# Hansard-T/FHE-Linformer

Hardware: AMD Instinct MI355X
Metric: encrypted Linformer-d128 forward ms/sample (lower is better)
Workload: dtype u64

## Files before the change

fhe-linformer_amd/capi.py:

```python
import ctypes as C
import os

import numpy as np

_HERE = os.path.dirname(os.path.abspath(__file__))
_LIB = None


class FhelinError(RuntimeError):
    def __init__(self, code, msg):
        super().__init__(f"fhelin error {code}: {msg}")
        self.code = code


class Params(C.Structure):
    _fields_ = [
        ("log_n", C.c_int32), ("n_q", C.c_int32), ("first_bits", C.c_int32), ("scale_bits", C.c_int32),
        ("n_p", C.c_int32), ("special_bits", C.c_int32), ("dnum", C.c_int32), ("log_slots", C.c_int32),
        ("hamming", C.c_int32), ("device", C.c_int32), ("seed", C.c_uint64),
    ]


PRESETS = {
    "bench": dict(log_n=16, n_q=24, first_bits=55, scale_bits=52, n_p=6, special_bits=60, dnum=4, log_slots=14, hamming=192),
# ... 127 lines not shown
        "fhelin_fc_rotsum": (i32, [vp, vp, i32, i32, C.POINTER(vp)]),
        "fhelin_fc_repeat": (i32, [vp, vp, i32, i32, C.POINTER(vp)]),
        "fhelin_fc_add_many": (i32, [vp, C.POINTER(vp), i32, C.POINTER(vp)]),
        "fhelin_fc_matmul_pt": (i32, [vp, C.POINTER(vp), i32, vp, vp, i32, i32, C.POINTER(vp)]),
        "fhelin_fc_matmul_ct": (i32, [vp, C.POINTER(vp), i32, vp, i32, i32, C.POINTER(vp)]),
        "fhelin_fc_matmulRElarge": (i32, [vp, C.POINTER(vp), i32, C.POINTER(vp), i32, vp, C.c_double, C.POINTER(vp)]),
        "fhelin_fc_matmulCRlarge": (i32, [vp, C.POINTER(vp), i32, C.POINTER(vp), vp, C.POINTER(vp)]),
        "fhelin_fc_matmulScores": (i32, [vp, C.POINTER(vp), i32, vp, C.POINTER(vp)]),
        "fhelin_fc_wrapUpRepeated": (i32, [vp, C.POINTER(vp), i32, C.POINTER(vp)]),
        "fhelin_fc_wrapUpExpanded": (i32, [vp, C.POINTER(vp), i32, C.POINTER(vp)]),
        "fhelin_fc_unwrapExpanded": (i32, [vp, vp, i32, C.POINTER(vp)]),
        "fhelin_fc_unwrapScoresExpanded": (i32, [vp, vp, i32, C.POINTER(vp)]),
        "fhelin_fc_unwrap_512_in_4_128": (i32, [vp, vp, i32, C.POINTER(vp)]),
        "fhelin_fc_unwrapRepeatedLarge": (i32, [vp, C.POINTER(vp), i32, i32, C.POINTER(vp)]),
        "fhelin_fc_generate_containers": (i32, [vp, C.POINTER(vp), i32, vp, C.POINTER(vp), C.POINTER(i32)]),
        "fhelin_fc_wrap_containers": (i32, [vp, C.POINTER(vp), i32, i32, C.POINTER(vp)]),
        "fhelin_mult_real": (i32, [vp, vp, C.c_double, C.POINTER(vp)]),
        "fhelin_add_real": (i32, [vp, vp, C.c_double, C.POINTER(vp)]),
        "fhelin_mult_many": (i32, [vp, C.POINTER(vp), i32, C.POINTER(vp)]),
        "fhelin_lincomb": (i32, [vp, C.POINTER(vp), C.POINTER(C.c_double), i32, C.c_double, C.POINTER(vp)]),
        "fhelin_eval_poly": (i32, [vp, vp, C.POINTER(C.c_double), i32, C.POINTER(vp)]),
        "fhelin_eval_chebyshev": (i32, [vp, vp, C.POINTER(C.c_double), i32, C.c_double, C.c_double, C.POINTER(vp)]),
        "fhelin_eval_chebyshev_batch": (i32, [vp, C.POINTER(vp), i32, C.POINTER(C.c_double), i32, C.c_double, C.c_double, C.POINTER(vp)]),
        "fhelin_bootstrap_setup": (i32, [vp, i32, i32, i32]),
        "fhelin_bootstrap": (i32, [vp, vp, C.POINTER(vp)]),
        "fhelin_bootstrap_config": (i32, [vp, i32, i32, i32, i32]),
        "fhelin_bootstrap_partial": (i32, [vp, vp, i32, C.POINTER(vp)]),
        "fhelin_bootstrap_drop": (i32, [vp, vp, i32, C.POINTER(vp)]),
        "fhelin_bootstrap_batch": (i32, [vp, C.POINTER(vp), i32, C.POINTER(vp)]),
        "fhelin_bootstrap_iter": (i32, [vp, vp, i32, C.POINTER(vp)]),
        "fhelin_bootstrap_iter_batch": (i32, [vp, C.POINTER(vp), i32, i32, C.POINTER(vp)]),
        "fhelin_bootstrap_iter_drop": (i32, [vp, vp, i32, i32, C.POINTER(vp)]),
        "fhelin_bootstrap_describe": (i32, [vp, C.POINTER(i32), i32, C.POINTER(i32)]),
        "fhelin_bootstrap_diag": (i32, [vp, i32, i32, i32, C.POINTER(vp)]),
        "fhelin_bootstrap_cheb": (i32, [vp, C.POINTER(C.c_double), i32, C.POINTER(i32)]),
        "fhelin_fcb_matmulScores": (i32, [vp, C.POINTER(vp), i32, C.POINTER(vp), i32, C.POINTER(vp)]),
        "fhelin_fcb_matmul_ct": (i32, [vp, C.POINTER(vp), C.POINTER(vp), i32, i32, i32, C.POINTER(vp)]),
        "fhelin_fcb_wrapUpRepeated": (i32, [vp, C.POINTER(vp), i32, i32, C.POINTER(vp)]),
        "fhelin_fcb_wrapUpExpanded": (i32, [vp, C.POINTER(vp), i32, i32, C.POINTER(vp)]),
        "fhelin_fcb_unwrapExpanded": (i32, [vp, C.POINTER(vp), i32, i32, C.POINTER(vp)]),
        "fhelin_fcb_unwrapRepeatedLarge": (i32, [vp, C.POINTER(vp), i32, i32, i32, C.POINTER(vp)]),
        "fhelin_fcb_generate_containers": (i32, [vp, C.POINTER(vp), i32, i32, vp, C.POINTER(vp), C.POINTER(i32)]),
        "fhelin_fc_rotsum_batch": (i32, [vp, C.POINTER(vp), i32, i32, i32, i32, C.POINTER(vp)]),
        "fhelin_add_plain_batch": (i32, [vp, C.POINTER(vp), i32, vp, C.POINTER(vp)]),
        "fhelin_eval_poly_batch": (i32, [vp, C.POINTER(vp), i32, C.POINTER(C.c_double), i32, C.POINTER(vp)]),
        "fhelin_mult_many_batch": (i32, [vp, C.POINTER(vp), i32, i32, C.POINTER(vp)]),
        "fhelin_evalkeys_save": (i32, [vp, C.c_char_p]),
        "fhelin_evalkeys_params": (i32, [C.c_char_p, C.POINTER(Params)]),
        "fhelin_evalkeys_info": (i32, [C.c_char_p, C.POINTER(i32), C.POINTER(i32)]),
        "fhelin_evalkeys_load": (i32, [vp, C.c_char_p]),
        "fhelin_evalkeys_save_compact": (i32, [vp, C.c_char_p]),
        "fhelin_ctx_set_seeded_keys": (i32, [vp, i32]),
        "fhelin_ctx_key_set_seed": (i32, [vp, vp]),
        "fhelin_debug_key_digest": (i32, [vp, vp, i32, i32, C.POINTER(C.c_uint64), C.POINTER(i32)]),
        "fhelin_ctx_set_seeded_encryption": (i32, [vp, i32]),
        "fhelin_ct_compact_bytes": (i32, [vp, C.POINTER(C.c_size_t)]),
        "fhelin_ct_export_compact": (i32, [vp, vp, vp, C.c_size_t]),
        "fhelin_compact_info": (i32, [vp, C.c_size_t, C.POINTER(i32), C.POINTER(i32), C.POINTER(i32), C.POINTER(i32)]),
        "fhelin_ct_import_compact": (i32, [vp, C.POINTER(vp), C.POINTER(C.c_size_t), i32, C.POINTER(vp)]),
        "fhelin_debug_seeded_expand": (i32, [vp, vp, C.c_uint64, i32, i32, i32, vp, f32p]),
        "fhelin_client_ingest_wrapped": (i32, [vp, vp, vp, vp, i32, i32, vp, vp, vp, vp, vp, vp, i32, i32, vp, C.POINTER(vp),
                                               C.POINTER(i32), vp]),
        "fhelin_client_ingest_wrapped_interleaved": (i32, [vp, i32, C.POINTER(vp), C.POINTER(vp), vp, i32, i32, vp, vp, vp, vp, vp, vp, i32,
                                                           i32, vp, C.POINTER(vp), C.POINTER(i32), C.POINTER(vp)]),
        "fhelin_wrapped_info": (i32, [vp, C.POINTER(i32), C.POINTER(i32), C.POINTER(i32), vp, i32]),
        "fhelin_unwrap_inputs": (i32, [vp, C.POINTER(vp), i32, C.POINTER(vp)]),
        "fhelin_sanitize": (i32, [vp, C.POINTER(vp), i32, vp, i32, i32, C.POINTER(vp)]),
        "fhelin_debug_flood": (i32, [vp, vp, C.c_uint64, i32, i32, vp, C.c_size_t]),
        "fhelin_decrypt_flooded": (i32, [vp, vp, i32, C.POINTER(C.c_double), i32]),
        "fhelin_debug_sampler_peek": (i32, [vp, i32, vp, u64p]),
        "fhelin_debug_pt_from_residues": (i32, [vp, vp, i32, C.POINTER(vp)]),
        "fhelin_debug_pt_from_residues_full": (i32, [vp, vp, C.c_double, C.c_double, C.POINTER(vp)]),
        "fhelin_lt_create": (i32, [vp, C.POINTER(C.c_double), C.POINTER(i32), i32, i32, i32, C.POINTER(vp)]),
        "fhelin_lt_create_pts": (i32, [vp, C.POINTER(vp), C.POINTER(i32), C.POINTER(i32), i32, i32, C.POINTER(vp)]),
        "fhelin_lt_info": (i32, [vp, C.POINTER(i32), C.POINTER(i32), C.POINTER(i32), C.POINTER(i32)]),
        "fhelin_lt_rotations": (i32, [vp, C.POINTER(i32), i32, C.POINTER(i32)]),
        "fhelin_lt_apply": (i32, [vp, vp, C.POINTER(vp), i32, i32, C.POINTER(vp)]),
        "fhelin_lt_free": (None, [vp]),
        "fhelin_debug_dot_plain": (i32, [vp, C.POINTER(vp), C.POINTER(vp), i32, C.POINTER(vp)]),
        "fhelin_debug_dot_groups": (i32, [vp, C.POINTER(vp), i32, i32, C.POINTER(vp), i32, C.POINTER(vp)]),
        "fhelin_debug_dot_cyclic": (i32, [vp, C.POINTER(vp), i32, C.POINTER(vp), C.POINTER(vp)]),
        "fhelin_debug_dot_window": (i32, [vp, C.POINTER(vp), C.POINTER(vp), C.POINTER(vp), C.POINTER(vp), i32]),
        "fhelin_debug_rotate_many_batch": (i32, [vp, C.POINTER(vp), i32, C.POINTER(i32), i32, C.POINTER(vp)]),
        "fhelin_ctx_set_interleave": (i32, [vp, i32]),
        "fhelin_ctx_interleave": (i32, [vp, C.POINTER(i32)]),
        "fhelin_evalkeys_interleave": (i32, [C.c_char_p, C.POINTER(i32)]),
        "fhelin_encrypt_interleaved_batch": (i32, [vp, C.POINTER(C.c_double), i32, i32, i32, i32, C.POINTER(vp)]),
        "fhelin_decrypt_interleaved": (i32, [vp, vp, i32, C.POINTER(C.c_double), i32]),
        "fhelin_decrypt_batch": (i32, [vp, C.POINTER(vp), i32, i32, i32, C.POINTER(i32), i32, C.POINTER(C.c_double), i32]),
        "fhelin_ctx_set_device_decode": (i32, [vp, i32]),
        "fhelin_client_ingest_interleaved": (i32, [vp, i32, C.POINTER(vp), C.POINTER(vp), vp, i32, i32, vp, vp, vp, vp, vp, vp, i32, i32,
                                                   C.POINTER(vp), C.POINTER(vp)]),
    }
    for name, (res, args) in sigs.items():
        fn = getattr(lib, name)
        fn.restype = res
        fn.argtypes = args
    _LIB = lib
    return lib


def compact_info(blob):
    lib = load_library()
    b = bytes(blob)
    v = [C.c_int32() for _ in range(4)]
    rc = lib.fhelin_compact_info(C.c_char_p(b), len(b), *[C.byref(x) for x in v])
    if rc != 0:
        raise FhelinError(rc, lib.fhelin_last_error().decode())
    return dict(zip(("log_n", "ell", "deg", "slots"), (x.value for x in v)))


def interleave(vectors):
    v = np.asarray(vectors)
    assert v.ndim == 2
    return np.ascontiguousarray(v.T).reshape(-1)


def deinterleave(physical, stride):
    w = np.asarray(physical)
    assert w.ndim == 1 and w.size % stride == 0
    return np.ascontiguousarray(w.reshape(-1, stride).T)


def _np_u64(a):
    a = np.ascontiguousarray(a, dtype=np.uint64)
    return a, a.ctypes.data_as(C.c_void_p)


class DevBuf:

    def __init__(self, eng, nbytes):
        self.eng, self.nbytes = eng, int(nbytes)
        p = C.c_void_p()
        eng._ck(eng.lib.fhelin_dev_alloc(eng.h, self.nbytes, C.byref(p)))
        self.ptr = p

    def upload(self, arr):
        arr = np.ascontiguousarray(arr)
        assert arr.nbytes <= self.nbytes
        self.eng._ck(self.eng.lib.fhelin_dev_upload(self.eng.h, self.ptr, arr.ctypes.data_as(C.c_void_p), arr.nbytes))
        return self

    def download(self, shape, dtype=np.uint64):
        out = np.empty(shape, dtype=dtype)
        assert out.nbytes <= self.nbytes
        self.eng._ck(self.eng.lib.fhelin_dev_download(self.eng.h, out.ctypes.data_as(C.c_void_p), self.ptr, out.nbytes))
        return out

    def free(self):
        if self.ptr:
            self.eng._ck(self.eng.lib.fhelin_dev_free(self.eng.h, self.ptr))
            self.ptr = None


class Engine:

    def __init__(self, preset="bench", device=0, seed=0, seed_bytes=None, interleave=1, **overrides):
        self.lib = load_library()
        cfg = dict(PRESETS[preset]) if isinstance(preset, str) else dict(preset)
        cfg.update(overrides)
        self.params = Params(device=device, seed=seed, **cfg)
        h = C.c_void_p()
        if seed_bytes is not None:
            assert len(seed_bytes) == 32
            sb = (C.c_uint8 * 32)(*bytes(seed_bytes))
            rc = self.lib.fhelin_ctx_create_seeded(C.byref(self.params), sb, C.byref(h))
# ... 632 lines not shown

    def raw_mult_relin(self, a, b):
        return self._un(self.lib.fhelin_raw_mult_relin, a, b.h)

    @staticmethod
    def _harr_opt(objs):
        return (C.c_void_p * len(objs))(*[(o.h if o is not None else None) for o in objs])

    def debug_pt_from_residues(self, residues):
        r = np.ascontiguousarray(residues, dtype=np.uint64)
        ell, n = r.shape
        assert n == self.N
        h = C.c_void_p()
        self._ck(self.lib.fhelin_debug_pt_from_residues(self.h, r.ctypes.data_as(C.c_void_p), ell, C.byref(h)))
        return Pt(self, h)

    def debug_pt_from_residues_full(self, residues, scale):
        r = np.ascontiguousarray(residues, dtype=np.uint64)
        assert r.shape == (self.n_q + self.n_p, self.N)
        hi = float(scale)
        lo = float(np.longdouble(scale) - np.longdouble(hi))
        h = C.c_void_p()
        self._ck(self.lib.fhelin_debug_pt_from_residues_full(self.h, r.ctypes.data_as(C.c_void_p), hi, lo, C.byref(h)))
        return Pt(self, h)

    def lt_create(self, diags, indices, n1=0, slots=None):
        slots = (1 << self.params.log_slots) if slots is None else int(slots)
        n = len(indices)
        d = np.ascontiguousarray(diags, dtype=np.float64).reshape(n, -1) if n else np.zeros((0, slots))
        assert n == 0 or d.shape[1] == slots
        idx = (C.c_int32 * max(n, 1))(*[int(i) for i in indices])
        h = C.c_void_p()
        self._ck(self.lib.fhelin_lt_create(self.h, d.ctypes.data_as(C.POINTER(C.c_double)), idx, n, slots, int(n1), C.byref(h)))
        return LinearTransform(self, h)

    def lt_create_pts(self, pts, baby, giant):
        n2, n1 = len(giant), len(baby)
        assert len(pts) == n2 and all(len(r) == n1 for r in pts)
        b = (C.c_int32 * n1)(*[int(i) for i in baby])
        g = (C.c_int32 * n2)(*[int(i) for i in giant])
        h = C.c_void_p()
        self._ck(self.lib.fhelin_lt_create_pts(self.h, self._harr_opt([p for r in pts for p in r]), b, g, n1, n2, C.byref(h)))
        return LinearTransform(self, h)

    def lt_apply(self, lt, v, rescale=False):
        outs = self._outs(max(len(v), 1))
        self._ck(self.lib.fhelin_lt_apply(self.h, lt.h, self._harr(v), len(v), int(bool(rescale)), outs))
        return self._cts(outs, len(v))

    def debug_dot_plain(self, cts, pts):
        assert len(cts) == len(pts)
        h = C.c_void_p()
        self._ck(self.lib.fhelin_debug_dot_plain(self.h, self._harr(cts), self._harr(pts), len(cts), C.byref(h)))
        return Ct(self, h)

    def debug_dot_groups(self, cts, pts):
        nb, na, ng = len(cts), len(cts[0]), len(pts)
        assert all(len(r) == na for r in cts) and all(len(r) == na for r in pts)
        outs = self._outs(nb * ng)
        self._ck(self.lib.fhelin_debug_dot_groups(self.h, self._harr([c for r in cts for c in r]), nb, na,
                                                  self._harr_opt([p for r in pts for p in r]), ng, outs))
        flat = self._cts(outs, nb * ng)
        return [flat[x * ng:(x + 1) * ng] for x in range(nb)]

    def debug_dot_cyclic(self, cts, pts):
        assert len(pts) == 32
        outs = self._outs(32)
        self._ck(self.lib.fhelin_debug_dot_cyclic(self.h, self._harr(cts), len(cts), self._harr(pts), outs))
        return self._cts(outs, 32)

    def debug_dot_window(self, cur, prev, pts, dest, accumulate=False):
        assert len(cur) == len(prev) == len(pts) == len(dest) == 32
        self._ck(self.lib.fhelin_debug_dot_window(self.h, self._harr_opt(cur), self._harr_opt(prev), self._harr(pts), self._harr(dest),
                                                  int(bool(accumulate))))

    def debug_rotate_many_batch(self, cts, indices):
        n = len(indices)
        idx = (C.c_int32 * n)(*indices)
        outs = self._outs(len(cts) * n)
        self._ck(self.lib.fhelin_debug_rotate_many_batch(self.h, self._harr(cts), len(cts), idx, n, outs))
        flat = self._cts(outs, len(cts) * n)
        return [flat[i * n:(i + 1) * n] for i in range(len(cts))]

    @staticmethod
    def _harr(objs):
        return (C.c_void_p * len(objs))(*[o.h for o in objs])

    def _outs(self, n):
        return (C.c_void_p * n)()

    def _cts(self, arr, n):
        return [Ct(self, C.c_void_p(arr[i])) for i in range(n)]

    def mult_real(self, a, k):
        return self._un(self.lib.fhelin_mult_real, a, float(k))

    def add_real(self, a, k):
        return self._un(self.lib.fhelin_add_real, a, float(k))

    def mult_many(self, v):
        h = C.c_void_p()
        self._ck(self.lib.fhelin_mult_many(self.h, self._harr(v), len(v), C.byref(h)))
        return Ct(self, h)

    def lincomb(self, v, coeffs, c0=0.0):
        cf = np.ascontiguousarray(coeffs, dtype=np.float64)
        h = C.c_void_p()
        self._ck(self.lib.fhelin_lincomb(self.h, self._harr(v), cf.ctypes.data_as(C.POINTER(C.c_double)), len(v), float(c0), C.byref(h)))
        return Ct(self, h)

    def eval_poly(self, x, coeffs):
        cf = np.ascontiguousarray(coeffs, dtype=np.float64)
        return self._un(self.lib.fhelin_eval_poly, x, cf.ctypes.data_as(C.POINTER(C.c_double)), cf.size)

    def eval_chebyshev(self, x, coeffs, a=-1.0, b=1.0):
        cf = np.ascontiguousarray(coeffs, dtype=np.float64)
        return self._un(self.lib.fhelin_eval_chebyshev, x, cf.ctypes.data_as(C.POINTER(C.c_double)), cf.size, float(a), float(b))

    def eval_chebyshev_batch(self, xs, coeffs, a=-1.0, b=1.0):
        cf = np.ascontiguousarray(coeffs, dtype=np.float64)
        outs = self._outs(len(xs))
        self._ck(self.lib.fhelin_eval_chebyshev_batch(self.h, self._harr(xs), len(xs), cf.ctypes.data_as(C.POINTER(C.c_double)), cf.size,
                                                      float(a), float(b), outs))
        return self._cts(outs, len(xs))

    def bootstrap(self, a):
        return self._un(self.lib.fhelin_bootstrap, a)

    def bootstrap_setup(self, budget_enc=3, budget_dec=3, slots=0):
        self._ck(self.lib.fhelin_bootstrap_setup(self.h, budget_enc, budget_dec, slots))

    def bootstrap_config(self, K=28, R=3, cheb_degree=47, correction=10):
        self._ck(self.lib.fhelin_bootstrap_config(self.h, K, R, cheb_degree, correction))

    def bootstrap_batch(self, v):
        outs = self._outs(len(v))
        self._ck(self.lib.fhelin_bootstrap_batch(self.h, self._harr(v), len(v), outs))
        return self._cts(outs, len(v))

    def bootstrap_drop(self, a, drop):
        return self._un(self.lib.fhelin_bootstrap_drop, a, int(drop))

    def bootstrap_iter(self, a, precision):
        return self._un(self.lib.fhelin_bootstrap_iter, a, int(precision))

    def bootstrap_iter_batch(self, v, precision):
        outs = self._outs(len(v))
        self._ck(self.lib.fhelin_bootstrap_iter_batch(self.h, self._harr(v), len(v), int(precision), outs))
        return self._cts(outs, len(v))

    def bootstrap_iter_drop(self, a, precision, drop):
        return self._un(self.lib.fhelin_bootstrap_iter_drop, a, int(precision), int(drop))

    def bootstrap_describe(self):
        n = C.c_int32()
        self._ck(self.lib.fhelin_bootstrap_describe(self.h, None, 0, C.byref(n)))
        d = (C.c_int32 * n.value)()
        self._ck(self.lib.fhelin_bootstrap_describe(self.h, d, n.value, C.byref(n)))
        d = list(d)
        out = dict(zip(("packed", "slots", "K", "R", "cheb_degree", "correction", "depth"), d[:7]))
        out["packed"] = bool(out["packed"])
        n_c2s, n_s2c = d[7], d[8]
        pos, stages = 9, []
        for k in range(n_c2s + n_s2c):
            which, idx = (0, k) if k < n_c2s else (1, k - n_c2s)
            st_slots, nt = d[pos], d[pos + 1]
# ... 306 lines not shown
```

fhe-linformer_amd/csrc/capi_debug.cpp:

```cpp
#include "../../include/fhelin.h"
#include <hip/hip_runtime.h>
#include <algorithm>
#include <vector>
#include "capi_internal.h"

using namespace fhelin;

#define NEED(x) if (!(x)) return capi_fail(FHELIN_ERR_ARG, "null argument")

namespace {
std::vector<CtPtr> cts_in(fhelin_ctx* c, const fhelin_ct* const* v, int n, bool nullable = false) {
    std::vector<CtPtr> in(n);
    for (int i = 0; i < n; ++i) {
        if (!v[i]) {
            if (!nullable) throw Error(FHELIN_ERR_ARG, "null ciphertext in array");
            continue;
        }
        const CtPtr& p = ct_in(c, v[i]);
        if (p->npoly != 2 || p->deg != 1) throw Error(FHELIN_ERR_ARG, "debug_dot: operands are degree-1 ciphertexts of two components");
        in[i] = p;
    }
    return in;
}
std::vector<PtPtr> pts_in(const fhelin_pt* const* v, int n, bool nullable = false) {
// ... 58 lines not shown

int fhelin_debug_dot_plain(fhelin_ctx* c, const fhelin_ct* const* cts, const fhelin_pt* const* pts, int32_t n, fhelin_ct** out) {
    NEED(c && cts && pts && out);
    FHELIN_TRY
    if (n < 1) throw Error(FHELIN_ERR_ARG, "debug_dot_plain: at least one term");
    *out = wrap(c, c->ev.dot_plain(cts_in(c, cts, n), pts_in(pts, n)));
    FHELIN_CATCH
}

int fhelin_debug_dot_groups(fhelin_ctx* c, const fhelin_ct* const* cts, int32_t nb, int32_t na, const fhelin_pt* const* pts, int32_t ng,
                            fhelin_ct** outs) {
    NEED(c && cts && pts && outs);
    FHELIN_TRY
    if (nb < 1 || na < 1 || na > EwDotGroups::MAX_A || ng < 1 || ng > EwDotGroups::MAX_G)
        throw Error(FHELIN_ERR_ARG, "debug_dot_groups: 1 <= na <= 16, 1 <= ng <= 8, nb >= 1");
    std::vector<CtPtr> flat = cts_in(c, cts, nb * na);
    std::vector<std::vector<PtPtr>> p(ng);
    for (int g = 0; g < ng; ++g) p[g] = pts_in(pts + (size_t)g * na, na, true);
    const CtPtr& f = flat[0];
    for (const CtPtr& x : flat)
        if (x->ell != f->ell) throw Error(FHELIN_ERR_ARG, "debug_dot_groups: operands of one limb count");
    std::vector<CtPtr> dest = c->ev.new_ct_batch(nb * ng, 2, f->ell, f->deg + 1, f->scale, f->slots);
    bool ok;
    if (nb == 1) {
        ok = c->ev.dot_plain_groups(flat, p, 0, dest);
    } else {
        flat = c->ev.make_contiguous(flat);
        std::vector<std::vector<CtPtr>> in(nb), o(nb);
        for (int x = 0; x < nb; ++x) {
            in[x].assign(flat.begin() + (size_t)x * na, flat.begin() + (size_t)(x + 1) * na);
            o[x].assign(dest.begin() + (size_t)x * ng, dest.begin() + (size_t)(x + 1) * ng);
        }
        ok = c->ev.dot_plain_groups_batch(in, p, 0, o);
    }
    if (!ok) throw Error(FHELIN_ERR_STATE, "debug_dot_groups: the evaluator refused the operands (no fall-back here)");
    for (int i = 0; i < nb * ng; ++i) outs[i] = wrap(c, dest[i]);
    FHELIN_CATCH
}

int fhelin_debug_dot_cyclic(fhelin_ctx* c, const fhelin_ct* const* cts, int32_t n, const fhelin_pt* const* pts, fhelin_ct** outs) {
    NEED(c && cts && pts && outs);
    FHELIN_TRY
    constexpr int P = EwCyclic::PERIOD;
    if (n < 1 || n > P) throw Error(FHELIN_ERR_ARG, "debug_dot_cyclic: 1 <= n <= 32");
    std::vector<CtPtr> in = cts_in(c, cts, n);
    std::vector<CtPtr> dest = c->ev.new_ct_batch(P, 2, in[0]->ell, in[0]->deg + 1, in[0]->scale, in[0]->slots);
    if (!c->ev.dot_plain_cyclic(in, pts_in(pts, P), dest))
        throw Error(FHELIN_ERR_STATE, "debug_dot_cyclic: the evaluator refused the operands (no fall-back here)");
    for (int k = 0; k < P; ++k) outs[k] = wrap(c, dest[k]);
    FHELIN_CATCH
}

int fhelin_debug_dot_window(fhelin_ctx* c, const fhelin_ct* const* cur, const fhelin_ct* const* prev, const fhelin_pt* const* pts,
                            fhelin_ct* const* dest, int32_t accumulate) {
    NEED(c && cur && prev && pts && dest);
    FHELIN_TRY
    constexpr int W = EwWindow::W;
    std::vector<CtPtr> d(W);
    for (int t = 0; t < W; ++t) {
        if (!dest[t]) throw Error(FHELIN_ERR_ARG, "null ciphertext in array");
        d[t] = ct_in(c, dest[t]);
    }
    if (!c->ev.dot_plain_window(cts_in(c, cur, W, true), cts_in(c, prev, W, true), pts_in(pts, W), d, accumulate != 0))
        throw Error(FHELIN_ERR_STATE, "debug_dot_window: the evaluator refused the operands (no fall-back here)");
    FHELIN_CATCH
}

int fhelin_debug_rotate_many_batch(fhelin_ctx* c, const fhelin_ct* const* cts, int32_t n_ct, const int32_t* indices, int32_t n,
                                   fhelin_ct** outs) {
    NEED(c && cts && indices && outs);
    FHELIN_TRY
    if (n_ct < 1 || n < 1) throw Error(FHELIN_ERR_ARG, "debug_rotate_many_batch: at least one ciphertext and one index");
    std::vector<CtPtr> in(n_ct);
    for (int i = 0; i < n_ct; ++i) {
        if (!cts[i]) throw Error(FHELIN_ERR_ARG, "null ciphertext in array");
        in[i] = ct_in(c, cts[i]);
    }
    const std::vector<std::vector<CtPtr>> o = c->ev.rotate_many_batch(in, std::vector<int>(indices, indices + n));
    for (int i = 0; i < n_ct; ++i)
        for (int k = 0; k < n; ++k) outs[(size_t)i * n + k] = wrap(c, o[i][k]);
    FHELIN_CATCH
}

}
```

fhe-linformer_amd/csrc/context.cpp:

```cpp
#include "context.h"
#include <hip/hip_runtime.h>
#include <algorithm>
#include <cstdio>
#include <cstdlib>
#include <cstring>
#include <sys/random.h>
#include <time.h>
#include <cxxabi.h>
#include <dlfcn.h>
#include <execinfo.h>

namespace fhelin {

template <class T>
const T* Context::upload_table(const std::vector<T>& v) {
    void* p = nullptr;
    size_t bytes = std::max<size_t>(v.size() * sizeof(T), 16);
    hip_check(hipMalloc(&p, bytes), "hipMalloc(table)");
    if (!v.empty()) hip_check(hipMemcpy(p, v.data(), v.size() * sizeof(T), hipMemcpyHostToDevice), "hipMemcpy(table)");
    table_allocs.push_back(p);
    return static_cast<const T*>(p);
}
template const u64* Context::upload_table<u64>(const std::vector<u64>&);
template const int* Context::upload_table<int>(const std::vector<int>&);
// ... 19 lines not shown
        while (got < sizeof p.seed_bytes) {
            const ssize_t n = getrandom(p.seed_bytes + got, sizeof p.seed_bytes - got, 0);
            if (n <= 0) throw Error(FHELIN_ERR_INTERNAL, "getrandom failed: no entropy for key generation");
            got += (size_t)n;
        }
    }
    p.have_seed_bytes = true;
}

static Params resolve_params(Params p) {
    resolve_seed(p);
    if (p.n_p < 0 && p.n_q >= 1 && p.dnum >= 1 && p.special_bits >= 1) {
        const int a = (p.n_q + p.dnum - 1) / p.dnum;
        const int first = p.first_bits + (std::min(a, p.n_q) - 1) * p.scale_bits;
        const int other = p.n_q > a ? std::min(a, p.n_q - a) * p.scale_bits : 0;
        p.n_p = (std::max(first, other) + p.special_bits - 1) / p.special_bits;
    }
    return p;
}

Context::Context(const Params& p_in) : prm(resolve_params(p_in)) {
    const Params& p = prm;
    if (p.log_n < 12 || p.log_n > 17) throw Error(FHELIN_ERR_ARG, "log_n must be in [12,17]");
    if (p.n_q < 1 || p.n_q > 64 || p.n_p < 0 || p.n_p > 16) throw Error(FHELIN_ERR_ARG, "bad limb counts");
    if (p.dnum < 1) throw Error(FHELIN_ERR_ARG, "dnum must be >= 1");
    if (p.first_bits > 60 || p.scale_bits > 60 || p.special_bits > 60) throw Error(FHELIN_ERR_ARG, "primes must be <= 60 bits");
    if (p.first_bits < 20 || p.scale_bits < 20 || (p.n_p > 0 && p.special_bits < 20)) throw Error(FHELIN_ERR_ARG, "primes must be >= 20 bits");
    if (p.log_slots < 1 || p.log_slots > p.log_n - 1) throw Error(FHELIN_ERR_ARG, "log_slots out of range");
    N = 1 << p.log_n;
    L = p.n_q - 1;
    K = p.n_p;
    alpha = (p.n_q + p.dnum - 1) / p.dnum;
    if (alpha > 16) throw Error(FHELIN_ERR_ARG, "digit size > 16 limbs not supported");
    if ((p.n_q + alpha - 1) / alpha > 16) throw Error(FHELIN_ERR_ARG, "more than 16 key-switching digits not supported");
    try {
        chain = make_prime_chain(p.log_n, p.n_q, p.first_bits, p.scale_bits, p.n_p, p.special_bits);
    } catch (const std::exception& e) {
        throw Error(FHELIN_ERR_ARG, std::string("prime chain: ") + e.what());
    }
    moduli = chain.q;
    moduli.insert(moduli.end(), chain.p.begin(), chain.p.end());
    for (u64 q : moduli)
        if (q >> 60) throw Error(FHELIN_ERR_ARG, "prime chain: a modulus is >= 2^60 (lower scale_bits or first_bits)");
    for (u64 q : moduli) {
        barrett.push_back(h_barrett(q));
        tw.push_back(make_twiddles(q, p.log_n));
    }
    sf_real.assign(p.n_q + 1, 0.0L);
    sf_real[0] = (long double)chain.q[L];
    for (int k = 0; k < L; ++k) sf_real[k + 1] = sf_real[k] * sf_real[k] / (long double)chain.q[L - k];

    pool.fill_word = DevicePool::parse_fill(std::getenv("FHELIN_POOL_FILL"));

    if (p.device < 0) return;

    int ndev = 0;
    if (hipGetDeviceCount(&ndev) != hipSuccess || ndev <= 0)
        throw Error(FHELIN_ERR_NO_DEVICE, "no HIP device visible: the fhe-linformer_amd engine has no CPU fallback");
    if (p.device >= ndev) throw Error(FHELIN_ERR_ARG, "device index out of range");
    hip_check(hipSetDevice(p.device), "hipSetDevice");
    hip_check(hipStreamCreateWithFlags(&stream, hipStreamNonBlocking), "hipStreamCreate");
    main_stream = stream;
    own_stream = true;
    {
        int want = 2;
        if (const char* e = std::getenv("FHELIN_LANES")) want = std::atoi(e);
        n_lanes = std::max(0, std::min(want, DevicePool::MAX_LANES - 1));
        for (int k = 1; k <= n_lanes; ++k) {
            hip_check(hipStreamCreateWithFlags(&lane_stream[k], hipStreamNonBlocking), "hipStreamCreate(lane)");
            hip_check(hipEventCreateWithFlags(&lane_event[k], hipEventDisableTiming), "hipEventCreate(lane)");
        }
        hip_check(hipEventCreateWithFlags(&fork_event, hipEventDisableTiming), "hipEventCreate(fork)");
        pool.lane_stream[0] = main_stream;
        for (int k = 1; k <= n_lanes; ++k) pool.lane_stream[k] = lane_stream[k];
        pool.have_streams = true;
        if (const char* e = std::getenv("FHELIN_ASYNC")) async_lanes = std::atoi(e) != 0;
        if (const char* e = std::getenv("FHELIN_FUSE_MODDOWN")) fuse_moddown = std::atoi(e) != 0;
        if (const char* e = std::getenv("FHELIN_FUSE_FINISH")) fuse_finish = std::atoi(e) != 0;
        if (const char* e = std::getenv("FHELIN_HOST_ENCODE")) host_encode = std::atoi(e) != 0;
        if (const char* e = std::getenv("FHELIN_DEVICE_DECODE")) device_decode = std::atoi(e) != 0;
        if (const char* e = std::getenv("FHELIN_ROT_GATHER")) rot_gather = std::atoi(e) != 0;
        if (const char* e = std::getenv("FHELIN_FUSE_LIFT")) fuse_lift = std::atoi(e) != 0;
        if (const char* e = std::getenv("FHELIN_LDS_DIGITS")) lds_digits = std::atoi(e) != 0;
        if (const char* e = std::getenv("FHELIN_NTT_TRACE")) trace_small_ntt = std::atoi(e);
        if (const char* e = std::getenv("FHELIN_SCALAR_TRACE")) trace_scalar = std::atoi(e);
        if (const char* e = std::getenv("FHELIN_HOST_WAITS")) trace_waits = std::atoi(e) != 0;
    }
    hip_check(hipEventCreate(&ev_start), "hipEventCreate");
    stage_words = (size_t)2 << p.log_n;
    for (int i = 0; i < STAGE_SLOTS; ++i) {
        hip_check(hipHostMalloc(reinterpret_cast<void**>(&stage_buf[i]), stage_words * sizeof(u64), hipHostMallocDefault), "hipHostMalloc(stage)");
        hip_check(hipEventCreateWithFlags(&stage_ev[i], hipEventDisableTiming), "hipEventCreate(stage)");
    }
    hip_check(hipHostMalloc(reinterpret_cast<void**>(&small_buf), (size_t)SMALL_SLOTS * SMALL_WORDS * sizeof(u64), hipHostMallocDefault), "hipHostMalloc(stage, small)");
    for (int i = 0; i < SMALL_SLOTS; ++i) hip_check(hipEventCreateWithFlags(&small_ev[i], hipEventDisableTiming), "hipEventCreate(stage, small)");
    hip_check(hipEventCreate(&ev_stop), "hipEventCreate");
    has_device = true;

    const int nl = (int)moduli.size();
    {
        std::vector<u64> bar(2 * nl), ninv(8 * nl, 0);
        for (int i = 0; i < nl; ++i) {
            bar[2 * i] = barrett[i].r0;
            bar[2 * i + 1] = barrett[i].r1;
            ninv[8 * i] = tw[i].n_inv;
            ninv[8 * i + 1] = tw[i].n_inv_s;
            ninv[8 * i + 2] = tw[i].w1_n_inv;
            ninv[8 * i + 3] = tw[i].w1_n_inv_s;
            int bits = 0;
            while (bits < 64 && (moduli[i] >> bits)) ++bits;
            if (bits >= 12 && bits <= 60) {
                ninv[8 * i + 4] = (u64)(bits - 10);
                ninv[8 * i + 5] = (u64)((((u128)1) << (bits + 22)) / moduli[i]);
            }
        }
        dt.log_n = p.log_n;
        dt.n_limbs = nl;
        dt.moduli = upload_table(moduli);
        dt.barrett = upload_table(bar);
        {
            std::vector<u64> qi(nl);
            for (int i = 0; i < nl; ++i) {
                u64 x = moduli[i];
                for (int it = 0; it < 6; ++it) x *= 2 - moduli[i] * x;
                qi[i] = x;
            }
            dt.qinv = upload_table(qi);
            std::vector<u64> mr(2 * (size_t)nl);
            for (int i = 0; i < nl; ++i) {
                mr[2 * i] = mont_r(moduli[i]);
                mr[2 * i + 1] = h_shoup(mr[2 * i], moduli[i]);
            }
            dt.mont = upload_table(mr);
        }
        dt.ninv = upload_table(ninv);
        std::vector<u64> f((size_t)nl * 2 * N), g((size_t)nl * 2 * N);
        for (int i = 0; i < nl; ++i) {
            std::memcpy(&f[(size_t)i * 2 * N], tw[i].fwd.data(), sizeof(u64) * 2 * N);
            std::memcpy(&g[(size_t)i * 2 * N], tw[i].inv.data(), sizeof(u64) * 2 * N);
        }
        dt.tw_fwd = upload_table(f);
        dt.tw_inv = upload_table(g);
        const size_t tiles = N >> 12;
        const size_t per_limb = tiles * 15 * 256 * 2;
        for (int dir = 0; dir < 2; ++dir) {
            const std::vector<u64>& src = dir ? g : f;
            std::vector<u64> r((size_t)nl * per_limb);
            for (int i = 0; i < nl; ++i)
                for (size_t T = 0; T < tiles; ++T)
                    for (int kb = 0; kb < 4; ++kb)
                        for (int j = 0; j < (8 >> kb); ++j)
                            for (size_t tau = 0; tau < 256; ++tau) {
                                const size_t idx = (N >> (kb + 1)) + ((((T << 8) | tau)) << (3 - kb)) + j;
                                const size_t s_ = (size_t)(8 >> kb) - 1 + j;
                                const size_t o = (size_t)i * per_limb + ((T * 15 + s_) * 256 + tau) * 2;
                                r[o] = src[(size_t)i * 2 * N + 2 * idx];
                                r[o + 1] = src[(size_t)i * 2 * N + 2 * idx + 1];
                            }
            (dir ? dt.tw_rows_inv : dt.tw_rows_fwd) = upload_table(r);
        }
    }
    {
        std::vector<u64> phatinv(2 * std::max(K, 1)), phatmod((size_t)std::max(K, 1) * (L + 1)), pinv(2 * (L + 1));
        for (int j = 0; j < K; ++j) {
            u64 pj = chain.p[j];
            u64 hat = prod_mod(chain.p, j, pj);
// ... 307 lines not shown
```

fhe-linformer_amd/csrc/context.h:

```cpp
#pragma once
#include <cstdint>
#include <map>
#include <memory>
#include <stdexcept>
#include <string>
#include <unordered_map>
#include <vector>
#include <hip/hip_runtime_api.h>
#include "../../include/fhelin.h"
#include "hostmath.h"
#include "pool.h"
#include "kernels.h"

namespace fhelin {

struct Params {
    int log_n = 16;
    int n_q = 24;
    int first_bits = 55;
    int scale_bits = 52;
    int n_p = 6;
    int special_bits = 60;
    int dnum = 4;
    int log_slots = 14;
// ... 51 lines not shown
    hipStream_t lane_stream[DevicePool::MAX_LANES] = {};
    hipEvent_t lane_event[DevicePool::MAX_LANES] = {};
    hipEvent_t fork_event = nullptr;
    bool async_lanes = true;
    int async_rr = 0;
    u64 lane_seq[DevicePool::MAX_LANES] = {};
    std::vector<std::pair<u64, std::shared_ptr<void>>> lane_hold[DevicePool::MAX_LANES];
    void release_holds(int lane, u64 up_to_seq);
    void fork_lanes();
    void join_lanes();
    struct LaneScope {
        Context& c;
        LaneScope(Context& ctx, int k) : c(ctx) {
            c.stream = c.lane_stream[k];
            c.pool.cur_lane = k;
        }
        ~LaneScope() {
            c.stream = c.main_stream;
            c.pool.cur_lane = 0;
        }
    };
    DevicePool pool;
    DeviceTables dt{};
    std::vector<void*> table_allocs;
    hipEvent_t ev_start = nullptr, ev_stop = nullptr;

    static constexpr int STAGE_SLOTS = 64;
    u64* stage_buf[STAGE_SLOTS] = {};
    hipEvent_t stage_ev[STAGE_SLOTS] = {};
    bool stage_used[STAGE_SLOTS] = {};
    int stage_next = 0;
    size_t stage_words = 0;
    static constexpr int SMALL_SLOTS = 256;
    static constexpr size_t SMALL_WORDS = 8192;
    u64* small_buf = nullptr;
    hipEvent_t small_ev[SMALL_SLOTS] = {};
    bool small_used[SMALL_SLOTS] = {};
    int small_next = 0;
    void upload_async(u64* dst, const u64* src, size_t words);

    const u64* d_phatinv = nullptr;
    const u64* d_phatmod = nullptr;
    const u64* d_pinv = nullptr;
    const u64* d_pmod = nullptr;
    const u64* d_qlinv = nullptr;
    const u64* d_qlmod = nullptr;
    std::vector<LevelTables> lvl;
    std::map<u64, const u32*> automorph_maps;

    explicit Context(const Params& p);
    ~Context();
    Context(const Context&) = delete;
    Context& operator=(const Context&) = delete;

    void require_device() const;
    template <class T> T* dalloc(size_t count) { return static_cast<T*>(pool.alloc(count * sizeof(T))); }
    template <class T> Scratch<T> scratch(size_t count) { return Scratch<T>(pool, count); }
    template <class T> const T* upload_table(const std::vector<T>& v);
    int limb_id_q(int i) const { return i; }
    int limb_id_p(int j) const { return L + 1 + j; }
    int digits_at(int ell) const { return (ell + alpha - 1) / alpha; }
    u64 galois_element(long rot_index) const;
    int stride = 1;
    bool stride_explicit = false;
    bool stride_locked = false;
    u64 rot_element(int rot_index) const { return stride == 1 ? galois_element(rot_index) : galois_element((long)stride * rot_index); }
    struct PhysicalScope {
        Context& c;
        int was;
        explicit PhysicalScope(Context& ctx) : c(ctx), was(ctx.stride) { c.stride = 1; }
        ~PhysicalScope() { c.stride = was; }
    };
    const u32* automorph_map(u64 galois);
    const u32* automorph_inverse_of(const u32* map);
    std::map<const u32*, const u32*> automorph_inverse;
    u32 automorph_ginv_of(const u32* map) const;
    std::map<const u32*, u32> automorph_ginv;
    bool fuse_finish = true;
    bool fuse_moddown = false;
    bool host_encode = false;
    bool device_decode = false;
    bool rot_gather = true;
    bool fuse_lift = true;
    bool lds_digits = true;
    struct FftDev {
        const u32* rot = nullptr;
        const double* ksi = nullptr;
    };
    std::map<int, FftDev> fft_dev;
    void sync();
    void ntt(const LimbBatch& b, bool inverse, int active = -1) {
        stats.limb_ntt += (u64)(active >= 0 ? active : b.nvec);
        if (trace_small_ntt && b.nvec <= trace_small_ntt) note_small_ntt(b.nvec);
        launch_ntt(dt, b, inverse, stream);
    }
    bool trace_waits = false;
    std::map<std::string, std::pair<u64, u64>> wait_sites;
    void note_wait(const char* site, u64 ns) {
        auto& e = wait_sites[site];
        e.first += 1;
        e.second += ns;
    }
    int trace_small_ntt = 0;
    std::map<std::string, std::pair<u64, u64>> small_ntt_sites;
    void note_small_ntt(int nvec);
    int trace_scalar = 0;
    std::map<std::string, std::pair<u64, u64>> scalar_sites;
    void note_scalar(int nvec);
    void ntt_epilogue(const LimbBatch& b, const NttEpilogue& ep) {
        stats.limb_ntt += (u64)b.nvec;
        if (trace_small_ntt && b.nvec <= trace_small_ntt) note_small_ntt(b.nvec);
        launch_ntt_epilogue(dt, b, ep, stream);
    }
};

}
```

fhe-linformer_amd/csrc/evaluator.cpp:

```cpp
#include "evaluator.h"
#include <map>
#include <hip/hip_runtime.h>
#include <cmath>
#include <cstring>

namespace fhelin {

DevBlock::~DevBlock() {
    if (d && ctx) {
        try { ctx->pool.free(d); } catch (...) {}
    }
}
Ciphertext::~Ciphertext() {
    if (async_ev) (void)hipEventDestroy(async_ev);
    if (d && ctx && !block) {
        try { ctx->pool.free(d); } catch (...) {}
    }
}
Encoding::~Encoding() {
    if (ready) (void)hipEventDestroy(ready);
    if (d && ctx) {
        try { ctx->pool.free(d, lanes_ordered); } catch (...) {}
    }
}
// ... 115 lines not shown
            it.b[i] = nullptr;
        }
        launch_ew_items(c_.dt, it, 4, v[0]->ell, c_.stream);
    }
    hip_check(hipGetLastError(), "batch gather");
    return o;
}

KeyPtr Evaluator::new_key() {
    c_.require_device();
    auto k = std::make_shared<EvalKey>();
    k->ctx = &c_;
    k->digits = c_.digits_at(c_.L + 1);
    k->d = c_.dalloc<u64>(k->words());
    c_.stride_locked = true;
    return k;
}

void Evaluator::keyswitch(const u64* c_ntt, int ell, const EvalKey& key, u64* out, const u64* add0, const u64* add1,
                          const u32* map, const u64* post) {
    keyswitch_batch(1, c_ntt, 0, ell, key, out, 0, add0, add1, 0, map, post, 0);
}

void Evaluator::keyswitch_batch(int B, const u64* c_ntt, size_t c_stride, int ell, const EvalKey& key, u64* out, size_t out_stride,
                                const u64* add0, const u64* add1, size_t add_stride, const u32* map, const u64* post,
                                size_t post_stride) {
    keyswitch_impl(B, nullptr, c_ntt, c_stride, ell, &key, out, out_stride, add0, add1, add_stride, map, post, post_stride);
}

void Evaluator::keyswitch_rows(const KsRows& rows, const u64* c_ntt, size_t c_stride, int ell, u64* out, size_t out_stride,
                               const u64* add0, size_t add_stride) {
    const int B = (int)rows.keys.size();
    if (B < 1) return;
    if (B > KsShape::MAX_ROWS || rows.maps.size() != rows.keys.size()) throw Error(FHELIN_ERR_ARG, "keyswitch_rows: bad row count");
    keyswitch_impl(B, &rows, c_ntt, c_stride, ell, nullptr, out, out_stride, add0, nullptr, add_stride, nullptr, nullptr, 0);
}

void Evaluator::keyswitch_impl(int B, const KsRows* rows, const u64* c_ntt, size_t c_stride, int ell, const EvalKey* key, u64* out,
                               size_t out_stride, const u64* add0, const u64* add1, size_t add_stride, const u32* map, const u64* post,
                               size_t post_stride) {
    c_.require_device();
    if (c_.K < 1) throw Error(FHELIN_ERR_STATE, "hybrid key switching needs at least one special prime");
    if (B < 1) return;
    const size_t N = c_.N;
    const int K = c_.K;
    KsShape sh{ell, K, c_.alpha, c_.lvl[ell].beta, c_.L + 1, B, c_stride, out_stride, add_stride, post_stride};
    const bool shared = rows && rows->shared_input;
    if (rows) {
        sh.per_row = 1;
        sh.shared_input = shared ? 1 : 0;
        for (int b = 0; b < B; ++b) {
            sh.evk_row[b] = rows->keys[b]->d;
            sh.map_row[b] = rows->maps[b];
        }
    }
    KsShape shu = sh;
    shu.batch = shared ? 1 : B;
    c_.stats.keyswitch += (u64)B;
    c_.stats.keyswitch_limbs += (u64)B * ell;
    const bool identity = !map && !rows;
    const bool gather = !identity && !add1 && rot_in_gather();
    const u64* evk = key ? key->d : nullptr;
    if (gather) {
        sh.gather = 1;
        if (rows) {
            for (int b = 0; b < B; ++b) {
                sh.evk_row[b] = permuted(*rows->keys[b], rows->maps[b]);
                sh.ginv_row[b] = c_.automorph_ginv_of(rows->maps[b]);
            }
        } else {
            evk = permuted(*key, map);
            sh.map_row[0] = map;
            sh.ginv = c_.automorph_ginv_of(map);
        }
        if (add0) {
            sh.gsrc = add0;
            sh.gsrc_stride = add_stride;
            sh.gsrc_pmod = c_.d_pmod;
        }
    }
    Scratch<u64> ext = modup(shu, c_ntt, !gather);
    Scratch<u64> accQ = c_.scratch<u64>((size_t)B * 2 * ell * N);
    Scratch<u64> accP = c_.scratch<u64>((size_t)B * 2 * K * N);
    launch_ks_inner(c_.dt, sh, accQ, accP, ext, evk, c_ntt, c_.stream);
    if (gather) moddown(sh, accQ, accP, out, nullptr, nullptr, nullptr, post, true);
    else moddown(sh, accQ, accP, out, add0, add1, map, post, c_.fuse_moddown || (c_.fuse_finish && identity));
    launch_ok("keyswitch");
}


Scratch<u64> Evaluator::modup(const KsShape& up, const u64* src, bool times_r2, int group2, size_t group2_stride) {
    const size_t N = c_.N;
    const int n = up.batch, ell = up.ell, nt = ell + c_.K;
    const LevelTables& lt = c_.lvl[ell];
    Scratch<u64> cc = c_.scratch<u64>((size_t)n * ell * N);
    {
        LimbBatch ib{cc, n * ell, nullptr, 0, ell, src};
        if (n > 1 && up.c_stride != (size_t)ell * N) {
            ib.src_group = ell;
            ib.src_group_stride = up.c_stride;
        }
        if (group2 > 0) {
            ib.src_group2 = group2;
            ib.src_group2_stride = group2_stride;
        }
        c_.ntt(ib, true);
    }
    Scratch<u64> ext = c_.scratch<u64>((size_t)n * lt.beta * nt * N);
    launch_modup_conv(c_.dt, up, ext, cc, src, lt.up_hatinv, times_r2 ? lt.up_hatmod_r2 : lt.up_hatmod, c_.stream);
    LimbBatch eb{ext, n * lt.beta * nt, lt.ext_limb_tab, 0, 1};
    eb.tab_len = lt.beta * nt;
    eb.lazy_out = true;
    c_.ntt(eb, false, n * (lt.beta * nt - ell));
    return ext;
}

void Evaluator::moddown(const KsShape& sh, const u64* accQ, u64* accP, u64* out, const u64* add0, const u64* add1, const u32* map,
                        const u64* post, bool row_pass, const std::function<void(const u64* conv)>& finish) {
    const size_t N = c_.N;
    const int B = sh.batch, ell = sh.ell, K = c_.K;
    if (row_pass && sh.gsrc && !sh.gsrc_pmod) throw Error(FHELIN_ERR_INTERNAL, "moddown: the row pass cannot gather");
    c_.ntt(LimbBatch{accP, B * 2 * K, nullptr, c_.L + 1, K}, true);
    Scratch<u64> conv = c_.scratch<u64>((size_t)B * 2 * ell * N);
    launch_moddown_conv(c_.dt, sh, conv, accP, c_.d_phatinv, c_.d_phatmod, c_.stream);
    const LimbBatch cb{conv, B * 2 * ell, nullptr, 0, ell};
    if (row_pass) {
        NttEpilogue ep;
        ep.acc = accQ;
        ep.acc_poly_stride = (size_t)ell * N;
        ep.out = out;
        ep.out_stride = sh.out_stride;
        ep.w = c_.d_pinv;
        ep.ell = ell;
        ep.add0 = add0;
        ep.add1 = add1;
        ep.add_stride = sh.add_stride;
        ep.post = post;
        ep.post_stride = sh.post_stride;
        if (sh.gather) {
        } else if (sh.per_row) {
            ep.per_row = 1;
            for (int b = 0; b < B; ++b) ep.invmap_row[b] = c_.automorph_inverse_of(sh.map_row[b]);
        } else if (map) {
            ep.invmap = c_.automorph_inverse_of(map);
        }
        c_.ntt_epilogue(cb, ep);
        return;
    }
    c_.ntt(cb, false);
    if (finish) finish(conv);
    else launch_moddown_finish(c_.dt, sh, out, accQ, conv, c_.d_pinv, add0, add1, map, post, c_.stream);
}

void Evaluator::moddown_rescale(const KsShape& sh, const u64* accQ, u64* accP, u64* out) {
    const size_t N = c_.N;
    const int B = sh.batch, ell = sh.ell, K = c_.K;
    const LevelTables& lt = c_.lvl[ell];
    c_.ntt(LimbBatch{accP, B * 2 * K, nullptr, c_.L + 1, K}, true);
    Scratch<u64> top = c_.scratch<u64>((size_t)B * 2 * N);
    {
        LimbBatch tb{top, B * 2, nullptr, ell - 1, 1, accQ + (size_t)(ell - 1) * N};
        tb.src_group = 1;
        tb.src_group_stride = (size_t)ell * N;
        c_.ntt(tb, true);
    }
    Scratch<u64> conv = c_.scratch<u64>((size_t)B * 2 * (ell - 1) * N);
    launch_moddown_rescale_conv(c_.dt, sh, conv, accP, top, lt.md_hatinv, lt.md_hatmod, lt.md_mmod, c_.stream);
    moddown_rescale_finish(sh, out, accQ, conv, lt.md_minv);
}

void Evaluator::moddown_rescale_exact(const KsShape& sh, const u64* accQ, u64* accP, u64* out, u32 f2) {
    const size_t N = c_.N;
    const int B = sh.batch, ell = sh.ell, K = c_.K;
    const LevelTables& lt = c_.lvl[ell];
    {
        LimbBatch ib{accP, B * 2 * (K + 1), lt.mdx_limb_tab, 0, 1};
        ib.tab_len = K + 1;
        c_.ntt(ib, true);
    }
    Scratch<u64> conv = c_.scratch<u64>((size_t)B * 2 * (ell - 1) * N);
    launch_moddown_rescale_exact_conv(c_.dt, sh, f2, conv, accP, c_.d_phatinv, c_.d_phatmod, c_.d_pinv, c_.d_pmod,
                                      c_.d_qlmod + (size_t)(ell - 1) * (c_.L + 1), c_.stream);
    moddown_rescale_finish(sh, out, accQ, conv, lt.md_minv);
}

void Evaluator::moddown_rescale_finish(const KsShape& sh, u64* out, const u64* accQ, u64* conv, const u64* minv) {
    const int e1 = sh.ell - 1;
    const LimbBatch cb{conv, sh.batch * 2 * e1, nullptr, 0, e1};
    if (c_.fuse_finish) {
        NttEpilogue ep;
        ep.acc = accQ;
        ep.acc_poly_stride = (size_t)sh.ell * c_.N;
        ep.out = out;
        ep.out_stride = sh.out_stride;
        ep.w = minv;
        ep.ell = e1;
        c_.ntt_epilogue(cb, ep);
        return;
    }
    c_.ntt(cb, false);
    launch_moddown_rescale_finish(c_.dt, sh, out, accQ, conv, minv, c_.stream);
}

Evaluator::Rotations Evaluator::rotations(const int* indices, int n) {
    Rotations rot;
    rot.n = n;
    for (int r = 0; r < n; ++r) {
        const RotKey k = rotation_key(indices[r]);
        rot.key[r] = k.key.get();
        rot.map[r] = k.map;
        if (k.g % (u64)(c_.N / 256) != 1) rot.tiles_in_place = false;
    }
    return rot;
}

void Evaluator::set_rotations(KsShape& sh, const Rotations& rot, bool shared_digits, const u64* const* keys) {
    sh.n_rot = rot.n;
    for (int r = 0; r < rot.n; ++r) {
        sh.map_rot[r] = rot.map[r];
        sh.evk_rot[r] = keys ? keys[r] : permuted(*rot.key[r], rot.map[r]);
    }
    if (shared_digits) sh.lds_digits = c_.lds_digits && rot.tiles_in_place ? 1 : 0;
}

void Evaluator::rotation_sum(KsShape& sh, const u64* ext, const u64* c1, const u64* c0, size_t c0_stride, u64* out, const u64* post) {
    const size_t N = c_.N;
    const bool rp = sum_in_row_pass();
    sh.gsrc = c0;
    sh.gsrc_stride = c0_stride;
    if (rp) sh.gsrc_pmod = c_.d_pmod;
    Scratch<u64> accQ = c_.scratch<u64>((size_t)sh.batch * 2 * sh.ell * N);
    Scratch<u64> accP = c_.scratch<u64>((size_t)sh.batch * 2 * sh.k * N);
    launch_ks_inner_multi(c_.dt, sh, accQ, accP, ext, c1, c_.stream);
    moddown(sh, accQ, accP, out, nullptr, nullptr, nullptr, post, rp);
}

int Evaluator::slot_count(int slots) const { return slots > 0 ? slots : (1 << c_.prm.log_slots); }

Evaluator::RotKey Evaluator::rotation_key(int index) {
    const u64 g = c_.rot_element(index);
    auto it = rot_keys.find(g);
    if (it == rot_keys.end()) throw Error(FHELIN_ERR_KEY, "no rotation key for index " + std::to_string(index) + " (EvalRotateKeyGen list)");
    return RotKey{it->second, c_.automorph_map(g), g};
}

bool Evaluator::have_rotation_keys(const std::vector<int>& indices, int slots) const {
    const int ns = slot_count(slots);
    for (int r : indices) {
        if (r % ns == 0) return false;
        if (!rot_keys.count(c_.rot_element(r))) return false;
    }
    return !indices.empty();
}

const u64* Evaluator::permuted(const EvalKey& key, const u32* map) {
    if (key.d_perm) return key.d_perm;
    const int nvec = key.digits * 2 * (c_.L + 1 + c_.K);
    key.d_perm = c_.dalloc<u64>(key.words());
    launch_automorph_pack30(c_.dt, key.d_perm, key.d, map, nvec, c_.stream);
    launch_ok("key permutation");
    hip_check(hipStreamSynchronize(c_.stream), "key permutation sync");
    return key.d_perm;
}

std::vector<CtPtr> Evaluator::rotate_sum_batch(const std::vector<CtPtr>& vin, const std::vector<int>& indices) {
    if (vin.empty()) return {};
    const int R = (int)indices.size();
    if (R < 1 || R > KsShape::MAX_ROT) throw Error(FHELIN_ERR_ARG, "rotate_sum_batch: 1..7 rotations");
    if (!have_rotation_keys(indices, vin[0]->slots)) throw Error(FHELIN_ERR_KEY, "rotate_sum_batch: missing rotation key");
    if (c_.K < 1) throw Error(FHELIN_ERR_STATE, "hybrid key switching needs at least one special prime");
    const Rotations rot = rotations(indices.data(), R);
    const size_t N = c_.N;
    return for_groups(vin.size(), batch_limit, [&](size_t f, size_t i) { return same_shape(*vin[f], *vin[i]); },
                      [&](const std::vector<size_t>& idx) {
        if (vin[idx[0]]->npoly != 2) throw Error(FHELIN_ERR_STATE, "rotate: ciphertext must have 2 components");
        const std::vector<CtPtr> chunk = make_contiguous(pick(vin, idx), 0);
        const int B = (int)chunk.size(), ell = chunk[0]->ell;
        const size_t pn = (size_t)ell * N, ctw = 2 * pn;
        std::vector<CtPtr> o = new_ct_batch(B, 2, ell, chunk[0]->deg, chunk[0]->scale, chunk[0]->slots);
        const u64* base = chunk[0]->d;
        KsShape sh{ell, c_.K, c_.alpha, c_.lvl[ell].beta, c_.L + 1, B, ctw, ctw, pn, ctw};
        set_rotations(sh, rot, true);
        int steps = 0;
        while ((1 << steps) < R + 1) ++steps;
        c_.stats.keyswitch += (u64)B * steps;
        c_.stats.keyswitch_limbs += (u64)B * steps * ell;
        {
            Scratch<u64> ext = modup(sh, base + pn, false);
            rotation_sum(sh, ext, base + pn, base, ctw, o[0]->d, base);
            launch_ok("rotate_sum_batch");
        }
        for (int b = 0; b < B; ++b) o[b]->scale = vin[idx[b]]->scale;
        return o;
    });
}

Evaluator::FoldedKey Evaluator::folded_key(const PtPtr& p, int index, long double scale) {
    const RotKey rk = rotation_key(index);
    for (size_t i = 0; i < folded_keys.size(); ++i) {
        const FoldedKey& f = folded_keys[i];
        if (f.pt.get() == p.get() && f.key.get() == rk.key.get() && f.index == index && f.scale == scale) {
            FoldedKey hit = f;
            if (i + 1 != folded_keys.size()) {
                folded_keys.erase(folded_keys.begin() + i);
                folded_keys.push_back(hit);
            }
            return hit;
        }
    }
    FoldedKey f;
    f.pt = p;
    f.key = rk.key;
    f.index = index;
    f.scale = scale;
    const int nl = c_.L + 1 + c_.K;
    f.enc = p->at(nl, scale);
    f.d = std::make_shared<DevBlock>();
    f.d->ctx = &c_;
    f.d->d = c_.dalloc<u64>(f.key->words());
    launch_fold_key(c_.dt, f.d->d, f.key->d, rk.map, f.enc->d, f.key->digits * 2 * nl, c_.stream);
    launch_ok("fold_key");
    hip_check(hipStreamSynchronize(c_.stream), "fold_key sync");
    if (folded_keys.size() >= MAX_FOLDED) {
        hip_check(hipStreamSynchronize(c_.main_stream), "folded key eviction sync");
        for (int k = 1; k <= c_.n_lanes; ++k) hip_check(hipStreamSynchronize(c_.lane_stream[k]), "folded key eviction sync (lane)");
        folded_keys.erase(folded_keys.begin());
    }
    folded_keys.push_back(f);
    return f;
}

std::vector<CtPtr> Evaluator::hoisted_dot_rows(const std::vector<CtPtr>& xin, const std::vector<PtPtr>& pts, const std::vector<int>& indices,
                                              bool rescale_out) {
    if (xin.empty()) return {};
    const int R = (int)indices.size();
    if (R < 1 || R > KsShape::MAX_ROT || (int)pts.size() != R + 1)
        throw Error(FHELIN_ERR_ARG, "hoisted_dot_rows: 1..7 rotations, one plaintext per rotation + the unrotated term's");
    if (!have_rotation_keys(indices, xin[0]->slots)) throw Error(FHELIN_ERR_KEY, "hoisted_dot_rows: missing rotation key");
    if (c_.K < 1) throw Error(FHELIN_ERR_STATE, "hybrid key switching needs at least one special prime");
    const int ns = slot_count(xin[0]);
    for (int r : indices)
        if (r % ns == 0) throw Error(FHELIN_ERR_ARG, "hoisted_dot_rows: a rotation by 0 is the unrotated term (pts[0])");
    if (rescale_out && c_.K + 1 > 16)
        return rescale_batch(hoisted_dot_rows(xin, pts, indices, false));
    std::vector<CtPtr> x = xin;
    {
        std::vector<CtPtr> need;
        std::vector<size_t> pos;
        for (size_t i = 0; i < x.size(); ++i)
            if (x[i]->deg >= 2) {
                need.push_back(x[i]);
                pos.push_back(i);
            }
        if (!need.empty()) {
            std::vector<CtPtr> r = rescale_batch(need);
            for (size_t k = 0; k < pos.size(); ++k) x[pos[k]] = r[k];
        }
    }
    const Rotations rot = rotations(indices.data(), R);
    const size_t N = c_.N;
    const int K = c_.K;
    hipStream_t s = c_.stream;
    return for_groups(x.size(), batch_limit, [&](size_t f, size_t i) { return same_shape(*x[f], *x[i]); },
                      [&](const std::vector<size_t>& idx) {
        if (x[idx[0]]->npoly != 2) throw Error(FHELIN_ERR_STATE, "hoisted_dot_rows: ciphertext must have 2 components");
        const std::vector<CtPtr> chunk = make_contiguous(pick(x, idx), 0);
        const int B = (int)chunk.size(), ell = chunk[0]->ell;
        const size_t pn = (size_t)ell * N, ctw = 2 * pn;
        const long double sf = c_.sf_real[chunk[0]->level()];
        const bool merged = rescale_out && ell >= 2 && K + 1 <= 16;
        if (rescale_out && !merged) throw Error(FHELIN_ERR_STATE, "hoisted_dot_rows: no limb left to drop");
        const int oell = merged ? ell - 1 : ell;
        std::vector<CtPtr> o = new_ct_batch(B, 2, oell, merged ? chunk[0]->deg : chunk[0]->deg + 1, chunk[0]->scale * sf, chunk[0]->slots);
        const u64* base = chunk[0]->d;
        KsShape sh{ell, K, c_.alpha, c_.lvl[ell].beta, c_.L + 1, B, ctw, (size_t)2 * oell * N, pn, ctw};
        HoistAdd h;
        h.n_rot = R;
        std::vector<FoldedKey> hold;
        const std::shared_ptr<Encoding> e0 = pts[0]->at(ell, sf);
        h.v[0] = e0->d;
        const u64* folded[KsShape::MAX_ROT];
        for (int r = 0; r < R; ++r) {
            hold.push_back(folded_key(pts[r + 1], indices[r], sf));
            folded[r] = hold.back().d->d;
            h.v[r + 1] = hold.back().enc->d;
        }
        set_rotations(sh, rot, true, folded);
        for (int r = 0; r < R; ++r) h.map[r] = sh.map_rot[r];
        c_.stats.keyswitch += (u64)B * R;
        c_.stats.keyswitch_limbs += (u64)B * R * ell;
        c_.stats.ct_pt_mult += (u64)B * (R + 1);
        c_.stats.ct_pt_limbs += (u64)B * (R + 1) * ell;
        if (merged) {
            c_.stats.rescale += (u64)B;
            c_.stats.rescale_limbs += (u64)B * ell;
        }
        {
            Scratch<u64> ext = modup(sh, base + pn, false);
            Scratch<u64> accQ = c_.scratch<u64>((size_t)B * 2 * ell * N);
            Scratch<u64> accP = c_.scratch<u64>((size_t)B * 2 * K * N);
            launch_ks_inner_multi(c_.dt, sh, accQ, accP, ext, base + pn, s);
            if (!merged) {
                Scratch<u64> pre = c_.scratch<u64>((size_t)B * ctw);
                launch_hoist_addends(c_.dt, sh, h, pre, base, s);
                moddown(sh, accQ, accP, o[0]->d, nullptr, nullptr, nullptr, pre, sum_in_row_pass());
            } else {
                h.acc = accQ;
                h.pmod = c_.d_pmod;
                launch_hoist_addends(c_.dt, sh, h, nullptr, base, s);
                moddown_rescale(sh, accQ, accP, o[0]->d);
            }
            launch_ok("hoisted_dot_rows");
        }
        for (int b = 0; b < B; ++b) {
            o[b]->scale = x[idx[b]]->scale * sf;
            if (merged) o[b]->scale = o[b]->scale / (long double)c_.chain.q[ell - 1];
        }
        return o;
    });
}

std::vector<CtPtr> Evaluator::linear_transform_rows(const std::vector<CtPtr>& xin, const std::vector<std::vector<PtPtr>>& pts,
                                                    const std::vector<int>& baby, const std::vector<int>& giant, bool rescale_out) {
    const int n1 = (int)baby.size(), n2 = (int)giant.size();
    if (n1 < 1 || n1 > LtDot::MAX_STEPS || n2 < 1 || (int)pts.size() != n2 || baby[0] != 0)
        throw Error(FHELIN_ERR_ARG, "linear_transform_rows: 1..32 baby steps (the first unrotated), >= 1 giant steps, pts [n2][n1]");
    for (const auto& row : pts)
        if ((int)row.size() != n1) throw Error(FHELIN_ERR_ARG, "linear_transform_rows: pts [n2][n1]");
    c_.require_device();
    if (c_.stride != 1) throw Error(FHELIN_ERR_STATE, "linear_transform_rows: interleaved samples (slot stride != 1) are not supported");
    if (c_.K < 1) throw Error(FHELIN_ERR_STATE, "hybrid key switching needs at least one special prime");
    if (xin.empty()) return {};
    const int ns = slot_count(xin[0]);
    struct Step {
        int b;
        const EvalKey* key;
        const u32* map;
    };
    std::vector<Step> steps;
    for (int b = 0; b < n1; ++b) {
        bool any = false;
        for (int g = 0; g < n2; ++g) any = any || pts[g][b];
        if (!any) continue;
        if (b > 0 && baby[b] % ns == 0) throw Error(FHELIN_ERR_ARG, "linear_transform_rows: a baby step by 0 is the unrotated term (baby[0])");
        if (b == 0) {
            steps.push_back(Step{0, nullptr, nullptr});
        } else {
            const RotKey rk = rotation_key(baby[b]);
            steps.push_back(Step{b, rk.key.get(), rk.map});
        }
    }
    if (steps.empty()) throw Error(FHELIN_ERR_ARG, "linear_transform_rows: no term");
    for (int g : giant)
        if (g % ns != 0) (void)rotation_key(g);
    std::vector<CtPtr> x = xin;
    rescale_degree2(x, nullptr, "linear_transform_rows: ciphertext must have 2 components");
    const size_t N = c_.N;
    const int K = c_.K, nl = c_.L + 1 + K;
    std::vector<CtPtr> out = for_groups(x.size(), std::max(1, batch_limit / n2), [&](size_t f, size_t i) { return same_shape(*x[f], *x[i]); },
                                        [&](const std::vector<size_t>& idx) {
        const std::vector<CtPtr> chunk = make_contiguous(pick(x, idx), 0);
        const int B = (int)chunk.size(), ell = chunk[0]->ell;
        const size_t pn = (size_t)ell * N, ctw = 2 * pn;
        const long double sf = c_.sf_real[chunk[0]->level()];
        std::vector<std::shared_ptr<Encoding>> enc((size_t)n2 * n1);
        size_t terms = 0;
        for (int g = 0; g < n2; ++g)
            for (int b = 0; b < n1; ++b)
                if (pts[g][b]) {
                    enc[(size_t)g * n1 + b] = pts[g][b]->at(nl, sf);
                    ++terms;
                }
        std::vector<CtPtr> o = new_ct_batch(B * n2, 2, ell, chunk[0]->deg + 1, chunk[0]->scale * sf, chunk[0]->slots);
        const u64* base = chunk[0]->d;
        KsShape sh{ell, K, c_.alpha, c_.lvl[ell].beta, c_.L + 1, B, ctw, ctw, pn, ctw};
        c_.stats.ct_pt_mult += (u64)B * terms;
        c_.stats.ct_pt_limbs += (u64)B * terms * ell;
        {
            Scratch<u64> ext = modup(sh, base + pn, false);
            Scratch<u64> accQ = c_.scratch<u64>((size_t)B * n2 * 2 * ell * N);
            Scratch<u64> accP = c_.scratch<u64>((size_t)B * n2 * 2 * K * N);
            std::vector<Scratch<u64>> tabs;
            for (int g0 = 0; g0 < n2; g0 += LtStep::MAX_G) {
                LtDot ld;
// ... 360 lines not shown
    bool uniform = xs.size() >= 2 && !c_.fuse_moddown && c_.K >= 1;
    for (const CtPtr& x : xs)
        uniform = uniform && x->npoly == 2 && x->ell == xs[0]->ell && x->deg == xs[0]->deg && x->slots == xs[0]->slots;
    if (!uniform) {
        for (size_t i = 0; i < xs.size(); ++i) out[i] = rotate_many(xs[i], indices);
        return out;
    }
    const int ns = slot_count(xs[0]);
    std::vector<size_t> todo;
    for (size_t i = 0; i < xs.size(); ++i) out[i].resize(indices.size());
    for (size_t k = 0; k < indices.size(); ++k) {
        if (indices[k] % ns == 0)
            for (size_t i = 0; i < xs.size(); ++i) out[i][k] = xs[i];
        else
            todo.push_back(k);
    }
    const int R = (int)todo.size();
    if (R == 0) return out;
    const bool gather = rot_in_gather() && R <= (int)KsShape::MAX_ROWS;
    std::vector<const EvalKey*> keys;
    std::vector<const u32*> maps;
    for (size_t k : todo) {
        const RotKey rk = rotation_key(indices[k]);
        keys.push_back(rk.key.get());
        maps.push_back(rk.map);
    }
    const size_t N = c_.N;
    const int K = c_.K, L1 = c_.L + 1, ell = xs[0]->ell;
    const size_t pn = (size_t)ell * N, ctw = 2 * pn;
    const LevelTables& lt = c_.lvl[ell];
    const int nt = ell + K;
    hipStream_t s = c_.stream;
    const size_t per_pass = (size_t)std::max(1, 160 / R);
    for (size_t lo = 0; lo < xs.size(); lo += per_pass) {
        const size_t hi = std::min(xs.size(), lo + per_pass);
        const int B = (int)(hi - lo);
        std::vector<CtPtr> in = make_contiguous(std::vector<CtPtr>(xs.begin() + lo, xs.begin() + hi), 6);
        const u64* base = in[0]->d;
        const int rows = B * R;
        c_.stats.keyswitch += (u64)rows;
        c_.stats.keyswitch_limbs += (u64)rows * ell;
        std::vector<CtPtr> o = new_ct_batch(rows, 2, ell, xs[lo]->deg, xs[lo]->scale, xs[lo]->slots);
        {
            Scratch<u64> ext = modup(KsShape{ell, K, c_.alpha, lt.beta, L1, B, ctw, 0, 0, 0}, base + pn, !gather);
            Scratch<u64> accQ = c_.scratch<u64>((size_t)rows * 2 * ell * N);
            Scratch<u64> accP = c_.scratch<u64>((size_t)rows * 2 * K * N);
            auto row_shape = [&](int first, int cnt) {
                KsShape sh{ell, K, c_.alpha, lt.beta, L1, B * cnt, ctw, ctw, ctw, 0};
                sh.per_row = 1;
                sh.shared_input = 1;
                sh.row_mod = cnt;
                sh.ext_batch_stride = (size_t)lt.beta * nt * N;
                for (int b = 0; b < cnt; ++b) {
                    sh.evk_row[b] = keys[first + b]->d;
                    sh.map_row[b] = maps[first + b];
                }
                return sh;
            };
            auto for_row_chunks = [&](auto&& launch) {
                for (int i = 0; i < B; ++i)
                    for (int first = 0; first < R; first += KsShape::MAX_ROWS) {
                        const int cnt = std::min(R - first, (int)KsShape::MAX_ROWS);
                        KsShape sh1{ell, K, c_.alpha, lt.beta, L1, cnt, 0, ctw, 0, 0};
                        sh1.per_row = 1;
                        sh1.shared_input = 1;
                        for (int b = 0; b < cnt; ++b) {
                            sh1.evk_row[b] = keys[first + b]->d;
                            sh1.map_row[b] = maps[first + b];
                        }
                        launch(sh1, (size_t)i * R + first, i);
                    }
            };
            const bool one_chunk = R <= (int)KsShape::MAX_ROWS;
            if (gather) {
                KsShape sh = row_shape(0, R);
                sh.gather = 1;
                for (int b = 0; b < R; ++b) {
                    sh.evk_row[b] = permuted(*keys[b], maps[b]);
                    sh.ginv_row[b] = c_.automorph_ginv_of(maps[b]);
                }
                sh.gsrc = base;
                sh.gsrc_stride = ctw;
                sh.gsrc_pmod = c_.d_pmod;
                launch_ks_inner(c_.dt, sh, accQ, accP, ext, nullptr, base + pn, s);
                moddown(sh, accQ, accP, o[0]->d, nullptr, nullptr, nullptr, nullptr, true);
            } else {
                if (one_chunk) launch_ks_inner(c_.dt, row_shape(0, R), accQ, accP, ext, nullptr, base + pn, s);
                else
                    for_row_chunks([&](const KsShape& sh1, size_t row0, int i) {
                        launch_ks_inner(c_.dt, sh1, accQ + row0 * 2 * ell * N, accP + row0 * 2 * K * N, ext + (size_t)i * lt.beta * nt * N, nullptr,
                                        base + pn + (size_t)i * ctw, s);
                    });
                moddown(KsShape{ell, K, c_.alpha, lt.beta, L1, rows, 0, ctw, 0, 0}, accQ, accP, nullptr, nullptr, nullptr, nullptr, nullptr, false,
                        [&](const u64* conv) {
                            if (one_chunk)
                                launch_moddown_finish(c_.dt, row_shape(0, R), o[0]->d, accQ, conv, c_.d_pinv, base, nullptr, nullptr, nullptr, s);
                            else
                                for_row_chunks([&](const KsShape& sh1, size_t row0, int i) {
                                    launch_moddown_finish(c_.dt, sh1, o[row0]->d, accQ + row0 * 2 * ell * N, conv + row0 * 2 * ell * N,
                                                          c_.d_pinv, base + (size_t)i * ctw, nullptr, nullptr, nullptr, s);
                                });
                        });
            }
            launch_ok("rotate_many_batch");
        }
        for (int i = 0; i < B; ++i)
            for (int r = 0; r < R; ++r) {
                o[(size_t)i * R + r]->scale = xs[lo + i]->scale;
                out[lo + i][todo[r]] = o[(size_t)i * R + r];
            }
    }
    return out;
}

std::vector<CtPtr> Evaluator::rescale_batch(const std::vector<CtPtr>& vin) {
    return for_groups(vin.size(), batch_limit,
                      [&](size_t f, size_t i) { return vin[i]->npoly == 2 && vin[f]->npoly == 2 && vin[i]->ell == vin[f]->ell; },
                      [&](const std::vector<size_t>& idx) {
        if (idx.size() < 2) return std::vector<CtPtr>{rescale(vin[idx[0]])};
        const std::vector<CtPtr> chunk = make_contiguous(pick(vin, idx), 5);
        const int B = (int)chunk.size(), ell = chunk[0]->ell, P = 2 * B;
        if (ell < 2) throw Error(FHELIN_ERR_STATE, "rescale: no limb left to drop");
        const size_t N = c_.N;
        const u64* base = chunk[0]->d;
        Scratch<u64> last = c_.scratch<u64>((size_t)P * N);
        c_.stats.rescale += (u64)B;
        c_.stats.rescale_limbs += (u64)B * ell;
        LimbBatch lb{last, P, nullptr, ell - 1, 1, base + (size_t)(ell - 1) * N};
        lb.src_group = 1;
        lb.src_group_stride = (size_t)ell * N;
        c_.ntt(lb, true);
        std::vector<CtPtr> o = new_ct_batch(B, 2, ell - 1, 1, 0, chunk[0]->slots);
        rescale_finish(o[0]->d, base, last, P, ell);
        launch_ok("rescale_batch");
        last.reset();
        for (int b = 0; b < B; ++b) {
            const CtPtr& a = vin[idx[b]];
            o[b]->scale = a->scale / (long double)c_.chain.q[ell - 1];
            o[b]->deg = a->deg > 1 ? a->deg - 1 : 1;
        }
        return o;
    });
}

std::vector<CtPtr> Evaluator::mult_plain_batch(const std::vector<CtPtr>& vin, const PtPtr& p) {
    return mult_plain_each(vin, std::vector<PtPtr>(vin.size(), p));
}

std::vector<CtPtr> Evaluator::mult_plain_each(const std::vector<CtPtr>& vin, const std::vector<PtPtr>& p) {
    if (vin.size() != p.size()) throw Error(FHELIN_ERR_ARG, "mult_plain_each: one plaintext per ciphertext");
    if (vin.empty()) return {};
    std::vector<CtPtr> x = vin;
    rescale_degree2(x);
    std::vector<CtPtr> out(x.size());
    bool one_shape = x.size() > 1;
    for (const CtPtr& c : x) one_shape = one_shape && c->npoly == x[0]->npoly && c->ell == x[0]->ell && c->deg == x[0]->deg;
    std::vector<CtPtr> all;
    if (one_shape) all = new_ct_batch((int)x.size(), x[0]->npoly, x[0]->ell, x[0]->deg + 1, x[0]->scale, x[0]->slots);
    for_runs(x.size(), [&](size_t a, size_t b) { return x[a]->npoly == x[b]->npoly && x[a]->ell == x[b]->ell && x[a]->deg == x[b]->deg; },
             [&](size_t lo, size_t hi) {
                 const CtPtr& f = x[lo];
                 std::vector<CtPtr> o = one_shape ? std::vector<CtPtr>(all.begin() + lo, all.begin() + hi)
                                                  : new_ct_batch((int)(hi - lo), f->npoly, f->ell, f->deg + 1, f->scale, f->slots);
                 EwItems it;
                 it.n = (int)(hi - lo);
                 it.vecs = f->npoly * f->ell;
                 it.b_vecs = f->ell;
// ... 331 lines not shown
    for (int k0 = 0; k0 < B; k0 += EwItems::MAX_ITEMS) {
        EwItems it;
        it.n = std::min(B - k0, (int)EwItems::MAX_ITEMS);
        for (int k = 0; k < it.n; ++k) {
            it.out[k] = d[k0 + k]->d;
            it.a[k] = x[idx[k0 + k]]->d;
            it.b[k] = y[idx[k0 + k]]->d;
        }
        launch_tensor_items(c_.dt, it, ell, c_.stream);
    }
    return d;
}

void Evaluator::product_operands(const std::vector<CtPtr>& a, const std::vector<CtPtr>& b, std::vector<CtPtr>& x, std::vector<CtPtr>& y) {
    std::vector<CtPtr> ra = a, rb = b;
    rescale_degree2(ra, &rb, "mult: operands must have 2 components");
    match_batch(ra, rb, x, y);
}

std::vector<CtPtr> Evaluator::mult_batch(const std::vector<CtPtr>& a, const std::vector<CtPtr>& b) {
    if (a.size() != b.size()) throw Error(FHELIN_ERR_ARG, "mult_batch: operand count mismatch");
    if (!relin_key) throw Error(FHELIN_ERR_KEY, "no relinearisation key (EvalMultKeyGen not called)");
    std::vector<CtPtr> x, y;
    product_operands(a, b, x, y);
    std::vector<CtPtr> out = for_groups(a.size(), batch_limit, [&](size_t f, size_t i) { return x[i]->ell == x[f]->ell; },
                                        [&](const std::vector<size_t>& idx) {
        const int B = (int)idx.size(), ell = x[idx[0]]->ell;
        const size_t pn = (size_t)ell * c_.N;
        const std::vector<CtPtr> d = tensor_products(x, y, idx);
        std::vector<CtPtr> o = new_ct_batch(B, 2, ell, 2, 0, x[idx[0]]->slots);
        keyswitch_batch(B, d[0]->d + 2 * pn, 3 * pn, ell, *relin_key, o[0]->d, 2 * pn, d[0]->d, d[0]->d + pn, 3 * pn, nullptr, nullptr, 0);
        for (int k = 0; k < B; ++k) {
            const size_t i = idx[k];
            o[k]->deg = x[i]->deg + y[i]->deg;
            o[k]->scale = x[i]->scale * y[i]->scale;
        }
        return o;
    });
    launch_ok("mult_batch");
    return out;
}

std::vector<CtPtr> Evaluator::mult_affine_rescale_batch(const std::vector<CtPtr>& a, const std::vector<CtPtr>& b, int f, double cadd,
                                                        const std::vector<CtPtr>& sub) {
    if (a.size() != b.size() || (!sub.empty() && sub.size() != a.size())) throw Error(FHELIN_ERR_ARG, "mult_affine_rescale_batch: operand count mismatch");
    if (f != 1 && f != 2) throw Error(FHELIN_ERR_ARG, "mult_affine_rescale_batch: factor 1 or 2");
    if (!relin_key) throw Error(FHELIN_ERR_KEY, "no relinearisation key (EvalMultKeyGen not called)");
    if (c_.K < 1 || c_.K + 1 > 16) throw Error(FHELIN_ERR_STATE, "mult_affine_rescale_batch: 1..15 special primes");
    std::vector<CtPtr> ra = a, rb = b, x(a.size()), y(a.size());
    rescale_degree2(ra, &rb, "mult: operands must have 2 components");
    for (size_t i = 0; i < a.size(); ++i) match(ra[i], rb[i], x[i], y[i]);
    const size_t N = c_.N;
    const int K = c_.K, L1 = c_.L + 1;
    hipStream_t s = c_.stream;
    auto product_scale = [&](size_t i) { return x[i]->scale * y[i]->scale; };
    return for_groups(a.size(), batch_limit,
                      [&](size_t f0, size_t i) { return x[i]->ell == x[f0]->ell && fabsl(product_scale(i) / product_scale(f0) - 1.0L) < 1e-12L; },
                      [&](const std::vector<size_t>& idx) {
        const size_t first = idx[0];
        const int B = (int)idx.size(), ell = x[first]->ell;
        if (ell < 2) throw Error(FHELIN_ERR_STATE, "mult_affine_rescale_batch: no limb left to drop");
        const size_t pn = (size_t)ell * N;
        const long double sc = product_scale(first);
        const LevelTables& lt = c_.lvl[ell];
        const std::vector<CtPtr> d = tensor_products(x, y, idx);
        std::vector<CtPtr> sadj;
        if (!sub.empty()) {
            for (int k = 0; k < B; ++k) sadj.push_back(adjust(sub[idx[k]], ell, 2, sc));
            sadj = make_contiguous(sadj, 7);
        }
        ScalarSet cst;
        if (cadd != 0.0) real_to_scalars(c_, (long double)cadd * sc, ell, cst);
        KsShape sh{ell, K, c_.alpha, lt.beta, L1, B, 3 * pn, (size_t)2 * (ell - 1) * N, pn, 0};
        c_.stats.keyswitch += (u64)B;
        c_.stats.keyswitch_limbs += (u64)B * ell;
        c_.stats.rescale += (u64)B;
        c_.stats.rescale_limbs += (u64)B * ell;
        const u64* c_ntt = d[0]->d + 2 * pn;
        std::vector<CtPtr> o = new_ct_batch(B, 2, ell - 1, 1, 0, x[first]->slots);
        {
            Scratch<u64> ext = modup(sh, c_ntt, true);
            Scratch<u64> accQ = c_.scratch<u64>((size_t)B * 2 * ell * N);
            Scratch<u64> accP = c_.scratch<u64>((size_t)B * 2 * K * N);
            launch_ks_inner(c_.dt, sh, accQ, accP, ext, relin_key->d, c_ntt, s);
            launch_affine_acc(c_.dt, sh, accQ, d[0]->d, sadj.empty() ? nullptr : sadj[0]->d, cst, cadd != 0.0 ? 1 : 0, f, c_.d_pmod, s);
            if (f == 2) launch_ew_add(c_.dt, accP, accP, accP, B * 2 * K, B * 2 * K, L1, K, s);
            moddown_rescale(sh, accQ, accP, o[0]->d);
            launch_ok("mult_affine_rescale_batch");
        }
        for (int k = 0; k < B; ++k) o[k]->scale = product_scale(idx[k]) / (long double)c_.chain.q[ell - 1];
        return o;
    });
}

std::vector<CtPtr> Evaluator::mult_affine_unmerged(const std::vector<CtPtr>& a, const std::vector<CtPtr>& b, const std::vector<AffineSpec>& spec) {
    std::vector<CtPtr> t = mult_batch(a, b);
    const size_t n = t.size();
    {
        std::vector<size_t> pos;
        std::vector<CtPtr> sel;
        for (size_t i = 0; i < n; ++i)
            if (spec[i].f == 2) {
                pos.push_back(i);
                sel.push_back(t[i]);
            }
        if (!sel.empty()) {
            const std::vector<CtPtr> r = add_batch(sel, sel);
            for (size_t j = 0; j < pos.size(); ++j) t[pos[j]] = r[j];
        }
    }
    for (size_t i = 0; i < n; ++i)
        if (spec[i].cadd != 0.0) t[i] = add_real(t[i], spec[i].cadd);
    for (const bool neg : {true, false}) {
        std::vector<size_t> pos;
        std::vector<CtPtr> sel, ad;
        for (size_t i = 0; i < n; ++i)
            if (spec[i].addend && spec[i].negate == neg) {
                pos.push_back(i);
                sel.push_back(t[i]);
                ad.push_back(spec[i].addend);
            }
        if (sel.empty()) continue;
        const std::vector<CtPtr> r = neg ? sub_batch(sel, ad) : add_batch(sel, ad);
        for (size_t j = 0; j < pos.size(); ++j) t[pos[j]] = r[j];
    }
    return rescale_batch(t);
}

std::vector<CtPtr> Evaluator::mult_affine_batch(const std::vector<CtPtr>& a, const std::vector<CtPtr>& b, const std::vector<AffineSpec>& spec) {
    if (a.size() != b.size() || spec.size() != a.size()) throw Error(FHELIN_ERR_ARG, "mult_affine_batch: operand count mismatch");
    if (!relin_key) throw Error(FHELIN_ERR_KEY, "no relinearisation key (EvalMultKeyGen not called)");
    for (const AffineSpec& sp : spec) {
        if (sp.f != 1 && sp.f != 2) throw Error(FHELIN_ERR_ARG, "mult_affine_batch: factor 1 or 2");
        if (sp.addend && sp.addend->npoly != 2) throw Error(FHELIN_ERR_STATE, "add: component count mismatch");
    }
    if (!exact_products_on()) return mult_affine_unmerged(a, b, spec);
    const size_t n = a.size();
    std::vector<CtPtr> x, y;
    product_operands(a, b, x, y);
    for (size_t i = 0; i < n; ++i)
        if (x[i]->ell < 2 || (spec[i].addend && spec[i].addend->ell < x[i]->ell)) return mult_affine_unmerged(x, y, spec);
    const size_t N = c_.N;
    const int K = c_.K, L1 = c_.L + 1;
    hipStream_t s = c_.stream;
    static_assert(AffineItems::MAX_ITEMS <= EwItems::MAX_ITEMS, "the tensor products of a group are one launch");
    return for_groups(n, std::min(batch_limit, (int)AffineItems::MAX_ITEMS), [&](size_t f, size_t i) { return x[i]->ell == x[f]->ell; },
                      [&](const std::vector<size_t>& idx) {
        const size_t first = idx[0];
        const int B = (int)idx.size(), ell = x[first]->ell;
        const size_t pn = (size_t)ell * N;
        const std::vector<CtPtr> d = tensor_products(x, y, idx);
        AffineItems items;
        std::vector<CtPtr> adj(B);
        std::map<std::pair<const Ciphertext*, long double>, CtPtr> adjusted;
        std::vector<u64> cst((size_t)B * ell, 0);
        for (int k = 0; k < B; ++k) {
            const size_t i = idx[k];
            const AffineSpec& sp = spec[i];
            const long double sc = x[i]->scale * y[i]->scale;
            if (sp.f == 2) items.f2 |= 1u << k;
            if (sp.addend) {
                const CtPtr& ad = sp.addend;
                const std::pair<const Ciphertext*, long double> key{ad.get(), sc};
                auto hit = ad->deg == 1 ? adjusted.find(key) : adjusted.end();
                if (hit != adjusted.end()) {
                    adj[k] = hit->second;
                } else {
// ... 421 lines not shown
```

fhe-linformer_amd/csrc/evaluator.h:

```cpp
#pragma once
#include <cmath>
#include <functional>
#include <map>
#include <memory>
#include <vector>
#include "context.h"
#include "kernels_elem.h"

namespace fhelin {

struct DevBlock {
    Context* ctx = nullptr;
    u64* d = nullptr;
    ~DevBlock();
};

struct Ciphertext {
    Context* ctx = nullptr;
    u64* d = nullptr;
    std::shared_ptr<DevBlock> block;
    int npoly = 2;
    int ell = 0;
    int deg = 1;
    long double scale = 0;
// ... 39 lines not shown
    std::shared_ptr<Plaintext> shared;
    static constexpr size_t MAX_SHARED_ENCODINGS = 64;
    bool fixed = false;
};
typedef std::shared_ptr<Plaintext> PtPtr;

struct EvalKey {
    Context* ctx = nullptr;
    u64* d = nullptr;
    mutable u64* d_perm = nullptr;
    int digits = 0;
    bool seeded = false;
    ~EvalKey();
    size_t words() const { return (size_t)digits * 2 * (ctx->L + 1 + ctx->K) * ctx->N; }
};
typedef std::shared_ptr<EvalKey> KeyPtr;

inline bool same_scale(const Ciphertext& a, const Ciphertext& b) { return fabsl(b.scale / a.scale - 1.0L) < 1e-9L; }
inline bool same_shape(const Ciphertext& a, const Ciphertext& b) {
    return a.npoly == 2 && b.npoly == 2 && a.ell == b.ell && a.deg == b.deg && same_scale(a, b);
}

void real_to_scalars(const Context& c, long double v, int ell, ScalarSet& sc);

class Evaluator {
public:
    explicit Evaluator(Context& c) : c_(c) {}
    Context& ctx() { return c_; }

    CtPtr new_ct(int npoly, int ell, int deg, long double scale, int slots);
    std::vector<CtPtr> new_ct_batch(int count, int npoly, int ell, int deg, long double scale, int slots);
    static u64* contiguous_base(const std::vector<CtPtr>& v);
    std::vector<CtPtr> make_contiguous(const std::vector<CtPtr>& v, int site = -1);
    u64 gather_copies[8] = {};
    bool dot_groups = true;
    bool cheb_leaf_at_product = true;
    bool cheb_leaf_classes = true;
    bool cheb_rounds = true;
    bool adjust_items = true;
    int batch_limit = 32;
    CtPtr clone(const CtPtr& a);
    KeyPtr new_key();

    std::map<u64, KeyPtr> rot_keys;
    KeyPtr relin_key;
    KeyPtr conj_key;

    void keyswitch(const u64* c_ntt, int ell, const EvalKey& key, u64* out, const u64* add0, const u64* add1, const u32* map,
                   const u64* post = nullptr);
    void keyswitch_batch(int batch, const u64* c_ntt, size_t c_stride, int ell, const EvalKey& key, u64* out, size_t out_stride,
                         const u64* add0, const u64* add1, size_t add_stride, const u32* map, const u64* post, size_t post_stride);
    struct KsRows {
        std::vector<const EvalKey*> keys;
        std::vector<const u32*> maps;
        bool shared_input = false;
    };
    void keyswitch_rows(const KsRows& rows, const u64* c_ntt, size_t c_stride, int ell, u64* out, size_t out_stride, const u64* add0,
                        size_t add_stride);
    std::vector<CtPtr> rotate_sum_batch(const std::vector<CtPtr>& v, const std::vector<int>& indices);
    bool have_rotation_keys(const std::vector<int>& indices, int slots) const;
    const u64* permuted(const EvalKey& key, const u32* map);
    CtPtr rotate_each_sum(const std::vector<CtPtr>& v, const std::vector<int>& indices);
    std::vector<CtPtr> rotate_each_sum_rows(const std::vector<std::vector<CtPtr>>& rows, const std::vector<int>& indices);
    std::vector<CtPtr> hoisted_dot_rows(const std::vector<CtPtr>& xs, const std::vector<PtPtr>& pts, const std::vector<int>& indices,
                                        bool rescale_out = false);
    std::vector<CtPtr> linear_transform_rows(const std::vector<CtPtr>& xs, const std::vector<std::vector<PtPtr>>& pts,
                                             const std::vector<int>& baby, const std::vector<int>& giant, bool rescale_out = false);
    bool merged_products = false;
    bool merged_rescale = true;
    bool double_hoist = true;
    struct FoldedKey {
        PtPtr pt;
        KeyPtr key;
        int index = 0;
        long double scale = 0;
        std::shared_ptr<Encoding> enc;
        std::shared_ptr<DevBlock> d;
    };
    std::vector<FoldedKey> folded_keys;
    static constexpr size_t MAX_FOLDED = 12;
    FoldedKey folded_key(const PtPtr& p, int index, long double scale);
    std::vector<CtPtr> rotate_many(const CtPtr& a, const std::vector<int>& indices);
    std::vector<std::vector<CtPtr>> rotate_many_batch(const std::vector<CtPtr>& xs, const std::vector<int>& indices);
    std::vector<CtPtr> rotate_galois_batch(const std::vector<CtPtr>& v, u64 galois, const EvalKey& key, bool accumulate);
    std::vector<CtPtr> conjugate_batch(const std::vector<CtPtr>& v);
    std::vector<CtPtr> raw_modraise_batch(const std::vector<CtPtr>& v, int new_ell);
    std::vector<CtPtr> rotate_each(const std::vector<CtPtr>& v, const std::vector<int>& indices);
    std::vector<CtPtr> rotate_add_batch(const std::vector<CtPtr>& v, int index);
    std::vector<CtPtr> rotate_batch(const std::vector<CtPtr>& v, int index);
    std::vector<CtPtr> rotate_batch_impl(const std::vector<CtPtr>& v, int index, bool accumulate);
    std::vector<CtPtr> mult_plain_batch(const std::vector<CtPtr>& v, const PtPtr& p);
    std::vector<CtPtr> mult_plain_each(const std::vector<CtPtr>& v, const std::vector<PtPtr>& p);
    bool dot_plain_groups(const std::vector<CtPtr>& cts, const std::vector<std::vector<PtPtr>>& pts, long double pt_scale,
                          const std::vector<CtPtr>& dest);
    bool dot_plain_cyclic(const std::vector<CtPtr>& cts, const std::vector<PtPtr>& pts, const std::vector<CtPtr>& dest);
    bool dot_plain_window(const std::vector<CtPtr>& cur, const std::vector<CtPtr>& prev, const std::vector<PtPtr>& pts,
                          const std::vector<CtPtr>& dest, bool accumulate);
    bool dot_plain_groups_batch(const std::vector<std::vector<CtPtr>>& cts, const std::vector<std::vector<PtPtr>>& pts, long double pt_scale,
                                const std::vector<std::vector<CtPtr>>& dest);
    CtPtr dot_plain(const std::vector<CtPtr>& v, const std::vector<PtPtr>& p, long double pt_scale = 0,
                    const CtPtr& dest = CtPtr());
    std::vector<CtPtr> add_batch(const std::vector<CtPtr>& a, const std::vector<CtPtr>& b);
    std::vector<CtPtr> add_plain_batch(const std::vector<CtPtr>& v, const PtPtr& p);
    std::vector<CtPtr> sub_batch(const std::vector<CtPtr>& a, const std::vector<CtPtr>& b);
    std::vector<CtPtr> mult_batch(const std::vector<CtPtr>& a, const std::vector<CtPtr>& b);
    std::vector<CtPtr> mult_affine_rescale_batch(const std::vector<CtPtr>& a, const std::vector<CtPtr>& b, int f, double cadd,
                                                 const std::vector<CtPtr>& sub);
    struct AffineSpec {
        int f = 1;
        double cadd = 0;
        CtPtr addend;
        bool negate = false;
    };
    bool exact_products = true;
    bool exact_products_on() const { return exact_products && c_.K >= 1 && c_.K + 1 <= 16; }
    std::vector<CtPtr> mult_affine_batch(const std::vector<CtPtr>& a, const std::vector<CtPtr>& b, const std::vector<AffineSpec>& spec);
    std::vector<CtPtr> eval_chebyshev_many(const std::vector<CtPtr>& xs, const std::vector<double>& coeffs, double a, double b);
    std::vector<CtPtr> rescale_batch(const std::vector<CtPtr>& v);

    CtPtr add(const CtPtr& a, const CtPtr& b);
    CtPtr sub(const CtPtr& a, const CtPtr& b);
    CtPtr negate(const CtPtr& a);
    CtPtr add_plain(const CtPtr& a, const PtPtr& p);
    CtPtr mult_plain(const CtPtr& a, const PtPtr& p);
    CtPtr mult(const CtPtr& a, const CtPtr& b);
    CtPtr mult_no_relin(const CtPtr& a, const CtPtr& b);
    CtPtr relinearize(const CtPtr& a);
    CtPtr mult_int(const CtPtr& a, u64 k, bool raise_deg, long double new_scale, int keep_ell = 0);
    std::vector<CtPtr> adjust_deg1_batch(const std::vector<CtPtr>& v, int ell, long double scale);
    std::vector<CtPtr> adjust_deg1_batch(const std::vector<CtPtr>& v, int ell, const std::vector<long double>& scales);
    std::vector<CtPtr> scaled_diff_batch(const std::vector<CtPtr>& u, const std::vector<CtPtr>& w, const std::vector<u128>& a,
                                         const std::vector<u128>& c, bool raise_deg, const std::vector<long double>& scales);
    CtPtr mult_real(const CtPtr& a, double c);
    CtPtr add_real(const CtPtr& a, double c);
    CtPtr lincomb(const std::vector<CtPtr>& terms, const std::vector<double>& coef, double c0);
    CtPtr lincomb_at(const std::vector<CtPtr>& terms, const std::vector<double>& coef, double c0, long double want_scale, int keep_ell);
    CtPtr rotate(const CtPtr& a, int index);
    CtPtr conjugate(const CtPtr& a);
    CtPtr eval_poly(const CtPtr& x, const std::vector<double>& coeffs);
    CtPtr eval_chebyshev(const CtPtr& x, const std::vector<double>& coeffs, double a, double b);
    CtPtr mult_many(const std::vector<CtPtr>& v);
    std::vector<CtPtr> eval_poly_many(const std::vector<CtPtr>& xs, const std::vector<double>& coeffs);
    std::vector<CtPtr> mult_many_rows(const std::vector<std::vector<CtPtr>>& vs);
    CtPtr rescale(const CtPtr& a);
    CtPtr level_reduce(const CtPtr& a, int new_ell);
    CtPtr adjust(const CtPtr& a, int ell, int deg, long double scale);

    CtPtr raw_rescale(const CtPtr& a);
    void lift_and_ntt(u64* lifted, const u64* last, int P, int ell, const NttEpilogue* ep = nullptr, const u64* qlm_row = nullptr);
    void rescale_finish(u64* out, const u64* c, const u64* last, int P, int ell, const u64* qlinv_row = nullptr, const u64* qlm_row = nullptr);
    CtPtr raw_rotate(const CtPtr& a, u64 galois, const EvalKey& key, bool accumulate = false, const u32* map = nullptr);
    CtPtr rotate_add(const CtPtr& a, int index);
    CtPtr raw_mult_relin(const CtPtr& a, const CtPtr& b, const EvalKey& key);
    CtPtr raw_modraise(const CtPtr& a, int new_ell);

private:
    Context& c_;
    void keyswitch_impl(int batch, const KsRows* rows, const u64* c_ntt, size_t c_stride, int ell, const EvalKey* key, u64* out,
                        size_t out_stride, const u64* add0, const u64* add1, size_t add_stride, const u32* map, const u64* post,
                        size_t post_stride);
    Scratch<u64> modup(const KsShape& up, const u64* src, bool times_r2, int group2 = 0, size_t group2_stride = 0);
    void moddown(const KsShape& sh, const u64* accQ, u64* accP, u64* out, const u64* add0, const u64* add1, const u32* map, const u64* post,
                 bool row_pass = false, const std::function<void(const u64* conv)>& finish = nullptr);
    void moddown_rescale(const KsShape& sh, const u64* accQ, u64* accP, u64* out);
    void moddown_rescale_exact(const KsShape& sh, const u64* accQ, u64* accP, u64* out, u32 f2);
    int slot_count(int slots) const;
    int slot_count(const CtPtr& a) const { return slot_count(a->slots); }
    struct RotKey {
        const KeyPtr& key;
        const u32* map;
        u64 g;
    };
    RotKey rotation_key(int index);
    struct Rotations {
        int n = 0;
        const EvalKey* key[KsShape::MAX_ROT] = {};
        const u32* map[KsShape::MAX_ROT] = {};
        bool tiles_in_place = true;
    };
    Rotations rotations(const int* indices, int n);
    void set_rotations(KsShape& sh, const Rotations& rot, bool shared_digits, const u64* const* keys = nullptr);
    void rotation_sum(KsShape& sh, const u64* ext, const u64* c1, const u64* c0, size_t c0_stride, u64* out, const u64* post);
    void rescale_degree2(std::vector<CtPtr>& a, std::vector<CtPtr>* b = nullptr, const char* two_components = nullptr);
    std::vector<CtPtr> tensor_products(const std::vector<CtPtr>& x, const std::vector<CtPtr>& y, const std::vector<size_t>& idx);
    void product_operands(const std::vector<CtPtr>& a, const std::vector<CtPtr>& b, std::vector<CtPtr>& x, std::vector<CtPtr>& y);
    std::vector<CtPtr> mult_affine_unmerged(const std::vector<CtPtr>& a, const std::vector<CtPtr>& b, const std::vector<AffineSpec>& spec);
    bool sum_in_row_pass() const { return c_.fuse_finish && c_.rot_gather; }
    bool rot_in_gather() const { return c_.fuse_finish && c_.rot_gather && !c_.fuse_moddown; }
    void moddown_rescale_finish(const KsShape& sh, u64* out, const u64* accQ, u64* conv, const u64* minv);
    typedef std::vector<CtPtr> CtRow;
    CtRow cheb_recurse(const std::vector<double>& c, const std::vector<CtRow>& T, const std::map<int, CtRow>& G, int baby);
    std::vector<CtPtr> add_sub_batch(const std::vector<CtPtr>& a, const std::vector<CtPtr>& b, int op);
    void match(const CtPtr& a, const CtPtr& b, CtPtr& ao, CtPtr& bo);
    void match_batch(const std::vector<CtPtr>& a, const std::vector<CtPtr>& b, std::vector<CtPtr>& x, std::vector<CtPtr>& y);
};

}
```

fhe-linformer_amd/csrc/kernels_elem.h:

```cpp
#pragma once
#include "kernels.h"

namespace fhelin {

struct ScalarSet {
    u64 v[128];
};

void launch_ew_mul(const DeviceTables& t, u64* out, const u64* a, const u64* b, int nvec, int b_mod, int limb_first, int limb_count, hipStream_t s);
void launch_ew_add(const DeviceTables& t, u64* out, const u64* a, const u64* b, int nvec, int b_mod, int limb_first, int limb_count, hipStream_t s);
void launch_ew_sub(const DeviceTables& t, u64* out, const u64* a, const u64* b, int nvec, int b_mod, int limb_first, int limb_count, hipStream_t s);
void launch_ew_muladd(const DeviceTables& t, u64* out, const u64* acc, const u64* a, const u64* b, int nvec, int b_mod, int limb_first,
                      int limb_count, hipStream_t s);
void launch_ew_neg(const DeviceTables& t, u64* out, const u64* a, int nvec, int limb_first, int limb_count, hipStream_t s);
void launch_ew_scalar(const DeviceTables& t, u64* out, const u64* a, const ScalarSet& sc, int nvec, int limb_first, int limb_count, hipStream_t s,
                      int in_limbs = 0);
void launch_ew_addscalar(const DeviceTables& t, u64* out, const u64* a, const ScalarSet& sc, int nvec, int limb_first, int limb_count, hipStream_t s,
                         int add_vecs = -1);
struct LinComb {
    static constexpr int MAX_TERMS = 32;
    int n = 0;
    int vecs = 0;
    const u64* a[MAX_TERMS];
};
// ... 33 lines not shown
    static constexpr int MAX_ITEMS = 32;
    int n = 0;
    int vecs = 0;
    int ell = 0;
    u64* out[MAX_ITEMS];
    const u64* u[MAX_ITEMS];
    const u64* w[MAX_ITEMS];
};
void launch_ew_scaled_diff(const DeviceTables& t, const EwScaledDiff& d, const u64* consts, hipStream_t s);
struct EwScalarItems {
    static constexpr int MAX_ITEMS = EwItems::MAX_ITEMS;
    int n = 0;
    int npoly = 0;
    int ell = 0;
    int in_limbs[MAX_ITEMS];
    const u64* a[MAX_ITEMS];
};
void launch_ew_scalar_items(const DeviceTables& t, const EwScalarItems& d, u64* out, const u64* consts, hipStream_t s);
void launch_ew_dot(const DeviceTables& t, u64* out, const EwItems& it, int limb_count, hipStream_t s);
struct EwDotGroups {
    static constexpr int MAX_A = 16, MAX_G = 8;
    int na = 0, ng = 0, ell = 0;
    const u64* a[MAX_A];
    const u64* p[MAX_G][MAX_A];
    u64* out[MAX_G];
    int nbatch = 1;
    size_t a_stride[MAX_A] = {};
    size_t out_stride[MAX_G] = {};
    u32 pmask[MAX_G] = {};
};
void launch_ew_dot_groups(const DeviceTables& t, const EwDotGroups& d, hipStream_t s);
struct EwCyclic {
    static constexpr int PERIOD = 32;
    int n = 0, ell = 0;
    const u64* a[PERIOD];
    const u64* m[PERIOD];
    u64* out[PERIOD];
};
void launch_ew_cyclic_dot(const DeviceTables& t, const EwCyclic& d, hipStream_t s);
struct EwWindow {
    static constexpr int W = 32;
    int ell = 0, accumulate = 0;
    u32 cur_mask = 0, prev_mask = 0;
    const u64* cur[W];
    const u64* prev[W];
    const u64* m[W];
    u64* out[W];
};
void launch_ew_window_dot(const DeviceTables& t, const EwWindow& d, hipStream_t s);

struct KsShape {
    int ell;
    int k;
    int alpha;
    int beta;
    int L1;
    int batch = 1;
    size_t c_stride = 0;
    size_t out_stride = 0;
    size_t add_stride = 0;
    size_t post_stride = 0;
    static constexpr int MAX_ROWS = 16;
    int per_row = 0;
    int shared_input = 0;
    int row_mod = 0;
    const u64* evk_row[MAX_ROWS] = {};
    const u32* map_row[MAX_ROWS] = {};
    static constexpr int MAX_ROT = 7;
    int n_rot = 0;
    const u64* evk_rot[MAX_ROT] = {};
    const u32* map_rot[MAX_ROT] = {};
    size_t rot_ext_stride = 0;
    size_t rot_input_stride = 0;
    int lds_digits = 0;
    size_t ext_batch_stride = 0;
    const u64* gsrc = nullptr;
    size_t gsrc_stride = 0;
    const u64* gsrc_pmod = nullptr;
    int gather = 0;
    u32 ginv = 0;
    u32 ginv_row[MAX_ROWS] = {};
    int tch = 16;
    int accp_limbs = 0;
};
void launch_modup_conv(const DeviceTables& t, const KsShape& sh, u64* ext, const u64* cc, const u64* c_ntt, const u64* hatinv,
                       const u64* hatmod, hipStream_t s);
void launch_ks_inner(const DeviceTables& t, const KsShape& sh, u64* accQ, u64* accP, const u64* ext, const u64* evk, const u64* c_ntt,
                     hipStream_t s);
void launch_ks_inner_multi(const DeviceTables& t, const KsShape& sh, u64* accQ, u64* accP, const u64* ext, const u64* c_ntt,
                           hipStream_t s);
void launch_fold_key(const DeviceTables& t, u64* out, const u64* key, const u32* map, const u64* V, int nvec, hipStream_t s);
struct HoistAdd {
    int n_rot = 0;
    const u64* v[KsShape::MAX_ROT + 1] = {};
    const u32* map[KsShape::MAX_ROT] = {};
    u64* acc = nullptr;
    const u64* pmod = nullptr;
};
void launch_hoist_addends(const DeviceTables& t, const KsShape& sh, const HoistAdd& h, u64* pre, const u64* ct, hipStream_t s);
struct LtStep {
    static constexpr int MAX_G = 4;
    const u64* key;
    const u32* map;
    const u64* v[MAX_G];
    u32 mask;
    u32 pad;
};
struct LtDot {
    static constexpr int MAX_STEPS = 32;
    const LtStep* steps = nullptr;
    int n_steps = 0;
    int n_groups = 0;
    int g0 = 0, groups = 0;
    const u64* pmod = nullptr;
};
void launch_ks_inner_dot(const DeviceTables& t, const KsShape& sh, const LtDot& ld, u64* accQ, u64* accP, const u64* ext, const u64* c0,
                         const u64* c1, hipStream_t s);
void launch_moddown_conv(const DeviceTables& t, const KsShape& sh, u64* conv, const u64* accP, const u64* phatinv, const u64* phatmod,
                         hipStream_t s);
void launch_affine_acc(const DeviceTables& t, const KsShape& sh, u64* accQ, const u64* d, const u64* sub, const ScalarSet& cst, int has_cst, int f,
                       const u64* pmod, hipStream_t s);
void launch_moddown_rescale_conv(const DeviceTables& t, const KsShape& sh, u64* conv, const u64* accP, const u64* top, const u64* hatinv,
                                 const u64* hatmod, const u64* mmod, hipStream_t s);
void launch_moddown_rescale_finish(const DeviceTables& t, const KsShape& sh, u64* out, const u64* accQ, const u64* conv, const u64* minv,
                                   hipStream_t s);
struct AffineItems {
    static constexpr int MAX_ITEMS = 32;
    const u64* add[MAX_ITEMS] = {};
    u32 f2 = 0, neg = 0, cst = 0;
};
void launch_affine_acc_items(const DeviceTables& t, const KsShape& sh, const AffineItems& it, u64* accQ, u64* accP, const u64* d,
                             const u64* consts, const u64* pmod, hipStream_t s);
void launch_moddown_rescale_exact_conv(const DeviceTables& t, const KsShape& sh, u32 f2, u64* conv, const u64* accP, const u64* phatinv,
                                       const u64* phatmod, const u64* pinv, const u64* pmod, const u64* qlm, hipStream_t s);
void launch_moddown_finish(const DeviceTables& t, const KsShape& sh, u64* out, const u64* accQ, const u64* conv, const u64* pinv,
                           const u64* add0, const u64* add1, const u32* map, const u64* post, hipStream_t s);

}
```

fhe-linformer_amd/csrc/kernels_ks.hip:

```cpp
#include <hip/hip_runtime.h>
#include <cstdlib>
#include "kernels.h"
#include "kernels_elem.h"

namespace fhelin {
namespace {

typedef u64 u64x2 __attribute__((ext_vector_type(2)));

__device__ __forceinline__ Barrett load_barrett(const DeviceTables& t, int limb) {
    Barrett b;
    b.q = t.moduli[limb];
    b.r0 = t.barrett[2 * limb];
    b.r1 = t.barrett[2 * limb + 1];
    return b;
}

constexpr int TCH = 16;

template <int MAXA, bool FULL>
__device__ __forceinline__ void modup_body(const DeviceTables& t, const KsShape& sh, u64* __restrict__ ext, const u64* __restrict__ cc,
                                           const u64* __restrict__ hatinv, const u64* __restrict__ hatmod, int j, int lo, int cnt, size_t n) {
    const size_t N = (size_t)1 << t.log_n;
    const int nt = sh.ell + sh.k;
// ... 808 lines not shown
    const u64 q = t.moduli[tt];
    const u64 w = minv[2 * tt], ws = minv[2 * tt + 1];
    const size_t row = ((size_t)1 << t.log_n) >> 1;
    const size_t n2 = (size_t)blockIdx.x * 256 + threadIdx.x;
    const u64x2 a = reinterpret_cast<const u64x2*>(accQ)[(((size_t)bi * 2 + c) * sh.ell + tt) * row + n2];
    const u64x2 b = reinterpret_cast<const u64x2*>(conv)[(((size_t)bi * 2 + c) * e1 + tt) * row + n2];
    u64x2 r;
    r.x = mul_shoup(sub_mod(a.x, b.x, q), w, ws, q);
    r.y = mul_shoup(sub_mod(a.y, b.y, q), w, ws, q);
    reinterpret_cast<u64x2*>(out + (size_t)bi * sh.out_stride)[(size_t)v * row + n2] = r;
}

}

void launch_fold_key(const DeviceTables& t, u64* out, const u64* key, const u32* map, const u64* V, int nvec, hipStream_t s) {
    hipLaunchKernelGGL(fold_key_kernel, dim3((1u << t.log_n) / 512, (unsigned)nvec), dim3(256), 0, s, t, out, key, map, V);
}
void launch_hoist_addends(const DeviceTables& t, const KsShape& sh, const HoistAdd& h, u64* pre, const u64* ct, hipStream_t s) {
    hipLaunchKernelGGL(hoist_addends_kernel, dim3((1u << t.log_n) / 512, (unsigned)(sh.batch * 2 * sh.ell)), dim3(256), 0, s, t, sh, h, pre, ct);
}

void launch_affine_acc(const DeviceTables& t, const KsShape& sh, u64* accQ, const u64* d, const u64* sub, const ScalarSet& cst, int has_cst, int f,
                       const u64* pmod, hipStream_t s) {
    hipLaunchKernelGGL(affine_acc_kernel, dim3((1u << t.log_n) / 512, (unsigned)(sh.batch * 2 * sh.ell)), dim3(256), 0, s, t, sh, accQ, d, sub, cst,
                       has_cst, f, pmod);
}
static int conv_tch(unsigned planes, int targets) {
    static const int force = [] {
        const char* e = std::getenv("FHELIN_CONV_CHUNKS");
        return e ? std::atoi(e) : 0;
    }();
    if (force || planes < 2048u) return TCH;
    return targets > TCH ? targets : TCH;
}
void launch_moddown_rescale_conv(const DeviceTables& t, const KsShape& sh_in, u64* conv, const u64* accP, const u64* top, const u64* hatinv,
                                 const u64* hatmod, const u64* mmod, hipStream_t s) {
    KsShape sh = sh_in;
    const unsigned nx = (1u << t.log_n) / 256;
    sh.tch = conv_tch(nx * (unsigned)(sh.batch * 2), sh.ell - 1);
    dim3 g(nx, (unsigned)(sh.batch * 2), (unsigned)((sh.ell - 1 + sh.tch - 1) / sh.tch));
    hipLaunchKernelGGL(moddown_rescale_conv_kernel, g, dim3(256), 0, s, t, sh, conv, accP, top, hatinv, hatmod, mmod);
}
void launch_affine_acc_items(const DeviceTables& t, const KsShape& sh, const AffineItems& it, u64* accQ, u64* accP, const u64* d,
                             const u64* consts, const u64* pmod, hipStream_t s) {
    dim3 g((1u << t.log_n) / 512, (unsigned)(sh.batch * 2 * sh.ell));
    hipLaunchKernelGGL(affine_acc_items_kernel, g, dim3(256), 0, s, t, sh, it, accQ, accP, d, consts, pmod);
}
void launch_moddown_rescale_exact_conv(const DeviceTables& t, const KsShape& sh_in, u32 f2, u64* conv, const u64* accP, const u64* phatinv,
                                       const u64* phatmod, const u64* pinv, const u64* pmod, const u64* qlm, hipStream_t s) {
    KsShape sh = sh_in;
    const unsigned nx = (1u << t.log_n) / 256;
    sh.tch = conv_tch(nx * (unsigned)(sh.batch * 2), sh.ell - 1);
    dim3 g(nx, (unsigned)(sh.batch * 2), (unsigned)((sh.ell - 1 + sh.tch - 1) / sh.tch));
#define FHELIN_MDX_CASE(K) case K: hipLaunchKernelGGL((moddown_rescale_exact_conv_kernel<K>), g, dim3(256), 0, s, t, sh, f2, conv, accP, phatinv, phatmod, pinv, pmod, qlm); break;
    switch (sh.k) {
        FHELIN_MDX_CASE(1) FHELIN_MDX_CASE(2) FHELIN_MDX_CASE(3) FHELIN_MDX_CASE(4)
        FHELIN_MDX_CASE(5) FHELIN_MDX_CASE(6) FHELIN_MDX_CASE(7) FHELIN_MDX_CASE(8)
        default: hipLaunchKernelGGL((moddown_rescale_exact_conv_kernel<16>), g, dim3(256), 0, s, t, sh, f2, conv, accP, phatinv, phatmod, pinv, pmod, qlm); break;
    }
#undef FHELIN_MDX_CASE
}
void launch_moddown_rescale_finish(const DeviceTables& t, const KsShape& sh, u64* out, const u64* accQ, const u64* conv, const u64* minv,
                                   hipStream_t s) {
    dim3 g((1u << t.log_n) / 512, (unsigned)(sh.batch * 2 * (sh.ell - 1)));
    hipLaunchKernelGGL(moddown_rescale_finish_kernel, g, dim3(256), 0, s, t, sh, out, accQ, conv, minv);
}

void launch_modup_conv(const DeviceTables& t, const KsShape& sh_in, u64* ext, const u64* cc, const u64* c_ntt, const u64* hatinv,
                       const u64* hatmod, hipStream_t s) {
    KsShape sh = sh_in;
    const unsigned nx = (1u << t.log_n) / 256;
    sh.tch = conv_tch(nx * (unsigned)(sh.batch * sh.beta), sh.ell + sh.k);
    dim3 g(nx, (unsigned)(sh.batch * sh.beta), (unsigned)((sh.ell + sh.k + sh.tch - 1) / sh.tch));
#define FHELIN_MODUP_CASE(A) case A: hipLaunchKernelGGL((modup_conv_kernel<A>), g, dim3(256), 0, s, t, sh, ext, cc, c_ntt, hatinv, hatmod); break;
    switch (sh.alpha) {
        FHELIN_MODUP_CASE(1) FHELIN_MODUP_CASE(2) FHELIN_MODUP_CASE(3) FHELIN_MODUP_CASE(4)
        FHELIN_MODUP_CASE(5) FHELIN_MODUP_CASE(6) FHELIN_MODUP_CASE(7) FHELIN_MODUP_CASE(8)
        default: hipLaunchKernelGGL((modup_conv_kernel<16>), g, dim3(256), 0, s, t, sh, ext, cc, c_ntt, hatinv, hatmod); break;
    }
#undef FHELIN_MODUP_CASE
}
void launch_ks_inner(const DeviceTables& t, const KsShape& sh, u64* accQ, u64* accP, const u64* ext, const u64* evk, const u64* c_ntt,
                     hipStream_t s) {
    dim3 g((1u << t.log_n) / 512, (unsigned)(sh.batch * (sh.ell + sh.k)));
    if (sh.gather)
        hipLaunchKernelGGL(ks_inner_kernel<true>, g, dim3(256), 0, s, t, sh, accQ, accP, ext, evk, c_ntt);
    else
        hipLaunchKernelGGL(ks_inner_kernel<false>, g, dim3(256), 0, s, t, sh, accQ, accP, ext, evk, c_ntt);
}
void launch_ks_inner_multi(const DeviceTables& t, const KsShape& sh, u64* accQ, u64* accP, const u64* ext, const u64* c_ntt,
                           hipStream_t s) {
    static const int pair_rows = [] { const char* e = std::getenv("FHELIN_KS_ROW_PAIRS"); return e ? std::atoi(e) : 1; }();
    const bool stage = sh.lds_digits && sh.rot_ext_stride == 0 && sh.beta <= 4;
    if (pair_rows && sh.batch >= 2) {
        dim3 g((1u << t.log_n) / 512, (unsigned)(((sh.batch + 1) / 2) * (sh.ell + sh.k)));
        if (stage)
            hipLaunchKernelGGL((ks_inner_multi_kernel<true, 2>), g, dim3(256), 0, s, t, sh, accQ, accP, ext, c_ntt);
        else
            hipLaunchKernelGGL((ks_inner_multi_kernel<false, 2>), g, dim3(256), 0, s, t, sh, accQ, accP, ext, c_ntt);
        return;
    }
    dim3 g((1u << t.log_n) / 512, (unsigned)(sh.batch * (sh.ell + sh.k)));
    if (stage)
        hipLaunchKernelGGL((ks_inner_multi_kernel<true, 1>), g, dim3(256), 0, s, t, sh, accQ, accP, ext, c_ntt);
    else
        hipLaunchKernelGGL((ks_inner_multi_kernel<false, 1>), g, dim3(256), 0, s, t, sh, accQ, accP, ext, c_ntt);
}
void launch_ks_inner_dot(const DeviceTables& t, const KsShape& sh, const LtDot& ld, u64* accQ, u64* accP, const u64* ext, const u64* c0,
                         const u64* c1, hipStream_t s) {
    dim3 g((1u << t.log_n) / 512, (unsigned)(sh.batch * (sh.ell + sh.k)));
    if (ld.n_groups == 1)
        hipLaunchKernelGGL(ks_inner_dot_kernel<1>, g, dim3(256), 0, s, t, sh, ld, accQ, accP, ext, c0, c1);
    else if (ld.n_groups == 2)
        hipLaunchKernelGGL(ks_inner_dot_kernel<2>, g, dim3(256), 0, s, t, sh, ld, accQ, accP, ext, c0, c1);
    else
        hipLaunchKernelGGL((ks_inner_dot_kernel<LtStep::MAX_G>), g, dim3(256), 0, s, t, sh, ld, accQ, accP, ext, c0, c1);
}
void launch_moddown_conv(const DeviceTables& t, const KsShape& sh_in, u64* conv, const u64* accP, const u64* phatinv, const u64* phatmod,
                         hipStream_t s) {
    KsShape sh = sh_in;
    const unsigned nx = (1u << t.log_n) / 256;
    sh.tch = conv_tch(nx * (unsigned)(2 * sh.batch), sh.ell);
    dim3 g(nx, (unsigned)(2 * sh.batch), (unsigned)((sh.ell + sh.tch - 1) / sh.tch));
#define FHELIN_MODDOWN_CASE(K, S) case K: hipLaunchKernelGGL((moddown_conv_kernel<K, S>), g, dim3(256), 0, s, t, sh, conv, accP, phatinv, phatmod); break;
#define FHELIN_MODDOWN_SWITCH(S)                                                                                                                \
    switch (sh.k) {                                                                                                                             \
        FHELIN_MODDOWN_CASE(1, S) FHELIN_MODDOWN_CASE(2, S) FHELIN_MODDOWN_CASE(3, S) FHELIN_MODDOWN_CASE(4, S)                                 \
        FHELIN_MODDOWN_CASE(5, S) FHELIN_MODDOWN_CASE(6, S) FHELIN_MODDOWN_CASE(7, S) FHELIN_MODDOWN_CASE(8, S)                                 \
        default: hipLaunchKernelGGL((moddown_conv_kernel<16, S>), g, dim3(256), 0, s, t, sh, conv, accP, phatinv, phatmod); break;              \
    }
    if (sh.gather) {
        FHELIN_MODDOWN_SWITCH(true)
    } else {
        FHELIN_MODDOWN_SWITCH(false)
    }
#undef FHELIN_MODDOWN_SWITCH
#undef FHELIN_MODDOWN_CASE
}
void launch_moddown_finish(const DeviceTables& t, const KsShape& sh, u64* out, const u64* accQ, const u64* conv, const u64* pinv,
                           const u64* add0, const u64* add1, const u32* map, const u64* post, hipStream_t s) {
    dim3 g((1u << t.log_n) / 512, (unsigned)(sh.batch * 2 * sh.ell));
    hipLaunchKernelGGL(moddown_finish_kernel, g, dim3(256), 0, s, t, sh, out, accQ, conv, pinv, add0, add1, map, post);
}

}
```

fhe-linformer_amd/csrc/kernels_ntt.hip:

```cpp
#include <hip/hip_runtime.h>
#include <algorithm>
#include <cstdlib>
#include "kernels.h"

namespace fhelin {

namespace {

struct NttArgs {
    u64* data;
    const u64* src;
    const u64* tw;
    const u64* tw_rows;
    const u64* moduli;
    const u64* ninv;
    const int* limb_tab;
    int tab_len;
    int limb_first;
    int limb_count;
    int log_n;
    int nvec;
    int period;
    int lazy_out;
    int src_group;
    size_t src_group_stride;
    int src_group2;
    size_t src_group2_stride;
    const u64* lift_qlm;
    int lift_limb;
    int vec0;
};

__device__ __forceinline__ size_t src_offset(const NttArgs& a, int vec, int log_n) {
    if (a.src_group > 0) {
        const int g = vec / a.src_group;
        const size_t in = (size_t)(vec % a.src_group) << log_n;
        if (a.src_group2 > 0) return (size_t)(g / a.src_group2) * a.src_group2_stride + (size_t)(g % a.src_group2) * a.src_group_stride + in;
        return (size_t)g * a.src_group_stride + in;
    }
    return (size_t)vec << log_n;
}

constexpr int TILE = 4096;
constexpr int LDS_WORDS = TILE + TILE / 16;

__device__ __forceinline__ constexpr int tile_index(int tau, int k, int p) {
    return ((tau >> p) << (p + 4)) | (k << p) | (tau & ((1 << p) - 1));
}
__device__ __forceinline__ constexpr int lds_slot(int e) { return e + (e >> 4); }

__device__ __forceinline__ int limb_of(const NttArgs& a, int vec) {
    return a.limb_tab ? a.limb_tab[a.tab_len ? vec % a.tab_len : vec] : a.limb_first + (vec % a.limb_count);
}

typedef u64 u64x2 __attribute__((ext_vector_type(2)));

__device__ __forceinline__ int uniform(int v) { return __builtin_amdgcn_readfirstlane(v); }
typedef u32 u32x2 __attribute__((ext_vector_type(2)));
typedef u32 u32x4 __attribute__((ext_vector_type(4)));
struct Stream {
    __amdgpu_buffer_rsrc_t r;
};
__device__ __forceinline__ Stream stream(const void* ubase) {
    const u64 v = reinterpret_cast<u64>(ubase);
    const u32 lo = __builtin_amdgcn_readfirstlane((u32)v), hi = __builtin_amdgcn_readfirstlane((u32)(v >> 32));
    Stream s;
    s.r = __builtin_amdgcn_make_buffer_rsrc(reinterpret_cast<void*>(((u64)hi << 32) | lo), 0, 0xffffffff, 0x00020000);
    return s;
}
__device__ __forceinline__ u32 ld32(const Stream& s, u32 lane, int K, int soff = 0) {
    return __builtin_amdgcn_raw_buffer_load_b32(s.r, lane + (K & 4095), soff + (K & ~4095), 0);
}
__device__ __forceinline__ u64 ld64(const Stream& s, u32 lane, int K, int soff = 0) {
    const u32x2 v = __builtin_amdgcn_raw_buffer_load_b64(s.r, lane + (K & 4095), soff + (K & ~4095), 0);
    return ((u64)v.y << 32) | v.x;
}
__device__ __forceinline__ u64x2 ld128(const Stream& s, u32 lane, int K, int soff = 0) {
    const u32x4 v = __builtin_amdgcn_raw_buffer_load_b128(s.r, lane + (K & 4095), soff + (K & ~4095), 0);
    u64x2 r;
    r.x = ((u64)v.y << 32) | v.x;
    r.y = ((u64)v.w << 32) | v.z;
    return r;
}
__device__ __forceinline__ void st64(const Stream& s, u32 lane, int K, u64 x, int soff = 0) {
    u32x2 v;
    v.x = (u32)x;
// ... 146 lines not shown
    if (!INVERSE) {
        constexpr int P0 = LOGCW + A - 4;
        const u32 lane_in = goff(tile_index(tau, 0, P0));
#pragma unroll
        for (int k = 0; k < 16; ++k) x[k] = ld64(sbase, lane_in, goff(tile_index(0, k, P0)));
        if constexpr (LIFT) {
            const u64 half = a.moduli[a.lift_limb] >> 1, qlm = a.lift_qlm[limb];
#pragma unroll
            for (int k = 0; k < 16; ++k) {
                const u64 r = csub_mask(x[k], c.q);
                x[k] = x[k] > half ? sub_mod(r, qlm, c.q) : r;
            }
        }
        RoundTw rt, rn;
        load_round_tw<0, 4>(rt, tw, LOGN, 8 + P0 - LOGCW, 0, tau >> P0);
        fwd_round<0, 4, LAZY>(x, rt, c);
        int p_prev = P0;
        if constexpr (NFULL >= 2) {
            constexpr int P1 = LOGCW + A - 8;
            load_round_tw<0, 4>(rn, tw, LOGN, 8 + P1 - LOGCW, 0, tau >> P1);
            exchange(x, lds, tau, p_prev, P1, false);
            fwd_round<0, 4, LAZY>(x, rn, c);
            p_prev = P1;
        }
        if constexpr (REM > 0) {
            constexpr int PR = LOGCW;
            load_round_tw<0, REM>(rt, tw, LOGN, 8, 0, tau >> PR);
            exchange(x, lds, tau, p_prev, PR, NFULL >= 2);
            fwd_round<0, REM, LAZY>(x, rt, c);
            p_prev = PR;
        }
        constexpr int PL = REM > 0 ? LOGCW : (NFULL >= 2 ? LOGCW + A - 8 : P0);
        (void)p_prev;
        const u32 lane_out = goff(tile_index(tau, 0, PL));
#pragma unroll
        for (int k = 0; k < 16; ++k) st64(base, lane_out, goff(tile_index(0, k, PL)), x[k]);
    } else {
        const u64* ninv = a.ninv + 8 * limb;
        constexpr int P0 = LOGCW;
        const u32 lane_in = goff(tile_index(tau, 0, P0));
#pragma unroll
        for (int k = 0; k < 16; ++k) x[k] = ld64(sbase, lane_in, goff(tile_index(0, k, P0)));
        RoundTw rt, rn;
        load_round_tw<0, 4>(rt, tw, LOGN, 8, 0, tau >> P0);
        inv_round<0, 4, (NFULL == 1 && REM == 0), LAZY, 0, 2>(x, rt, c, ninv);
        int p_prev = P0;
        if constexpr (NFULL >= 2) {
            constexpr int P1 = LOGCW + 4;
            load_round_tw<0, 4>(rn, tw, LOGN, 8 + 4, 0, tau >> P1);
            exchange(x, lds, tau, p_prev, P1, false);
            inv_round<0, 4, (REM == 0), LAZY, 4, 2>(x, rn, c, ninv);
            p_prev = P1;
        }
        if constexpr (REM > 0) {
            constexpr int PR = 8;
            load_round_tw<4 - REM, 4>(rt, tw, LOGN, 8 + PR - LOGCW, 0, tau >> PR);
            exchange(x, lds, tau, p_prev, PR, NFULL >= 2);
            inv_round<4 - REM, 4, true, LAZY, 4 * NFULL, 2>(x, rt, c, ninv);
            p_prev = PR;
        }
        constexpr int PL = REM > 0 ? 8 : (NFULL >= 2 ? LOGCW + 4 : P0);
        (void)p_prev;
        const u32 lane_out = goff(tile_index(tau, 0, PL));
#pragma unroll
        for (int k = 0; k < 16; ++k) st64(base, lane_out, goff(tile_index(0, k, PL)), x[k]);
    }
}

template <int A, bool INVERSE, bool LIFT = false>
__global__ __launch_bounds__(256) __attribute__((amdgpu_waves_per_eu(LIFT ? 3 : 4))) void ntt_cols_kernel(NttArgs a) {
    constexpr int LOGTILES = A - 4;
    __shared__ u64 lds[LDS_WORDS];
    const int vec = a.vec0 + (blockIdx.x >> LOGTILES);
    const int tile = blockIdx.x & ((1 << LOGTILES) - 1);
    const int limb = uniform(limb_of(a, vec));
    if (limb < 0) return;
    const LimbConst c = limb_const(a, limb);
    if (lazy_prime<INVERSE>(c.q))
        cols_body<A, INVERSE, true, LIFT>(a, lds, vec, tile, limb, c);
    else
        cols_body<A, INVERSE, false, LIFT>(a, lds, vec, tile, limb, c);
}

template <bool INVERSE, bool LAZY, bool EPI>
__device__ __forceinline__ void rows_body(const NttArgs& a, u64* lds, int vec, int tile, int limb, const LimbConst& c,
                                          const NttEpilogue* ep) {
    const int log_n = a.log_n;
    const Stream tw = stream(reinterpret_cast<const u64x2*>(a.tw) + ((size_t)limb << log_n));
    const Stream trows = stream(reinterpret_cast<const u64x2*>(a.tw_rows) + (((size_t)limb << (log_n - 12)) + tile) * (15 * 256));
    [[maybe_unused]] u64* const vbase = a.data + ((size_t)vec << log_n) + ((size_t)tile << 12);
    const Stream base = stream(vbase);
    const Stream sbase = stream(a.src + src_offset(a, vec, log_n) + ((size_t)tile << 12));
    const int tau = threadIdx.x;
    const u32 lane4 = 8u * (u32)tile_index(tau, 0, 4), lane8 = 8u * (u32)tile_index(tau, 0, 8);
    auto koff = [](int k, int p) constexpr { return 8 * tile_index(0, k, p); };
    u64 x[16];

    if (!INVERSE) {
#pragma unroll
        for (int k = 0; k < 16; ++k) x[k] = ld64(sbase, lane4, koff(k, 4));
        RoundTw rt, rn;
        load_round_tw<0, 4>(rt, tw, log_n, 4, tile << 4, tau >> 4);
        fwd_round<0, 4, LAZY>(x, rt, c);
        load_round_tw_rows(rn, trows, tau);
        exchange(x, lds, tau, 4, 0, false);
        fwd_round<0, 4, LAZY>(x, rn, c);
        [[maybe_unused]] u64 av[16];
        [[maybe_unused]] int ell = 0, t = 0, poly = 0;
        if constexpr (EPI) {
            ell = ep->ell;
            poly = uniform(vec / ell);
            t = vec - poly * ell;
            const Stream acc = stream(ep->acc + (size_t)poly * ep->acc_poly_stride + ((size_t)t << log_n) + ((size_t)tile << 12));
#pragma unroll
            for (int k = 0; k < 16; ++k) av[k] = ld64(acc, lane8, koff(k, 8));
        }
        [[maybe_unused]] u64 epi_b = 0;
        if constexpr (EPI) {
            if (LAZY) {
                epi_b = 86 * c.q;
            } else if (c.q < (1ull << 60)) {
                epi_b = 10 * c.q;
            } else {
                epi_b = 2 * c.q;
#pragma unroll
                for (int k = 0; k < 16; ++k) x[k] = reduce_lazy_2q(x[k], c.q, c.sh, c.rr);
            }
        } else if (!(LAZY && a.lazy_out && c.q < (1ull << 53))) {
#pragma unroll
            for (int k = 0; k < 16; ++k)
                x[k] = csub_mask(reduce_lazy_2q(x[k], c.q, c.sh, c.rr), c.q);
        }
#if defined(FHELIN_ROWS_DIRECT_STORE)
        if constexpr (!EPI) {
#pragma unroll
            for (int k = 0; k < 16; k += 2) {
                u64x2 v;
                v.x = x[k];
                v.y = x[k + 1];
                reinterpret_cast<u64x2*>(vbase + 16 * tau)[k >> 1] = v;
            }
            return;
        }
#endif
        exchange(x, lds, tau, 0, 8, true);
        if constexpr (EPI) {
            const int bi = poly >> 1, comp = poly & 1;
            const size_t n = (size_t)1 << log_n;
            const u64 w = ep->w[2 * t], ws = ep->w[2 * t + 1];
#pragma unroll
            for (int k = 0; k < 16; ++k) x[k] = mul_shoup(av[k] + epi_b - x[k], w, ws, c.q);
            const u64* add = comp == 0 ? ep->add0 : ep->add1;
            if (add) {
                const Stream adds = stream(add + (size_t)bi * ep->add_stride + (size_t)t * n + ((size_t)tile << 12));
#pragma unroll
                for (int k = 0; k < 16; ++k) x[k] = add_mod(x[k], ld64(adds, lane8, koff(k, 8)), c.q);
            }
            const size_t row_off = (size_t)(comp * ell + t) * n;
            const bool has_post = ep->post != nullptr;
            const Stream post = stream(ep->post + (has_post ? (size_t)bi * ep->post_stride + row_off : 0));
            const Stream out = stream(ep->out + (size_t)bi * ep->out_stride + row_off);
            const int toff = tile << 15;
            const u32* im = ep->per_row ? ep->invmap_row[bi] : ep->invmap;
            if (im) {
                const Stream ims = stream(im + ((size_t)tile << 12));
#pragma unroll
                for (int k = 0; k < 16; ++k) {
                    const u32 j8 = 8u * ld32(ims, 4u * (u32)tau, 4 * tile_index(0, k, 8));
                    u64 r = x[k];
                    if (has_post) r = add_mod(r, ld64(post, j8, 0), c.q);
                    st64(out, j8, 0, r);
                }
            } else {
                if (has_post) {
#pragma unroll
                    for (int k = 0; k < 16; ++k) x[k] = add_mod(x[k], ld64(post, lane8, koff(k, 8), toff), c.q);
                }
#pragma unroll
                for (int k = 0; k < 16; ++k) st64(out, lane8, koff(k, 8), x[k], toff);
            }
        } else {
#pragma unroll
            for (int k = 0; k < 16; ++k) st64(base, lane8, koff(k, 8), x[k]);
        }
    } else {
#pragma unroll
        for (int k = 0; k < 16; ++k) x[k] = ld64(sbase, lane8, koff(k, 8));
        RoundTw rt, rn;
        load_round_tw_rows(rt, trows, tau);
        exchange(x, lds, tau, 8, 0, false);
        inv_round<0, 4, false, LAZY, 0, 1>(x, rt, c, nullptr);
        load_round_tw<0, 4>(rn, tw, log_n, 4, tile << 4, tau >> 4);
        exchange(x, lds, tau, 0, 4, true);
        inv_round<0, 4, false, LAZY, 4, 1>(x, rn, c, nullptr);
        if (LAZY) {
#pragma unroll
            for (int k = 0; k < 16; ++k) x[k] = reduce_lazy_2q(x[k], c.q, c.sh, c.rr);
        }
#pragma unroll
        for (int k = 0; k < 16; ++k) st64(base, lane4, koff(k, 4), x[k]);
    }
}

template <bool INVERSE, bool EPI = false>
__global__ __launch_bounds__(256) __attribute__((amdgpu_waves_per_eu(4))) void ntt_rows_kernel(NttArgs a, NttEpilogue ep) {
    __shared__ u64 lds[LDS_WORDS];
    const int logtiles = a.log_n - 12;
    int lid = blockIdx.x;
    const int nblk = gridDim.x;
    if ((nblk & 7) == 0) lid = (lid & 7) * (nblk >> 3) + (lid >> 3);
    int vec, tile;
    if (a.period > 0) {
        const int nper = a.nvec / a.period;
        const int rep = lid % nper, r = lid / nper;
        tile = r & ((1 << logtiles) - 1);
        vec = a.vec0 + rep * a.period + (r >> logtiles);
    } else {
        vec = a.vec0 + (lid >> logtiles);
        tile = lid & ((1 << logtiles) - 1);
    }
    vec = uniform(vec);
    tile = uniform(tile);
    const int limb = uniform(limb_of(a, vec));
    if (limb < 0) return;
    const LimbConst c = limb_const(a, limb);
    if (lazy_prime<INVERSE>(c.q))
        rows_body<INVERSE, true, EPI>(a, lds, vec, tile, limb, c, &ep);
    else
        rows_body<INVERSE, false, EPI>(a, lds, vec, tile, limb, c, &ep);
}

template <int A>
void launch_cols(const NttArgs& a, bool inverse, int blocks, hipStream_t s) {
    if (inverse)
        hipLaunchKernelGGL((ntt_cols_kernel<A, true>), dim3(blocks), dim3(256), 0, s, a);
    else if (a.lift_qlm)
        hipLaunchKernelGGL((ntt_cols_kernel<A, false, true>), dim3(blocks), dim3(256), 0, s, a);
    else
        hipLaunchKernelGGL((ntt_cols_kernel<A, false>), dim3(blocks), dim3(256), 0, s, a);
}

}

static void launch_ntt_impl(const DeviceTables& t, const LimbBatch& b, bool inverse, const NttEpilogue* ep, hipStream_t s);

void launch_ntt(const DeviceTables& t, const LimbBatch& b, bool inverse, hipStream_t s) { launch_ntt_impl(t, b, inverse, nullptr, s); }
void launch_ntt_epilogue(const DeviceTables& t, const LimbBatch& b, const NttEpilogue& ep, hipStream_t s) {
    launch_ntt_impl(t, b, false, &ep, s);
}

static void launch_ntt_impl(const DeviceTables& t, const LimbBatch& b, bool inverse, const NttEpilogue* ep, hipStream_t s) {
    if (b.nvec <= 0) return;
    NttArgs a;
    a.data = b.data;
    a.src = b.src ? b.src : b.data;
    a.src_group = b.src ? b.src_group : 0;
    a.src_group_stride = b.src_group_stride;
    a.src_group2 = (b.src && b.src_group > 0) ? b.src_group2 : 0;
    a.src_group2_stride = b.src_group2_stride;
    a.lazy_out = (!inverse && b.lazy_out) ? 1 : 0;
    a.lift_qlm = (!inverse && b.src && b.lift_limb >= 0) ? b.lift_qlm : nullptr;
    a.lift_limb = b.lift_limb;
    a.tw = inverse ? t.tw_inv : t.tw_fwd;
    a.tw_rows = inverse ? t.tw_rows_inv : t.tw_rows_fwd;
    a.moduli = t.moduli;
    a.ninv = t.ninv;
    a.limb_tab = b.limb_tab;
    a.tab_len = b.tab_len;
    a.limb_first = b.limb_first;
    a.limb_count = b.limb_count > 0 ? b.limb_count : 1;
    a.log_n = t.log_n;
    a.nvec = b.nvec;
    const int per = b.limb_tab ? b.tab_len : a.limb_count;
    a.period = (per > 0 && per < b.nvec && b.nvec % per == 0) ? per : 0;
    const int A = t.log_n - 8;
    a.vec0 = 0;
    static const int chunk_mb = [] {
        const char* e = std::getenv("FHELIN_NTT_CHUNK_MB");
        return e ? std::atoi(e) : 0;
    }();
    int chunk = b.nvec;
    if (chunk_mb > 0 && !ep) {
        const size_t vec_bytes = (size_t)8 << t.log_n;
        const int want = (int)std::max<size_t>(1, ((size_t)chunk_mb << 20) / vec_bytes);
        if (b.nvec > want + want / 2) {
            const int per = a.period > 0 ? a.period : 1;
            chunk = std::max(per, want / per * per);
        }
    }
    const int nvec_all = b.nvec, period_all = a.period;
    const u64* src_all = a.src;
    const int sg = a.src_group, sg2 = a.src_group2;
    for (int v0 = 0; v0 < nvec_all; v0 += chunk) {
        a.vec0 = v0;
        a.nvec = std::min(chunk, nvec_all - v0);
        a.period = (period_all > 0 && a.nvec % period_all == 0 && a.nvec > period_all) ? period_all : 0;
        a.src = src_all;
        a.src_group = sg;
        a.src_group2 = sg2;
        const int blocks = a.nvec << (t.log_n - 12);
        auto cols = [&]() {
            switch (A) {
                case 4: launch_cols<4>(a, inverse, blocks, s); break;
                case 5: launch_cols<5>(a, inverse, blocks, s); break;
                case 6: launch_cols<6>(a, inverse, blocks, s); break;
                case 7: launch_cols<7>(a, inverse, blocks, s); break;
                case 8: launch_cols<8>(a, inverse, blocks, s); break;
                case 9: launch_cols<9>(a, inverse, blocks, s); break;
                default: break;
            }
        };
        if (!inverse) {
            cols();
            a.src = a.data;
            a.src_group = 0;
            a.src_group2 = 0;
            if (ep)
                hipLaunchKernelGGL((ntt_rows_kernel<false, true>), dim3(blocks), dim3(256), 0, s, a, *ep);
            else
                hipLaunchKernelGGL((ntt_rows_kernel<false, false>), dim3(blocks), dim3(256), 0, s, a, NttEpilogue());
        } else {
            hipLaunchKernelGGL((ntt_rows_kernel<true, false>), dim3(blocks), dim3(256), 0, s, a, NttEpilogue());
            a.src = a.data;
            a.src_group = 0;
            a.src_group2 = 0;
            cols();
        }
    }
}

}
```

include/fhelin.h:

```cpp
#ifndef FHELIN_H
#define FHELIN_H

#include <stddef.h>
#include <stdint.h>

#ifdef __cplusplus
extern "C" {
#endif

#define FHELIN_OK 0
#define FHELIN_ERR_ARG 1
#define FHELIN_ERR_NO_DEVICE 2
#define FHELIN_ERR_HIP 3
#define FHELIN_ERR_STATE 4
#define FHELIN_ERR_KEY 5
#define FHELIN_ERR_INTERNAL 6

typedef struct fhelin_ctx fhelin_ctx;
typedef struct fhelin_ct fhelin_ct;
typedef struct fhelin_pt fhelin_pt;

typedef struct fhelin_params {
    int32_t log_n;
    int32_t n_q;
// ... 57 lines not shown
int fhelin_gen_relin_key(fhelin_ctx* c);
int fhelin_gen_rotation_keys(fhelin_ctx* c, const int32_t* indices, int32_t n);
int fhelin_gen_conj_key(fhelin_ctx* c);
int fhelin_secret_export(fhelin_ctx* c, uint64_t* out, size_t cap_words);
int fhelin_secret_import(fhelin_ctx* c, const uint64_t* in, size_t words);
int fhelin_key_export(fhelin_ctx* c, int32_t kind, int32_t index, uint64_t* out, size_t cap_words);
int fhelin_key_import(fhelin_ctx* c, int32_t kind, int32_t index, const uint64_t* in, size_t words);

int fhelin_encode(fhelin_ctx* c, const double* vals, int32_t n, int32_t level, int32_t slots, fhelin_pt** out);
void fhelin_pt_free(fhelin_pt* p);
int fhelin_pt_export(fhelin_ctx* c, const fhelin_pt* p, int32_t ell, double scale_hi, double scale_lo, uint64_t* out,
                     size_t cap_words);

int fhelin_encrypt(fhelin_ctx* c, const fhelin_pt* p, fhelin_ct** out);
int fhelin_encrypt_batch(fhelin_ctx* c, const double* vals, int32_t n_vec, int32_t n_per, int32_t level, int32_t slots, fhelin_ct** outs);
int fhelin_client_ingest(fhelin_ctx* c, const double* emb, const int32_t* tokens, const double* table, int32_t vocab, int32_t S,
                         const double* cls, const double* pos, const double* E_w, const double* E_b, const double* F_w, const double* F_b,
                         int32_t w_cols, int32_t level, fhelin_ct** outs, double* proj_out);
int fhelin_ctx_set_host_encode(fhelin_ctx* c, int32_t on);
int fhelin_debug_sample(fhelin_ctx* c, int32_t kind, int32_t n_poly, int64_t* out, size_t cap);
int fhelin_decrypt(fhelin_ctx* c, const fhelin_ct* ct, double* out, int32_t slots);
int fhelin_ct_import(fhelin_ctx* c, const uint64_t* limbs, int32_t npoly, int32_t ell, int32_t deg, double scale,
                     int32_t slots, fhelin_ct** out);
int fhelin_ct_export(fhelin_ctx* c, const fhelin_ct* ct, uint64_t* out, size_t cap_words);
int fhelin_ct_export_device(fhelin_ctx* c, const fhelin_ct* ct, uint64_t* d_out, size_t cap_words);
int fhelin_ct_import_device(fhelin_ctx* c, const uint64_t* d_limbs, int32_t npoly, int32_t ell, int32_t deg, double scale_hi,
                            double scale_lo, int32_t slots, fhelin_ct** out);
int fhelin_ct_scale(const fhelin_ct* ct, double* scale_hi, double* scale_lo);
int fhelin_ct_info(const fhelin_ct* ct, int32_t* npoly, int32_t* ell, int32_t* level, int32_t* deg, double* scale,
                   int32_t* slots);
int fhelin_ct_clone(fhelin_ctx* c, const fhelin_ct* ct, fhelin_ct** out);
void fhelin_ct_free(fhelin_ct* ct);

int fhelin_add(fhelin_ctx* c, const fhelin_ct* a, const fhelin_ct* b, fhelin_ct** out);
int fhelin_sub(fhelin_ctx* c, const fhelin_ct* a, const fhelin_ct* b, fhelin_ct** out);
int fhelin_negate(fhelin_ctx* c, const fhelin_ct* a, fhelin_ct** out);
int fhelin_add_plain(fhelin_ctx* c, const fhelin_ct* a, const fhelin_pt* p, fhelin_ct** out);
int fhelin_mult_plain(fhelin_ctx* c, const fhelin_ct* a, const fhelin_pt* p, fhelin_ct** out);
int fhelin_mult(fhelin_ctx* c, const fhelin_ct* a, const fhelin_ct* b, fhelin_ct** out);
int fhelin_rotate(fhelin_ctx* c, const fhelin_ct* a, int32_t index, fhelin_ct** out);
int fhelin_rotate_many(fhelin_ctx* c, const fhelin_ct* a, const int32_t* indices, int32_t n, fhelin_ct** outs);
int fhelin_rotate_each(fhelin_ctx* c, const fhelin_ct* const* v, const int32_t* indices, int32_t n, fhelin_ct** outs);
int fhelin_rotate_sum(fhelin_ctx* c, const fhelin_ct* const* v, int32_t n, const int32_t* indices, int32_t n_rot, fhelin_ct** outs);
int fhelin_hoisted_dot(fhelin_ctx* c, const fhelin_ct* const* v, int32_t n, const fhelin_pt* const* pts, const int32_t* indices,
                       int32_t n_rot, int32_t rescale, fhelin_ct** outs);
int fhelin_rotate_each_sum(fhelin_ctx* c, const fhelin_ct* const* v, const int32_t* indices, int32_t n, fhelin_ct** out);
int fhelin_rescale(fhelin_ctx* c, const fhelin_ct* a, fhelin_ct** out);
int fhelin_rotate_batch(fhelin_ctx* c, const fhelin_ct* const* v, int32_t n, int32_t index, fhelin_ct** outs);
int fhelin_rescale_batch(fhelin_ctx* c, const fhelin_ct* const* v, int32_t n, fhelin_ct** outs);
int fhelin_mult_plain_batch(fhelin_ctx* c, const fhelin_ct* const* v, int32_t n, const fhelin_pt* p, fhelin_ct** outs);
int fhelin_mult_batch(fhelin_ctx* c, const fhelin_ct* const* a, const fhelin_ct* const* b, int32_t n, fhelin_ct** outs);
int fhelin_add_batch(fhelin_ctx* c, const fhelin_ct* const* a, const fhelin_ct* const* b, int32_t n, fhelin_ct** outs);
int fhelin_mult_affine_batch(fhelin_ctx* c, const fhelin_ct* const* a, const fhelin_ct* const* b, int32_t n, const int32_t* f, const double* cadd,
                             const fhelin_ct* const* addend, const int32_t* negate, fhelin_ct** outs);
int fhelin_level_reduce(fhelin_ctx* c, const fhelin_ct* a, int32_t new_ell, fhelin_ct** out);

typedef struct fhelin_lt fhelin_lt;
int fhelin_lt_create(fhelin_ctx* c, const double* diags , const int32_t* diag_idx, int32_t n_diag, int32_t slots,
                     int32_t n1 , fhelin_lt** out);
int fhelin_lt_create_pts(fhelin_ctx* c, const fhelin_pt* const* pts , const int32_t* baby ,
                         const int32_t* giant , int32_t n1, int32_t n2, fhelin_lt** out);
int fhelin_lt_info(const fhelin_lt* lt, int32_t* n1, int32_t* n2, int32_t* n_terms, int32_t* slots);
int fhelin_lt_rotations(const fhelin_lt* lt, int32_t* out, int32_t cap, int32_t* n);
int fhelin_lt_apply(fhelin_ctx* c, const fhelin_lt* lt, const fhelin_ct* const* v, int32_t n, int32_t rescale, fhelin_ct** outs);
void fhelin_lt_free(fhelin_lt* lt);

int fhelin_raw_rescale(fhelin_ctx* c, const fhelin_ct* a, fhelin_ct** out);
int fhelin_raw_rotate(fhelin_ctx* c, const fhelin_ct* a, int32_t index, fhelin_ct** out);
int fhelin_raw_mult_relin(fhelin_ctx* c, const fhelin_ct* a, const fhelin_ct* b, fhelin_ct** out);
int fhelin_raw_modraise(fhelin_ctx* c, const fhelin_ct* a, int32_t new_ell, fhelin_ct** out);
int fhelin_raw_phase(fhelin_ctx* c, const fhelin_ct* a, fhelin_ct** out);

int fhelin_debug_pt_from_residues(fhelin_ctx* c, const uint64_t* residues, int32_t ell, fhelin_pt** out);
int fhelin_debug_pt_from_residues_full(fhelin_ctx* c, const uint64_t* residues, double scale_hi, double scale_lo, fhelin_pt** out);
int fhelin_debug_dot_plain(fhelin_ctx* c, const fhelin_ct* const* cts, const fhelin_pt* const* pts, int32_t n, fhelin_ct** out);
int fhelin_debug_dot_groups(fhelin_ctx* c, const fhelin_ct* const* cts , int32_t nb, int32_t na,
                            const fhelin_pt* const* pts , int32_t ng, fhelin_ct** outs );
int fhelin_debug_dot_cyclic(fhelin_ctx* c, const fhelin_ct* const* cts, int32_t n, const fhelin_pt* const* pts ,
                            fhelin_ct** outs );
int fhelin_debug_dot_window(fhelin_ctx* c, const fhelin_ct* const* cur , const fhelin_ct* const* prev ,
                            const fhelin_pt* const* pts , fhelin_ct* const* dest , int32_t accumulate);
int fhelin_debug_rotate_many_batch(fhelin_ctx* c, const fhelin_ct* const* cts, int32_t n_ct, const int32_t* indices, int32_t n,
                                   fhelin_ct** outs );

int fhelin_fc_mult_const(fhelin_ctx* c, const fhelin_ct* a, double d, fhelin_ct** out);
int fhelin_fc_mask(fhelin_ctx* c, const fhelin_ct* a, int32_t kind, int32_t x, int32_t y, double v, fhelin_ct** out);
int fhelin_fc_rotsum(fhelin_ctx* c, const fhelin_ct* a, int32_t slots, int32_t padding, fhelin_ct** out);
int fhelin_fc_repeat(fhelin_ctx* c, const fhelin_ct* a, int32_t slots, int32_t padding, fhelin_ct** out);
int fhelin_fc_add_many(fhelin_ctx* c, const fhelin_ct* const* v, int32_t n, fhelin_ct** out);
int fhelin_fc_matmul_pt(fhelin_ctx* c, const fhelin_ct* const* rows, int32_t n, const fhelin_pt* w, const fhelin_pt* bias,
                        int32_t slots, int32_t padding, fhelin_ct** outs);
int fhelin_fc_matmul_ct(fhelin_ctx* c, const fhelin_ct* const* rows, int32_t n, const fhelin_ct* w, int32_t slots,
                        int32_t padding, fhelin_ct** outs);
int fhelin_fc_matmulRElarge(fhelin_ctx* c, const fhelin_ct* const* rows, int32_t n, const fhelin_pt* const* weights,
                            int32_t nw, const fhelin_pt* bias, double mask_val, fhelin_ct** outs);
int fhelin_fc_matmulCRlarge(fhelin_ctx* c, const fhelin_ct* const* rows, int32_t n, const fhelin_pt* const* weights,
                            const fhelin_pt* bias, fhelin_ct** outs);
int fhelin_fc_matmulScores(fhelin_ctx* c, const fhelin_ct* const* queries, int32_t n, const fhelin_ct* key, fhelin_ct** out);
int fhelin_fc_wrapUpRepeated(fhelin_ctx* c, const fhelin_ct* const* v, int32_t n, fhelin_ct** out);
int fhelin_fc_wrapUpExpanded(fhelin_ctx* c, const fhelin_ct* const* v, int32_t n, fhelin_ct** out);
int fhelin_fc_unwrapExpanded(fhelin_ctx* c, const fhelin_ct* a, int32_t inputs_num, fhelin_ct** outs);
int fhelin_fc_unwrapScoresExpanded(fhelin_ctx* c, const fhelin_ct* a, int32_t inputs_num, fhelin_ct** outs);
int fhelin_fc_unwrap_512_in_4_128(fhelin_ctx* c, const fhelin_ct* a, int32_t index, fhelin_ct** outs4);
int fhelin_fc_unwrapRepeatedLarge(fhelin_ctx* c, const fhelin_ct* const* containers, int32_t nc, int32_t input_number,
                                  fhelin_ct** outs);
int fhelin_fc_unwrapRepeatedLarge_range(fhelin_ctx* c, const fhelin_ct* const* containers, int32_t nc, int32_t input_number,
                                        int32_t first, int32_t count, fhelin_ct** outs);
int fhelin_fc_generate_containers(fhelin_ctx* c, const fhelin_ct* const* inputs, int32_t n, const fhelin_pt* bias,
                                  fhelin_ct** outs, int32_t* n_out);
int fhelin_fc_wrap_containers(fhelin_ctx* c, const fhelin_ct* const* v, int32_t n, int32_t inputs_number, fhelin_ct** out);

int fhelin_fcb_matmulScores(fhelin_ctx* c, const fhelin_ct* const* queries, int32_t n, const fhelin_ct* const* keys, int32_t B,
                            fhelin_ct** outs);
int fhelin_fcb_matmul_ct(fhelin_ctx* c, const fhelin_ct* const* rows, const fhelin_ct* const* ws, int32_t n, int32_t slots, int32_t padding,
                         fhelin_ct** outs);
int fhelin_fcb_wrapUpRepeated(fhelin_ctx* c, const fhelin_ct* const* v, int32_t n, int32_t B, fhelin_ct** outs);
int fhelin_fcb_wrapUpExpanded(fhelin_ctx* c, const fhelin_ct* const* v, int32_t n, int32_t B, fhelin_ct** outs);
int fhelin_fcb_unwrapExpanded(fhelin_ctx* c, const fhelin_ct* const* cs, int32_t B, int32_t inputs_num, fhelin_ct** outs);
int fhelin_fcb_unwrapRepeatedLarge(fhelin_ctx* c, const fhelin_ct* const* containers, int32_t nc, int32_t B, int32_t input_number,
                                   fhelin_ct** outs);
int fhelin_fcb_generate_containers(fhelin_ctx* c, const fhelin_ct* const* inputs, int32_t n, int32_t B, const fhelin_pt* bias,
                                   fhelin_ct** outs, int32_t* n_out);
int fhelin_fc_rotsum_batch(fhelin_ctx* c, const fhelin_ct* const* v, int32_t n, int32_t slots, int32_t padding, int32_t repeat, fhelin_ct** outs);
int fhelin_add_plain_batch(fhelin_ctx* c, const fhelin_ct* const* v, int32_t n, const fhelin_pt* p, fhelin_ct** outs);
int fhelin_eval_poly_batch(fhelin_ctx* c, const fhelin_ct* const* xs, int32_t n, const double* coeffs, int32_t n_coeffs, fhelin_ct** outs);
int fhelin_mult_many_batch(fhelin_ctx* c, const fhelin_ct* const* v, int32_t n, int32_t B, fhelin_ct** outs);

int fhelin_mult_real(fhelin_ctx* c, const fhelin_ct* a, double k, fhelin_ct** out);
int fhelin_add_real(fhelin_ctx* c, const fhelin_ct* a, double k, fhelin_ct** out);
int fhelin_mult_many(fhelin_ctx* c, const fhelin_ct* const* v, int32_t n, fhelin_ct** out);
int fhelin_lincomb(fhelin_ctx* c, const fhelin_ct* const* v, const double* coeffs, int32_t n, double c0, fhelin_ct** out);
int fhelin_eval_poly(fhelin_ctx* c, const fhelin_ct* x, const double* coeffs, int32_t n, fhelin_ct** out);
int fhelin_eval_chebyshev(fhelin_ctx* c, const fhelin_ct* x, const double* coeffs, int32_t n, double a, double b, fhelin_ct** out);
int fhelin_eval_chebyshev_batch(fhelin_ctx* c, const fhelin_ct* const* xs, int32_t n, const double* coeffs, int32_t n_coeffs, double a,
                                double b, fhelin_ct** outs);
int fhelin_bootstrap_setup(fhelin_ctx* c, int32_t level_budget_enc, int32_t level_budget_dec, int32_t slots);
int fhelin_bootstrap(fhelin_ctx* c, const fhelin_ct* a, fhelin_ct** out);
int fhelin_bootstrap_batch(fhelin_ctx* c, const fhelin_ct* const* v, int32_t n, fhelin_ct** outs);
int fhelin_bootstrap_config(fhelin_ctx* c, int32_t K, int32_t R, int32_t cheb_degree, int32_t correction);
int fhelin_bootstrap_partial(fhelin_ctx* c, const fhelin_ct* a, int32_t stage, fhelin_ct** out);
int fhelin_bootstrap_drop(fhelin_ctx* c, const fhelin_ct* a, int32_t drop, fhelin_ct** out);
int fhelin_bootstrap_iter(fhelin_ctx* c, const fhelin_ct* a, int32_t precision, fhelin_ct** out);
int fhelin_bootstrap_iter_batch(fhelin_ctx* c, const fhelin_ct* const* v, int32_t n, int32_t precision, fhelin_ct** outs);
int fhelin_bootstrap_iter_drop(fhelin_ctx* c, const fhelin_ct* a, int32_t precision, int32_t drop, fhelin_ct** out);
int fhelin_bootstrap_describe(fhelin_ctx* c, int32_t* out, int32_t cap, int32_t* n);
int fhelin_bootstrap_diag(fhelin_ctx* c, int32_t which, int32_t stage, int32_t term, fhelin_pt** out);
int fhelin_bootstrap_cheb(fhelin_ctx* c, double* out, int32_t cap, int32_t* n);

int fhelin_evalkeys_save(fhelin_ctx* c, const char* path);
int fhelin_evalkeys_params(const char* path, fhelin_params* out);
int fhelin_evalkeys_info(const char* path, int32_t* boot7, int32_t* n_keys);
int fhelin_evalkeys_load(fhelin_ctx* c, const char* path);
int fhelin_debug_key_digest(fhelin_ctx* c, const uint64_t* words, int32_t n_limbs, int32_t limb_first, uint64_t* out_digests,
                            int32_t* out_ok);

int fhelin_ctx_set_seeded_encryption(fhelin_ctx* c, int32_t on);
int fhelin_ct_compact_bytes(const fhelin_ct* ct, size_t* bytes);
int fhelin_ct_export_compact(fhelin_ctx* c, const fhelin_ct* ct, uint8_t* out, size_t cap_bytes);
int fhelin_compact_info(const uint8_t* blob, size_t bytes, int32_t* log_n, int32_t* ell, int32_t* deg, int32_t* slots);
int fhelin_ct_import_compact(fhelin_ctx* c, const uint8_t* const* blobs, const size_t* sizes, int32_t n, fhelin_ct** outs);
int fhelin_debug_seeded_expand(fhelin_ctx* c, const uint8_t* seed32, uint64_t nonce0, int32_t ell, int32_t n_ct, int32_t reps,
                               uint64_t* out, float* ms);

int fhelin_ctx_set_seeded_keys(fhelin_ctx* c, int32_t on);
int fhelin_ctx_key_set_seed(const fhelin_ctx* c, uint8_t* out32);
int fhelin_evalkeys_save_compact(fhelin_ctx* c, const char* path);
// ... 39 lines not shown
```

Baseline: 224.1.

## Fuse key-switch P-limb inner product into the inverse NTT row pass

Adds a fused kernel that computes the key-switch inner product for the special-prime (P) limbs directly into LDS and then runs the inverse NTT row pass on it. Only the column pass is left for moddown. The standard inner-product kernel now skips the P limbs when fusion is active. This removes a global write and read of accP plus a separate row-pass launch. The trade-off is a heavier kernel that may hurt occupancy, and it is gated by a heuristic (non-multi, beta<=8) plus env knobs. A debug entry point is added to check the fused accP result.

Result: faster. 221.6 (median of 6 runs) (-1.1%).

```diff
diff --git a/fhe-linformer_amd/capi.py b/fhe-linformer_amd/capi.py
--- a/fhe-linformer_amd/capi.py
+++ b/fhe-linformer_amd/capi.py
@@ -233,6 +233,7 @@
         "fhelin_debug_dot_cyclic": (i32, [vp, C.POINTER(vp), i32, C.POINTER(vp), C.POINTER(vp)]),
         "fhelin_debug_dot_window": (i32, [vp, C.POINTER(vp), C.POINTER(vp), C.POINTER(vp), C.POINTER(vp), i32]),
         "fhelin_debug_rotate_many_batch": (i32, [vp, C.POINTER(vp), i32, C.POINTER(i32), i32, C.POINTER(vp)]),
+        "fhelin_debug_ks_accp": (i32, [vp, vp, i32, i32, C.POINTER(i32), i32, vp]),
         "fhelin_ctx_set_interleave": (i32, [vp, i32]),
         "fhelin_ctx_interleave": (i32, [vp, C.POINTER(i32)]),
         "fhelin_evalkeys_interleave": (i32, [C.c_char_p, C.POINTER(i32)]),
@@ -1031,6 +1032,15 @@
         flat = self._cts(outs, len(cts) * n)
         return [flat[i * n:(i + 1) * n] for i in range(len(cts))]
 
+    def debug_ks_accp(self, digits, ell, indices=()):
+        d = np.ascontiguousarray(digits, dtype=np.uint64)
+        batch, n = d.shape[0], len(indices)
+        assert d.shape[2:] == (ell + self.n_p, self.N)
+        idx = (C.c_int32 * max(n, 1))(*indices)
+        out = np.empty((batch, 2, self.n_p, self.N), dtype=np.uint64)
+        self._ck(self.lib.fhelin_debug_ks_accp(self.h, d.ctypes.data_as(C.c_void_p), ell, batch, idx, n, out.ctypes.data_as(C.c_void_p)))
+        return out
+
     @staticmethod
     def _harr(objs):
         return (C.c_void_p * len(objs))(*[o.h for o in objs])
diff --git a/fhe-linformer_amd/csrc/capi_debug.cpp b/fhe-linformer_amd/csrc/capi_debug.cpp
--- a/fhe-linformer_amd/csrc/capi_debug.cpp
+++ b/fhe-linformer_amd/csrc/capi_debug.cpp
@@ -164,4 +164,24 @@
     FHELIN_CATCH
 }
 
+int fhelin_debug_ks_accp(fhelin_ctx* c, const uint64_t* digits, int32_t ell, int32_t batch, const int32_t* indices, int32_t n_rot,
+                         uint64_t* out) {
+    NEED(c && digits && out && (indices || n_rot == 0));
+    FHELIN_TRY
+    Context& x = c->ctx;
+    x.require_device();
+    if (ell < 1 || ell > x.L + 1 || batch < 1) throw Error(FHELIN_ERR_ARG, "debug_ks_accp: bad shape");
+    const size_t N = x.N;
+    const size_t nd = (size_t)batch * x.lvl[ell].beta * (ell + x.K) * N, no = (size_t)batch * 2 * x.K * N;
+    for (size_t i = 0; i < nd; ++i)
+        if (digits[i] >> 60) throw Error(FHELIN_ERR_ARG, "debug_ks_accp: a digit is not below 2^60");
+    Scratch<u64> ext = x.scratch<u64>(nd);
+    Scratch<u64> acc = x.scratch<u64>(no);
+    hip_check(hipMemcpyAsync(ext, digits, nd * 8, hipMemcpyHostToDevice, x.stream), "debug_ks_accp upload");
+    c->ev.debug_ks_accp(ext, ell, batch, indices, n_rot, acc);
+    hip_check(hipMemcpyAsync(out, acc, no * 8, hipMemcpyDeviceToHost, x.stream), "debug_ks_accp download");
+    x.sync();
+    FHELIN_CATCH
 }
+
+}
diff --git a/fhe-linformer_amd/csrc/context.cpp b/fhe-linformer_amd/csrc/context.cpp
--- a/fhe-linformer_amd/csrc/context.cpp
+++ b/fhe-linformer_amd/csrc/context.cpp
@@ -125,6 +125,8 @@
         if (const char* e = std::getenv("FHELIN_ROT_GATHER")) rot_gather = std::atoi(e) != 0;
         if (const char* e = std::getenv("FHELIN_FUSE_LIFT")) fuse_lift = std::atoi(e) != 0;
         if (const char* e = std::getenv("FHELIN_LDS_DIGITS")) lds_digits = std::atoi(e) != 0;
+        if (const char* e = std::getenv("FHELIN_FUSE_ACCP_ROWS")) fuse_accp_rows = std::atoi(e);
+        if (const char* e = std::getenv("FHELIN_ACCP_ROWS_MIN_VECS")) accp_rows_min_vecs = std::atoi(e);
         if (const char* e = std::getenv("FHELIN_NTT_TRACE")) trace_small_ntt = std::atoi(e);
         if (const char* e = std::getenv("FHELIN_SCALAR_TRACE")) trace_scalar = std::atoi(e);
         if (const char* e = std::getenv("FHELIN_HOST_WAITS")) trace_waits = std::atoi(e) != 0;
diff --git a/fhe-linformer_amd/csrc/context.h b/fhe-linformer_amd/csrc/context.h
--- a/fhe-linformer_amd/csrc/context.h
+++ b/fhe-linformer_amd/csrc/context.h
@@ -157,6 +157,8 @@
     bool device_decode = false;
     bool rot_gather = true;
     bool fuse_lift = true;
+    int fuse_accp_rows = 1;
+    int accp_rows_min_vecs = 0;
     bool lds_digits = true;
     struct FftDev {
         const u32* rot = nullptr;
diff --git a/fhe-linformer_amd/csrc/evaluator.cpp b/fhe-linformer_amd/csrc/evaluator.cpp
--- a/fhe-linformer_amd/csrc/evaluator.cpp
+++ b/fhe-linformer_amd/csrc/evaluator.cpp
@@ -221,7 +221,7 @@
     Scratch<u64> ext = modup(shu, c_ntt, !gather);
     Scratch<u64> accQ = c_.scratch<u64>((size_t)B * 2 * ell * N);
     Scratch<u64> accP = c_.scratch<u64>((size_t)B * 2 * K * N);
-    launch_ks_inner(c_.dt, sh, accQ, accP, ext, evk, c_ntt, c_.stream);
+    inner_product(sh, accQ, accP, ext, evk, c_ntt, false);
     if (gather) moddown(sh, accQ, accP, out, nullptr, nullptr, nullptr, post, true);
     else moddown(sh, accQ, accP, out, add0, add1, map, post, c_.fuse_moddown || (c_.fuse_finish && identity));
     launch_ok("keyswitch");
@@ -254,12 +254,35 @@
     return ext;
 }
 
+void Evaluator::inner_product(KsShape& sh, u64* accQ, u64* accP, const u64* ext, const u64* evk, const u64* c_ntt, bool multi, bool fuse) {
+    const int K = c_.K, nvec = sh.batch * 2 * K;
+    const bool measured_faster = !multi && sh.beta <= 8;
+    const bool want = c_.fuse_accp_rows >= 2 || (c_.fuse_accp_rows == 1 && measured_faster);
+    sh.accp_rows = fuse && want && !sh.accp_limbs && sh.k == K && nvec >= c_.accp_rows_min_vecs ? 1 : 0;
+    if (multi) launch_ks_inner_multi(c_.dt, sh, accQ, accP, ext, c_ntt, c_.stream);
+    else launch_ks_inner(c_.dt, sh, accQ, accP, ext, evk, c_ntt, c_.stream);
+    if (!sh.accp_rows) return;
+    NttProduct pr;
+    pr.sh = sh;
+    pr.ext = ext;
+    pr.evk = evk;
+    pr.multi = multi ? 1 : 0;
+    c_.stats.limb_ntt += (u64)nvec;
+    launch_ntt_rows_product(c_.dt, LimbBatch{accP, nvec, nullptr, c_.L + 1, K}, pr, c_.stream);
+}
+
+void Evaluator::accp_inverse(const KsShape& sh, u64* accP) {
+    const LimbBatch b{accP, sh.batch * 2 * c_.K, nullptr, c_.L + 1, c_.K};
+    if (sh.accp_rows) launch_ntt_cols_inverse(c_.dt, b, c_.stream);
+    else c_.ntt(b, true);
+}
+
 void Evaluator::moddown(const KsShape& sh, const u64* accQ, u64* accP, u64* out, const u64* add0, const u64* add1, const u32* map,
                         const u64* post, bool row_pass, const std::function<void(const u64* conv)>& finish) {
     const size_t N = c_.N;
-    const int B = sh.batch, ell = sh.ell, K = c_.K;
+    const int B = sh.batch, ell = sh.ell;
     if (row_pass && sh.gsrc && !sh.gsrc_pmod) throw Error(FHELIN_ERR_INTERNAL, "moddown: the row pass cannot gather");
-    c_.ntt(LimbBatch{accP, B * 2 * K, nullptr, c_.L + 1, K}, true);
+    accp_inverse(sh, accP);
     Scratch<u64> conv = c_.scratch<u64>((size_t)B * 2 * ell * N);
     launch_moddown_conv(c_.dt, sh, conv, accP, c_.d_phatinv, c_.d_phatmod, c_.stream);
     const LimbBatch cb{conv, B * 2 * ell, nullptr, 0, ell};
@@ -293,9 +316,9 @@
 
 void Evaluator::moddown_rescale(const KsShape& sh, const u64* accQ, u64* accP, u64* out) {
     const size_t N = c_.N;
-    const int B = sh.batch, ell = sh.ell, K = c_.K;
+    const int B = sh.batch, ell = sh.ell;
     const LevelTables& lt = c_.lvl[ell];
-    c_.ntt(LimbBatch{accP, B * 2 * K, nullptr, c_.L + 1, K}, true);
+    accp_inverse(sh, accP);
     Scratch<u64> top = c_.scratch<u64>((size_t)B * 2 * N);
     {
         LimbBatch tb{top, B * 2, nullptr, ell - 1, 1, accQ + (size_t)(ell - 1) * N};
@@ -370,8 +393,26 @@
     if (rp) sh.gsrc_pmod = c_.d_pmod;
     Scratch<u64> accQ = c_.scratch<u64>((size_t)sh.batch * 2 * sh.ell * N);
     Scratch<u64> accP = c_.scratch<u64>((size_t)sh.batch * 2 * sh.k * N);
-    launch_ks_inner_multi(c_.dt, sh, accQ, accP, ext, c1, c_.stream);
+    inner_product(sh, accQ, accP, ext, nullptr, c1, true);
     moddown(sh, accQ, accP, out, nullptr, nullptr, nullptr, post, rp);
+}
+
+void Evaluator::debug_ks_accp(const u64* ext, int ell, int batch, const int* indices, int n_rot, u64* out) {
+    const size_t N = c_.N, pn = (size_t)ell * N;
+    if (ell < 1 || ell > c_.L + 1 || batch < 1 || n_rot < 0 || n_rot > (int)KsShape::MAX_ROT) throw Error(FHELIN_ERR_ARG, "debug_ks_accp: bad shape");
+    if (!n_rot && !relin_key) throw Error(FHELIN_ERR_KEY, "debug_ks_accp: no relinearisation key");
+    KsShape sh{ell, c_.K, c_.alpha, c_.lvl[ell].beta, c_.L + 1, batch, pn, 0, 0, 0};
+    Scratch<u64> own = c_.scratch<u64>((size_t)batch * pn);
+    hip_check(hipMemsetAsync(own, 0, (size_t)batch * pn * sizeof(u64), c_.stream), "hipMemsetAsync(debug_ks_accp)");
+    Scratch<u64> accQ = c_.scratch<u64>((size_t)batch * 2 * pn);
+    if (n_rot) {
+        set_rotations(sh, rotations(indices, n_rot), true, nullptr);
+        inner_product(sh, accQ, out, ext, nullptr, own, true);
+    } else {
+        inner_product(sh, accQ, out, ext, relin_key->d, own, false);
+    }
+    accp_inverse(sh, out);
+    launch_ok("debug_ks_accp");
 }
 
 int Evaluator::slot_count(int slots) const { return slots > 0 ? slots : (1 << c_.prm.log_slots); }
@@ -538,7 +579,7 @@
             Scratch<u64> ext = modup(sh, base + pn, false);
             Scratch<u64> accQ = c_.scratch<u64>((size_t)B * 2 * ell * N);
             Scratch<u64> accP = c_.scratch<u64>((size_t)B * 2 * K * N);
-            launch_ks_inner_multi(c_.dt, sh, accQ, accP, ext, base + pn, s);
+            inner_product(sh, accQ, accP, ext, nullptr, base + pn, true);
             if (!merged) {
                 Scratch<u64> pre = c_.scratch<u64>((size_t)B * ctw);
                 launch_hoist_addends(c_.dt, sh, h, pre, base, s);
@@ -1065,7 +1106,7 @@
                 sh.gsrc = base;
                 sh.gsrc_stride = ctw;
                 sh.gsrc_pmod = c_.d_pmod;
-                launch_ks_inner(c_.dt, sh, accQ, accP, ext, nullptr, base + pn, s);
+                inner_product(sh, accQ, accP, ext, nullptr, base + pn, false);
                 moddown(sh, accQ, accP, o[0]->d, nullptr, nullptr, nullptr, nullptr, true);
             } else {
                 if (one_chunk) launch_ks_inner(c_.dt, row_shape(0, R), accQ, accP, ext, nullptr, base + pn, s);
@@ -1563,7 +1604,7 @@
             Scratch<u64> ext = modup(sh, c_ntt, true);
             Scratch<u64> accQ = c_.scratch<u64>((size_t)B * 2 * ell * N);
             Scratch<u64> accP = c_.scratch<u64>((size_t)B * 2 * K * N);
-            launch_ks_inner(c_.dt, sh, accQ, accP, ext, relin_key->d, c_ntt, s);
+            inner_product(sh, accQ, accP, ext, relin_key->d, c_ntt, false, f != 2);
             launch_affine_acc(c_.dt, sh, accQ, d[0]->d, sadj.empty() ? nullptr : sadj[0]->d, cst, cadd != 0.0 ? 1 : 0, f, c_.d_pmod, s);
             if (f == 2) launch_ew_add(c_.dt, accP, accP, accP, B * 2 * K, B * 2 * K, L1, K, s);
             moddown_rescale(sh, accQ, accP, o[0]->d);
diff --git a/fhe-linformer_amd/csrc/evaluator.h b/fhe-linformer_amd/csrc/evaluator.h
--- a/fhe-linformer_amd/csrc/evaluator.h
+++ b/fhe-linformer_amd/csrc/evaluator.h
@@ -145,6 +145,7 @@
     FoldedKey folded_key(const PtPtr& p, int index, long double scale);
     std::vector<CtPtr> rotate_many(const CtPtr& a, const std::vector<int>& indices);
     std::vector<std::vector<CtPtr>> rotate_many_batch(const std::vector<CtPtr>& xs, const std::vector<int>& indices);
+    void debug_ks_accp(const u64* ext, int ell, int batch, const int* indices, int n_rot, u64* out);
     std::vector<CtPtr> rotate_galois_batch(const std::vector<CtPtr>& v, u64 galois, const EvalKey& key, bool accumulate);
     std::vector<CtPtr> conjugate_batch(const std::vector<CtPtr>& v);
     std::vector<CtPtr> raw_modraise_batch(const std::vector<CtPtr>& v, int new_ell);
@@ -223,6 +224,8 @@
                         size_t out_stride, const u64* add0, const u64* add1, size_t add_stride, const u32* map, const u64* post,
                         size_t post_stride);
     Scratch<u64> modup(const KsShape& up, const u64* src, bool times_r2, int group2 = 0, size_t group2_stride = 0);
+    void inner_product(KsShape& sh, u64* accQ, u64* accP, const u64* ext, const u64* evk, const u64* c_ntt, bool multi, bool fuse = true);
+    void accp_inverse(const KsShape& sh, u64* accP);
     void moddown(const KsShape& sh, const u64* accQ, u64* accP, u64* out, const u64* add0, const u64* add1, const u32* map, const u64* post,
                  bool row_pass = false, const std::function<void(const u64* conv)>& finish = nullptr);
     void moddown_rescale(const KsShape& sh, const u64* accQ, u64* accP, u64* out);
diff --git a/fhe-linformer_amd/csrc/kernels_elem.h b/fhe-linformer_amd/csrc/kernels_elem.h
--- a/fhe-linformer_amd/csrc/kernels_elem.h
+++ b/fhe-linformer_amd/csrc/kernels_elem.h
@@ -139,7 +139,16 @@
     u32 ginv_row[MAX_ROWS] = {};
     int tch = 16;
     int accp_limbs = 0;
-};
+    int accp_rows = 0;
+};
+struct NttProduct {
+    KsShape sh;
+    const u64* ext = nullptr;
+    const u64* evk = nullptr;
+    int multi = 0;
+};
+void launch_ntt_rows_product(const DeviceTables& t, const LimbBatch& b, const NttProduct& p, hipStream_t s);
+void launch_ntt_cols_inverse(const DeviceTables& t, const LimbBatch& b, hipStream_t s);
 void launch_modup_conv(const DeviceTables& t, const KsShape& sh, u64* ext, const u64* cc, const u64* c_ntt, const u64* hatinv,
                        const u64* hatmod, hipStream_t s);
 void launch_ks_inner(const DeviceTables& t, const KsShape& sh, u64* accQ, u64* accP, const u64* ext, const u64* evk, const u64* c_ntt,
diff --git a/fhe-linformer_amd/csrc/kernels_ks.hip b/fhe-linformer_amd/csrc/kernels_ks.hip
--- a/fhe-linformer_amd/csrc/kernels_ks.hip
+++ b/fhe-linformer_amd/csrc/kernels_ks.hip
@@ -914,7 +914,7 @@
 }
 void launch_ks_inner(const DeviceTables& t, const KsShape& sh, u64* accQ, u64* accP, const u64* ext, const u64* evk, const u64* c_ntt,
                      hipStream_t s) {
-    dim3 g((1u << t.log_n) / 512, (unsigned)(sh.batch * (sh.ell + sh.k)));
+    dim3 g((1u << t.log_n) / 512, (unsigned)(sh.batch * (sh.accp_rows ? sh.ell : sh.ell + sh.k)));
     if (sh.gather)
         hipLaunchKernelGGL(ks_inner_kernel<true>, g, dim3(256), 0, s, t, sh, accQ, accP, ext, evk, c_ntt);
     else
@@ -924,15 +924,16 @@
                            hipStream_t s) {
     static const int pair_rows = [] { const char* e = std::getenv("FHELIN_KS_ROW_PAIRS"); return e ? std::atoi(e) : 1; }();
     const bool stage = sh.lds_digits && sh.rot_ext_stride == 0 && sh.beta <= 4;
+    const int nt = sh.accp_rows ? sh.ell : sh.ell + sh.k;
     if (pair_rows && sh.batch >= 2) {
-        dim3 g((1u << t.log_n) / 512, (unsigned)(((sh.batch + 1) / 2) * (sh.ell + sh.k)));
+        dim3 g((1u << t.log_n) / 512, (unsigned)(((sh.batch + 1) / 2) * nt));
         if (stage)
             hipLaunchKernelGGL((ks_inner_multi_kernel<true, 2>), g, dim3(256), 0, s, t, sh, accQ, accP, ext, c_ntt);
         else
             hipLaunchKernelGGL((ks_inner_multi_kernel<false, 2>), g, dim3(256), 0, s, t, sh, accQ, accP, ext, c_ntt);
         return;
     }
-    dim3 g((1u << t.log_n) / 512, (unsigned)(sh.batch * (sh.ell + sh.k)));
+    dim3 g((1u << t.log_n) / 512, (unsigned)(sh.batch * nt));
     if (stage)
         hipLaunchKernelGGL((ks_inner_multi_kernel<true, 1>), g, dim3(256), 0, s, t, sh, accQ, accP, ext, c_ntt);
     else
diff --git a/fhe-linformer_amd/csrc/kernels_ntt.hip b/fhe-linformer_amd/csrc/kernels_ntt.hip
--- a/fhe-linformer_amd/csrc/kernels_ntt.hip
+++ b/fhe-linformer_amd/csrc/kernels_ntt.hip
@@ -2,6 +2,7 @@
 #include <algorithm>
 #include <cstdlib>
 #include "kernels.h"
+#include "kernels_elem.h"
 
 namespace fhelin {
 
@@ -314,7 +315,113 @@
         cols_body<A, INVERSE, false, LIFT>(a, lds, vec, tile, limb, c);
 }
 
-template <bool INVERSE, bool LAZY, bool EPI>
+template <int PG, bool SHORT>
+__device__ __forceinline__ void product_to_lds(u64* lds, const NttArgs& a, const NttProduct& pr, const u64* __restrict__ barrett,
+                                               const u64* __restrict__ qinv, int vec, int tile, int limb, u64 q, int tau) {
+    const KsShape& sh = pr.sh;
+    const int log_n = a.log_n;
+    const int K = sh.k, nt = sh.ell + K;
+    const int poly = uniform(vec / K), p = vec - poly * K, bi = poly >> 1, comp = poly & 1;
+    const int tt = sh.ell + p;
+    const size_t N = (size_t)1 << log_n;
+    const u64* ext = pr.ext;
+    const u64* key0 = pr.evk;
+    const u32* map0 = nullptr;
+    int n_rot = 1;
+    if (pr.multi) {
+        ext += (size_t)bi * (sh.ext_batch_stride ? sh.ext_batch_stride : (size_t)sh.beta * nt * N);
+        n_rot = sh.n_rot;
+    } else {
+        int ri = 0;
+        if (sh.row_mod) {
+            ri = bi % sh.row_mod;
+            ext += (size_t)(bi / sh.row_mod) * sh.ext_batch_stride;
+            key0 = sh.evk_row[ri];
+        } else {
+            if (!sh.shared_input) ext += (size_t)bi * sh.beta * nt * N;
+            if (sh.per_row) {
+                ri = bi;
+                key0 = sh.evk_row[bi];
+            }
+        }
+        if (sh.gather) map0 = sh.map_row[ri];
+    }
+    const int khi = pr.multi || sh.gather ? 32 : 30;
+    Barrett br;
+    br.q = q;
+    br.r0 = barrett[2 * limb];
+    br.r1 = barrett[2 * limb + 1];
+    const u64 qi = qinv[limb];
+    const size_t kstride = (size_t)(sh.L1 + K) << log_n;
+    const size_t klimb = ((size_t)limb << log_n) + ((size_t)tile << 12);
+    const u32 lane8 = 8u * (u32)tau;
+    u64* const from = lds + lds_slot(tile_index(tau, 0, 8));
+#pragma unroll 1
+    for (int g = 0; g < 16; g += PG) {
+        u64 lo[PG], hi[PG];
+        Acc30 acc[PG];
+#pragma unroll
+        for (int i = 0; i < PG; ++i) {
+            lo[i] = hi[i] = 0;
+            acc[i] = Acc30{0, 0, 0};
+        }
+        int pending = 0, folded = 0;
+#pragma unroll 1
+        for (int r = 0; r < n_rot; ++r) {
+            const u32* map = pr.multi ? sh.map_rot[r] : map0;
+            const u64* key = pr.multi ? sh.evk_rot[r] : key0;
+            const u64* dig = ext + (size_t)r * sh.rot_ext_stride + ((size_t)tt << log_n);
+            u32 off[PG];
+            if (map) {
+                const Stream ms = stream(map + ((size_t)tile << 12));
+#pragma unroll
+                for (int i = 0; i < PG; ++i) off[i] = 8u * ld32(ms, 4u * (u32)tau, 1024 * i, 1024 * g);
+            } else {
+#pragma unroll
+                for (int i = 0; i < PG; ++i) off[i] = ((u32)tile << 15) + lane8 + 2048u * (u32)(g + i);
+            }
+#pragma unroll 1
+            for (int j = 0; j < sh.beta; ++j) {
+                const Stream ds = stream(dig + ((size_t)j * nt << log_n));
+                const Stream ks = stream(key + (size_t)(2 * j + comp) * kstride + klimb);
+                u64 d[PG], kw[PG];
+#pragma unroll
+                for (int i = 0; i < PG; ++i) {
+                    d[i] = ld64(ds, off[i], 0);
+                    kw[i] = ld64(ks, lane8, 2048 * i, 2048 * g);
+                }
+#pragma unroll
+                for (int i = 0; i < PG; ++i) {
+                    u32 d0, d1;
+                    split30(d[i], d0, d1);
+                    mac30(acc[i], d0, d1, (u32)kw[i] & 0x3FFFFFFFu, (u32)(kw[i] >> khi));
+                }
+                if (!SHORT && ++pending == 8) {
+                    pending = 0;
+                    const bool fold = ++folded == 2;
+                    if (fold) folded = 0;
+#pragma unroll
+                    for (int i = 0; i < PG; ++i) {
+                        acc30_flush(acc[i], lo[i], hi[i]);
+                        acc[i] = Acc30{0, 0, 0};
+                        if (fold) {
+                            lo[i] = barrett_reduce128(lo[i], hi[i], br);
+                            hi[i] = 0;
+                        }
+                    }
+                }
+            }
+        }
+        u64* const fg = from + lds_slot(tile_index(0, 1, 8)) * g;
+#pragma unroll
+        for (int i = 0; i < PG; ++i) {
+            acc30_flush(acc[i], lo[i], hi[i]);
+            fg[lds_slot(tile_index(0, i, 8))] = redc128(lo[i], hi[i], q, qi);
+        }
+    }
+}
+
+template <bool INVERSE, bool LAZY, bool EPI, bool PROD = false>
 __device__ __forceinline__ void rows_body(const NttArgs& a, u64* lds, int vec, int tile, int limb, const LimbConst& c,
                                           const NttEpilogue* ep) {
     const int log_n = a.log_n;
@@ -416,11 +523,19 @@
             for (int k = 0; k < 16; ++k) st64(base, lane8, koff(k, 8), x[k]);
         }
     } else {
-#pragma unroll
-        for (int k = 0; k < 16; ++k) x[k] = ld64(sbase, lane8, koff(k, 8));
         RoundTw rt, rn;
-        load_round_tw_rows(rt, trows, tau);
-        exchange(x, lds, tau, 8, 0, false);
+        if constexpr (PROD) {
+            load_round_tw_rows(rt, trows, tau);
+            __syncthreads();
+            const u64* const to = lds + lds_slot(tile_index(tau, 0, 0));
+#pragma unroll
+            for (int k = 0; k < 16; ++k) x[k] = to[lds_slot(tile_index(0, k, 0))];
+        } else {
+#pragma unroll
+            for (int k = 0; k < 16; ++k) x[k] = ld64(sbase, lane8, koff(k, 8));
+            load_round_tw_rows(rt, trows, tau);
+            exchange(x, lds, tau, 8, 0, false);
+        }
         inv_round<0, 4, false, LAZY, 0, 1>(x, rt, c, nullptr);
         load_round_tw<0, 4>(rn, tw, log_n, 4, tile << 4, tau >> 4);
         exchange(x, lds, tau, 0, 4, true);
@@ -434,14 +549,11 @@
     }
 }
 
-template <bool INVERSE, bool EPI = false>
-__global__ __launch_bounds__(256) __attribute__((amdgpu_waves_per_eu(4))) void ntt_rows_kernel(NttArgs a, NttEpilogue ep) {
-    __shared__ u64 lds[LDS_WORDS];
+__device__ __forceinline__ void rows_block(const NttArgs& a, int& vec, int& tile) {
     const int logtiles = a.log_n - 12;
     int lid = blockIdx.x;
     const int nblk = gridDim.x;
     if ((nblk & 7) == 0) lid = (lid & 7) * (nblk >> 3) + (lid >> 3);
-    int vec, tile;
     if (a.period > 0) {
         const int nper = a.nvec / a.period;
         const int rep = lid % nper, r = lid / nper;
@@ -453,6 +565,13 @@
     }
     vec = uniform(vec);
     tile = uniform(tile);
+}
+
+template <bool INVERSE, bool EPI = false>
+__global__ __launch_bounds__(256) __attribute__((amdgpu_waves_per_eu(4))) void ntt_rows_kernel(NttArgs a, NttEpilogue ep) {
+    __shared__ u64 lds[LDS_WORDS];
+    int vec, tile;
+    rows_block(a, vec, tile);
     const int limb = uniform(limb_of(a, vec));
     if (limb < 0) return;
     const LimbConst c = limb_const(a, limb);
@@ -460,6 +579,23 @@
         rows_body<INVERSE, true, EPI>(a, lds, vec, tile, limb, c, &ep);
     else
         rows_body<INVERSE, false, EPI>(a, lds, vec, tile, limb, c, &ep);
+}
+
+__global__ __launch_bounds__(256) __attribute__((amdgpu_waves_per_eu(4))) void ntt_rows_product_kernel(NttArgs a, NttProduct pr, const u64* barrett,
+                                                                                                        const u64* qinv) {
+    __shared__ u64 lds[LDS_WORDS];
+    int vec, tile;
+    rows_block(a, vec, tile);
+    const int limb = uniform(limb_of(a, vec));
+    const LimbConst c = limb_const(a, limb);
+    if ((pr.multi ? pr.sh.n_rot : 1) * pr.sh.beta <= 8)
+        product_to_lds<8, true>(lds, a, pr, barrett, qinv, vec, tile, limb, c.q, threadIdx.x);
+    else
+        product_to_lds<4, false>(lds, a, pr, barrett, qinv, vec, tile, limb, c.q, threadIdx.x);
+    if (lazy_prime<true>(c.q))
+        rows_body<true, true, false, true>(a, lds, vec, tile, limb, c, nullptr);
+    else
+        rows_body<true, false, false, true>(a, lds, vec, tile, limb, c, nullptr);
 }
 
 template <int A>
@@ -474,14 +610,21 @@
 
 }
 
-static void launch_ntt_impl(const DeviceTables& t, const LimbBatch& b, bool inverse, const NttEpilogue* ep, hipStream_t s);
+enum NttPasses { BOTH_PASSES, ROWS_PRODUCT, COLS_ONLY };
+static void launch_ntt_impl(const DeviceTables& t, const LimbBatch& b, bool inverse, const NttEpilogue* ep, hipStream_t s,
+                            NttPasses which = BOTH_PASSES, const NttProduct* prod = nullptr);
 
 void launch_ntt(const DeviceTables& t, const LimbBatch& b, bool inverse, hipStream_t s) { launch_ntt_impl(t, b, inverse, nullptr, s); }
 void launch_ntt_epilogue(const DeviceTables& t, const LimbBatch& b, const NttEpilogue& ep, hipStream_t s) {
     launch_ntt_impl(t, b, false, &ep, s);
 }
-
-static void launch_ntt_impl(const DeviceTables& t, const LimbBatch& b, bool inverse, const NttEpilogue* ep, hipStream_t s) {
+void launch_ntt_rows_product(const DeviceTables& t, const LimbBatch& b, const NttProduct& p, hipStream_t s) {
+    launch_ntt_impl(t, b, true, nullptr, s, ROWS_PRODUCT, &p);
+}
+void launch_ntt_cols_inverse(const DeviceTables& t, const LimbBatch& b, hipStream_t s) { launch_ntt_impl(t, b, true, nullptr, s, COLS_ONLY); }
+
+static void launch_ntt_impl(const DeviceTables& t, const LimbBatch& b, bool inverse, const NttEpilogue* ep, hipStream_t s, NttPasses which,
+                            const NttProduct* prod) {
     if (b.nvec <= 0) return;
     NttArgs a;
     a.data = b.data;
@@ -512,7 +655,7 @@
         return e ? std::atoi(e) : 0;
     }();
     int chunk = b.nvec;
-    if (chunk_mb > 0 && !ep) {
+    if (chunk_mb > 0 && !ep && which == BOTH_PASSES) {
         const size_t vec_bytes = (size_t)8 << t.log_n;
         const int want = (int)std::max<size_t>(1, ((size_t)chunk_mb << 20) / vec_bytes);
         if (b.nvec > want + want / 2) {
@@ -552,7 +695,11 @@
             else
                 hipLaunchKernelGGL((ntt_rows_kernel<false, false>), dim3(blocks), dim3(256), 0, s, a, NttEpilogue());
         } else {
-            hipLaunchKernelGGL((ntt_rows_kernel<true, false>), dim3(blocks), dim3(256), 0, s, a, NttEpilogue());
+            if (which == ROWS_PRODUCT) {
+                hipLaunchKernelGGL(ntt_rows_product_kernel, dim3(blocks), dim3(256), 0, s, a, *prod, t.barrett, t.qinv);
+                continue;
+            }
+            if (which != COLS_ONLY) hipLaunchKernelGGL((ntt_rows_kernel<true, false>), dim3(blocks), dim3(256), 0, s, a, NttEpilogue());
             a.src = a.data;
             a.src_group = 0;
             a.src_group2 = 0;
diff --git a/include/fhelin.h b/include/fhelin.h
--- a/include/fhelin.h
+++ b/include/fhelin.h
@@ -163,6 +163,8 @@
                             const fhelin_pt* const* pts , fhelin_ct* const* dest , int32_t accumulate);
 int fhelin_debug_rotate_many_batch(fhelin_ctx* c, const fhelin_ct* const* cts, int32_t n_ct, const int32_t* indices, int32_t n,
                                    fhelin_ct** outs );
+int fhelin_debug_ks_accp(fhelin_ctx* c, const uint64_t* digits, int32_t ell, int32_t batch, const int32_t* indices, int32_t n_rot,
+                         uint64_t* out );
 
 int fhelin_fc_mult_const(fhelin_ctx* c, const fhelin_ct* a, double d, fhelin_ct** out);
 int fhelin_fc_mask(fhelin_ctx* c, const fhelin_ct* a, int32_t kind, int32_t x, int32_t y, double v, fhelin_ct** out);
```
